# gmongaras/Stable-Diffusion-3-From-Scratch

Measured on AMD Instinct MI355X. Metric: train images/sec MMDiT-B 256^2 bf16, higher is better.
Workload: dtype bf16

## Files before the change

stable-diffusion-3-from-scratch_amd/_lib.py:

```python
import ctypes
import os
import re

_HERE = os.path.dirname(os.path.abspath(__file__))
def experiment(name: str, default: str) -> str:
    return os.environ.get(name, default) if os.environ.get("MMDIT_EXPERIMENTS") == "1" else default


LIB_PATH = os.environ.get("MMDIT_LIB") or os.path.join(_HERE, "libmmdit_hip.so")
HEADER_PATH = os.path.join(_HERE, "..", "include", "mmdit_hip.h")
HEADER_EXT_PATH = os.path.join(_HERE, "..", "include", "mmdit_hip_ext.h")
HEADER_HD128_PATH = os.path.join(_HERE, "..", "include", "mmdit_hip_hd128.h")
HEADER_ROPE3_PATH = os.path.join(_HERE, "..", "include", "mmdit_hip_rope3.h")
HEADER_QKHALF_PATH = os.path.join(_HERE, "..", "include", "mmdit_hip_qkhalf.h")
HEADER_TEXTLOSS_PATH = os.path.join(_HERE, "..", "include", "mmdit_hip_textloss.h")
HEADER_COS2_PATH = os.path.join(_HERE, "..", "include", "mmdit_hip_cos2.h")
HEADER_FP8PAD_PATH = os.path.join(_HERE, "..", "include", "mmdit_hip_fp8pad.h")
HEADER_MXPAD_PATH = os.path.join(_HERE, "..", "include", "mmdit_hip_mxpad.h")
HEADER_OPTIM_PATH = os.path.join(_HERE, "..", "include", "mmdit_hip_optim.h")

F32, BF16 = 0, 1
ACT_NONE, ACT_SILU, ACT_SWIGLU, ACT_SWIGLU_BWD = 0, 1, 2, 3
PREC_BF16, PREC_SPLIT = 0, 1
FP8 = 2

_vp, _i, _i64, _f, _d = ctypes.c_void_p, ctypes.c_int, ctypes.c_int64, ctypes.c_float, ctypes.c_double


class GemmArgs(ctypes.Structure):
    _fields_ = [
        ("A", _vp), ("a_dtype", _i), ("a_kmajor", _i), ("lda", _i64),
        ("B", _vp), ("b_dtype", _i), ("b_kmajor", _i), ("ldb", _i64),
        ("C", _vp), ("c_dtype", _i), ("ldc", _i64),
        ("M", _i), ("N", _i), ("K", _i),
        ("bias", _vp),
        ("act", _i),
        ("gate", _vp), ("ld_gate", _i64), ("rows_per_batch", _i),
        ("residual", _vp), ("ld_res", _i64),
        ("aux", _vp), ("aux_dtype", _i), ("ld_aux", _i64),
        ("accumulate", _i),
        ("precision", _i),
        ("split_k", _i),
        ("stream_k", _i),
        ("conv_mode", _i), ("conv_H", _i), ("conv_W", _i), ("conv_C", _i),
        ("scale_a", _vp), ("scale_b", _vp), ("scale_mode", _i), ("c_scales", _vp),
        ("dbias", _vp),
        ("cu_budget", _i),
    ]


class LnFwdProblem(ctypes.Structure):
    _fields_ = [("x", ctypes.c_void_p), ("acc", ctypes.c_void_p), ("gate", ctypes.c_void_p), ("ld_gate", ctypes.c_int64), ("x_out", ctypes.c_void_p),
                ("scale", ctypes.c_void_p), ("shift", ctypes.c_void_p), ("ld_mod", ctypes.c_int64), ("rows", ctypes.c_int), ("rows_per_batch", ctypes.c_int),
                ("out", ctypes.c_void_p), ("mean", ctypes.c_void_p), ("rstd", ctypes.c_void_p)]


class LnBwdProblem(ctypes.Structure):
    _fields_ = [("dout", ctypes.c_void_p), ("x", ctypes.c_void_p), ("mean", ctypes.c_void_p), ("rstd", ctypes.c_void_p), ("scale", ctypes.c_void_p),
                ("ld_mod", ctypes.c_int64), ("dres", ctypes.c_void_p), ("rows", ctypes.c_int), ("rows_per_batch", ctypes.c_int),
                ("dx", ctypes.c_void_p), ("dscale", ctypes.c_void_p), ("dshift", ctypes.c_void_p), ("ld_dmod", ctypes.c_int64),
                ("acc", ctypes.c_void_p), ("gate", ctypes.c_void_p), ("ld_gate", ctypes.c_int64), ("dacc", ctypes.c_void_p), ("dgate", ctypes.c_void_p),
                ("ld_dgate", ctypes.c_int64), ("dbias", ctypes.c_void_p), ("ld_dbias", ctypes.c_int64)]


class QkProblem(ctypes.Structure):
    _fields_ = [("qkv", ctypes.c_void_p), ("wq", ctypes.c_void_p), ("wk", ctypes.c_void_p), ("rope_cos", ctypes.c_void_p), ("rope_sin", ctypes.c_void_p),
                ("tokens", ctypes.c_int), ("tok0", ctypes.c_int), ("dqkv", ctypes.c_void_p), ("dwq", ctypes.c_void_p), ("dwk", ctypes.c_void_p)]


class MlpBwdProblem(ctypes.Structure):
    _fields_ = [("dh", ctypes.c_void_p), ("gu", ctypes.c_void_p), ("dgu", ctypes.c_void_p), ("rows", ctypes.c_int), ("dbias", ctypes.c_void_p)]


class QkEpilogue(ctypes.Structure):
    _fields_ = [("wq", _vp), ("wk", _vp), ("rope_cos", _vp), ("rope_sin", _vp), ("tokens", _i), ("tok0", _i)]


_SIGNATURES = {
    "mmdit_abi_version": ([], _i),
    "mmdit_struct_size": ([_i], _i),
    "mmdit_build_arch": ([], ctypes.c_char_p),
    "mmdit_gemm": ([ctypes.POINTER(GemmArgs), _vp], _i),
    "mmdit_gemm_grouped": ([ctypes.POINTER(GemmArgs), _i, _vp], _i),
    "mmdit_gemm_plan": ([ctypes.POINTER(GemmArgs), _i], _i),
    "mmdit_gemm_set_workspace": ([_vp, ctypes.c_longlong], _i),
    "mmdit_debug_occupy": ([_i, ctypes.c_longlong, _vp], _i),
    "mmdit_gemm_set_claiming": ([_i], _i),
    "mmdit_gemm_get_claiming": ([], _i),
    "mmdit_device_cus": ([], _i),
    "mmdit_gemm_qkv_norm_rope": ([ctypes.POINTER(GemmArgs), ctypes.POINTER(QkEpilogue), _i, _i, _i, _vp, _vp, _vp, _vp], _i),
    "mmdit_gemm_zero_mask": ([ctypes.POINTER(GemmArgs), _i, ctypes.POINTER(ctypes.c_uint)], _i),
    "mmdit_fp8_amax": ([_vp, _i, _i64, _vp, _vp], _i),
    "mmdit_fp8_quantize": ([_vp, _i, _i64, _vp, _vp, _vp, _vp], _i),
    "mmdit_fp8_quantize_delayed": ([_vp, _i, _i64, _vp, _i, ctypes.c_float, _vp, _vp], _i),
    "mmdit_mxfp8_quantize": ([_vp, _i, _i, _i, _i64, _vp, _vp, _vp], _i),
    "mmdit_ln_modulate_fwd_mx": ([_vp, _vp, _i, _vp, _i64, _vp, _vp, _vp, _i64, _i, _i, _i, _vp, _vp, _vp, _vp, _vp], _i),
    "mmdit_swiglu_fwd_mx": ([_vp, _i, _i, _i, _vp, _vp, _vp], _i),
    "mmdit_attn_fwd_mx": ([_vp, _vp, _vp, _i, _i, _i, _i, ctypes.c_float, _vp, _vp, _vp, _vp, _vp], _i),
    "mmdit_cast": ([_vp, _i, _vp, _i, _i64, _vp], _i),
    "mmdit_ln_modulate_fwd": ([ctypes.POINTER(LnFwdProblem), _i, _i, _i, _i, _vp], _i),
    "mmdit_ln_modulate_bwd": ([ctypes.POINTER(LnBwdProblem), _i, _i, _i, _vp], _i),
    "mmdit_qk_norm_rope_fwd": ([ctypes.POINTER(QkProblem), _i, _i, _i, _i, _i, _vp, _vp, _vp, _vp], _i),
    "mmdit_qk_norm_rope_bwd": ([ctypes.POINTER(QkProblem), _i, _vp, _vp, _vp, _i, _i, _i, _i, _i, _i, _vp], _i),
    "mmdit_qk_norm_rope_fwd_merge": ([ctypes.POINTER(QkProblem), _i, _i, _i, _i, _i, _vp, _vp, _vp, _vp], _i),
    "mmdit_qk_norm_rope_bwd_merge": ([ctypes.POINTER(QkProblem), _i, _vp, _vp, _vp, _i, _i, _i, _i, _i, _i, _vp], _i),
    "mmdit_mlp_act_bwd": ([ctypes.POINTER(MlpBwdProblem), _i, _i, _i, _i, _vp], _i),
    "mmdit_gate_residual_fwd": ([_vp, _vp, _i, _vp, _i64, _i, _i, _i, _vp, _vp], _i),
    "mmdit_text_rmsnorm_fwd": ([_vp, _i, _vp, _vp, _vp, _vp, _i, _i, _i, _i, _vp, _vp, _i, _vp], _i),
    "mmdit_text_rmsnorm_bwd": ([_vp, _vp, _i, _vp, _i, _vp, _vp, _vp, _vp, _i, _i, _i, _i, _vp, _vp, _vp, _vp, _vp], _i),
    "mmdit_attn_fwd": ([_vp, _vp, _vp, _i, _i, _i, _i, _f, _i, _vp, _vp, _vp, _vp], _i),
    "mmdit_attn_bwd_qk": ([_vp] * 9 + [_i, _i, _i, _i, _f] + [_vp] * 11 + [_vp], _i),
    "mmdit_attn_bwd": ([_vp, _vp, _vp, _vp, _vp, _vp, _vp, _vp, _vp, _i, _i, _i, _i, _f, _vp, _vp, _vp, _i, _vp], _i),
    "mmdit_attn_fwd_kv": ([_vp, _vp, _vp, _i, _i, _i, _i, _i, _f, _i, _vp, _vp, _vp, _vp], _i),
    "mmdit_attn_bwd_kv": ([_vp, _vp, _vp, _vp, _vp, _vp, _vp, _vp, _vp, _i, _i, _i, _i, _i, _f, _vp, _vp, _vp, _i, _vp], _i),
    "mmdit_swiglu_fwd": ([_vp, _vp, _i, _i, _i, _vp], _i),
    "mmdit_gelu_fwd": ([_vp, _vp, _i, _i, _i, _vp], _i),
    "mmdit_silu_bwd": ([_vp, _i, _vp, _vp, _i, _i, _i, _vp, _i, _vp], _i),
    "mmdit_gate_residual_bwd": ([_vp, _vp, _i, _vp, _i64, _i, _i, _i, _vp, _i, _vp, _i64, _vp, _i64, _vp], _i),
    "mmdit_flow_loss": ([_vp, _vp, _vp, _i, _i64, _f, _vp, _vp, _vp, _vp], _i),
    "mmdit_colsum": ([_vp, _i, _i, _i, _i64, _vp, _vp], _i),
    "mmdit_vae_nchw_to_nhwc": ([_vp, _i, _i, _i, _i, _i, _i, ctypes.c_float, ctypes.c_float, _vp, _vp], _i),
    "mmdit_vae_nhwc_to_nchw": ([_vp, _i, _i, _i, _i, _i, ctypes.c_float, ctypes.c_float, _vp, _vp], _i),
    "mmdit_vae_im2col3x3": ([_vp, _i, _i, _i, _i, _i, _vp, _vp], _i),
    "mmdit_vae_groupnorm": ([_vp, _i, _vp, _vp, _i, _i, _i, _i, _i, ctypes.c_float, _i, _vp, _vp, _i, _vp], _i),
    "mmdit_vae_pad_cast": ([_vp, _i, _i, _i, _i, _i, _i, _vp, _vp], _i),
    "mmdit_vae_softmax_rows": ([_vp, _i, _i, _i, ctypes.c_float, _vp, _vp], _i),
    "mmdit_vae_attn_fwd": ([_vp, _vp, _vp, _i, _i, _i, _i, _f, _vp, _vp], _i),
    "mmdit_patchify": ([_vp, _i, _i, _i, _i, _i, _vp, _i, _vp], _i),
    "mmdit_unpatchify": ([_vp, _i, _i, _i, _i, _i, _vp, _i, _vp], _i),
    "mmdit_time_embed_fwd": ([_vp, _vp, _vp, _i, _i, _vp, _i, _vp], _i),
    "mmdit_time_embed_bwd": ([_vp, _i, _vp, _vp, _vp, _i, _i, _vp, _vp], _i),
    "mmdit_grad_sumsq": ([_vp, _vp, _vp, _i, _vp, _vp], _i),
    "mmdit_clip_coef": ([_vp, _i, _vp, _f, _vp, _vp], _i),
    "mmdit_adamw_step": ([_vp, _vp, _vp, _i, _vp, _vp, _d, _d, _d, _d, _d, _vp], _i),
    "mmdit_adamw_step_dlr": ([_vp, _vp, _vp, _i, _vp, _vp, _vp, _d, _d, _d, _d, _vp], _i),
    "mmdit_cast_multi": ([_vp, _vp, _vp, _i, _vp], _i),
}
_EXT_SIGNATURES = {
    "mmdit_attn_fwd_e4m3": ([_vp, _vp, _vp, _i, _i, _i, _i, _f, _vp, _vp, _vp, _vp, _vp], _i),
}
ATTN_E4M3_KEY_TILE, ATTN_E4M3_QUERY_TILE = 64, 128
_HD128_SIGNATURES = {
    "mmdit_attn_fwd_hd128": _SIGNATURES["mmdit_attn_fwd"],
    "mmdit_attn_bwd_hd128": _SIGNATURES["mmdit_attn_bwd"],
    "mmdit_qk_norm_rope_fwd_hd128": _SIGNATURES["mmdit_qk_norm_rope_fwd"],
    "mmdit_qk_norm_rope_bwd_hd128": _SIGNATURES["mmdit_qk_norm_rope_bwd"],
}
ATTN_HD128_KEY_TILE, ATTN_HD128_QUERY_TILE = 32, 128
QK_HD128_MAX_HEADS, QK_HD128_RL_MIN_ROWS = 21, 2048
_ROPE3_SIGNATURES = {
    "mmdit_qk_norm_rope3_fwd": ([ctypes.POINTER(QkProblem), _i, _i, _i, _i, _i, _i, _vp, _vp, _vp, _vp], _i),
    "mmdit_qk_norm_rope3_bwd": ([ctypes.POINTER(QkProblem), _i, _vp, _vp, _vp, _i, _i, _i, _i, _i, _i, _i, _vp], _i),
}
_QKHALF_SIGNATURES = {
    "mmdit_attn_fwd_qkhalf": _SIGNATURES["mmdit_attn_fwd"],
    "mmdit_attn_bwd_qkhalf": _SIGNATURES["mmdit_attn_bwd"],
    "mmdit_qk_norm_rope_fwd_qkhalf": ([ctypes.POINTER(QkProblem), _i, _i, _i, _i, _i, _i, _i, _vp, _vp, _vp, _vp], _i),
    "mmdit_qk_norm_rope_bwd_qkhalf": ([ctypes.POINTER(QkProblem), _i, _vp, _vp, _vp, _i, _i, _i, _i, _i, _i, _i, _i, _vp], _i),
}
QKHALF_QK_DIM, QKHALF_V_DIM = 32, 64
ATTN_QKHALF_KEY_TILE, ATTN_QKHALF_QUERY_TILE = 32, 128
_TEXTLOSS_SIGNATURES = {
    "mmdit_text_loss": ([_vp, _i, _vp, _i, _vp, _i64, _i, _f, _vp, _i, _vp, _vp, _vp], _i),
}
TEXT_LOSS_ROWS_PER_WG, TEXT_LOSS_MAX_PARTIALS = 4, 256
TEXT_LOSS_LANE_COLS, TEXT_LOSS_WAVE_COLS = 8, 512
_COS2_SIGNATURES = {
    "mmdit_qk_l2norm_rope_fwd": ([ctypes.POINTER(QkProblem), _i, _i, _i, _i, _i, _i, _vp, _vp, _vp, _vp], _i),
    "mmdit_qk_l2norm_rope_bwd": ([ctypes.POINTER(QkProblem), _i, _vp, _vp, _vp, _i, _i, _i, _i, _i, _i, _vp], _i),
    "mmdit_attn_cos2_ws_bytes": ([_i, _i, _i], ctypes.c_longlong),
    "mmdit_attn_cos2_fwd": ([_vp, _vp, _vp, _i, _i, _i, _i, _i, _vp, _vp, _i, _vp, _vp, _vp], _i),
    "mmdit_attn_cos2_bwd": ([_vp, _vp, _vp, _i, _vp, _vp, _vp, _vp, _i, _vp, _i, _i, _i, _i, _vp, _vp, _vp, _i, _vp, _vp], _i),
}
_FP8PAD_SIGNATURES = {
    "mmdit_fp8_quantize_pad": ([_vp, _i, _i, _i, _i64, _vp, _vp, _vp, _vp], _i),
    "mmdit_fp8_quantize_delayed_pad": ([_vp, _i, _i, _i, _i64, _vp, _i, ctypes.c_float, _vp, _vp], _i),
    "mmdit_mxfp8_quantize_pad": ([_vp, _i, _i, _i, _i64, _vp, _vp, _vp], _i),
}
_MXPAD_SIGNATURES = {
    "mmdit_ln_modulate_fwd_mx_pad": ([ctypes.POINTER(LnFwdProblem), _i, _i, _i, _vp, _vp, _vp], _i),
    "mmdit_attn_fwd_mx_pad": _SIGNATURES["mmdit_attn_fwd_mx"],
    "mmdit_attn_fwd_e4m3_mx_pad": _EXT_SIGNATURES["mmdit_attn_fwd_e4m3"],
}
_OPTIM_SIGNATURES = {
    "mmdit_adamw_step_dlr_pt": _SIGNATURES["mmdit_adamw_step_dlr"],
}
COS2_HEAD_DIM = 64
ATTN_COS2_TOKEN_CHUNK, ATTN_COS2_ROW_TILE = 128, 64
HEAD_DIMS = (64, 128)
ADAMW_CHUNK = 65536
ABI_VERSION = 10
_STRUCTS = [("mmdit_gemm_args", GemmArgs), ("mmdit_ln_fwd_problem", LnFwdProblem), ("mmdit_ln_bwd_problem", LnBwdProblem),
            ("mmdit_qk_problem", QkProblem), ("mmdit_mlp_bwd_problem", MlpBwdProblem), ("mmdit_adamw_tensor", None), ("mmdit_cast_tensor", None), ("mmdit_qk_epilogue", QkEpilogue)]

_lib = None


def declared_symbols():
    with open(HEADER_PATH) as f:
        txt = f.read()
    return sorted(set(re.findall(r"\b(mmdit_[a-z0-9_]+)\s*\(", txt)) - {"mmdit_stream_t"})


def declared_ext_symbols():
    with open(HEADER_EXT_PATH) as f:
        txt = f.read()
    return sorted(set(re.findall(r"\b(mmdit_[a-z0-9_]+)\s*\(", txt)) - {"mmdit_stream_t"})


def declared_hd128_symbols():
    with open(HEADER_HD128_PATH) as f:
        txt = f.read()
    return sorted(set(re.findall(r"\b(mmdit_[a-z0-9_]+)\s*\(", txt)) - {"mmdit_stream_t"})


def declared_rope3_symbols():
    with open(HEADER_ROPE3_PATH) as f:
        txt = f.read()
    return sorted(set(re.findall(r"\b(mmdit_[a-z0-9_]+)\s*\(", txt)) - {"mmdit_stream_t"})


def declared_qkhalf_symbols():
    with open(HEADER_QKHALF_PATH) as f:
        txt = f.read()
    return sorted(set(re.findall(r"\b(mmdit_[a-z0-9_]+)\s*\(", txt)) - {"mmdit_stream_t"})


def declared_textloss_symbols():
    with open(HEADER_TEXTLOSS_PATH) as f:
        txt = f.read()
    return sorted(set(re.findall(r"\b(mmdit_[a-z0-9_]+)\s*\(", txt)) - {"mmdit_stream_t"})


def declared_cos2_symbols():
    with open(HEADER_COS2_PATH) as f:
        txt = f.read()
    return sorted(set(re.findall(r"\b(mmdit_[a-z0-9_]+)\s*\(", txt)) - {"mmdit_stream_t"})


def declared_fp8pad_symbols():
    with open(HEADER_FP8PAD_PATH) as f:
        txt = f.read()
    return sorted(set(re.findall(r"\b(mmdit_[a-z0-9_]+)\s*\(", txt)) - {"mmdit_stream_t"})


def declared_mxpad_symbols():
    with open(HEADER_MXPAD_PATH) as f:
        txt = f.read()
    return sorted(set(re.findall(r"\b(mmdit_[a-z0-9_]+)\s*\(", txt)) - {"mmdit_stream_t"})


def declared_optim_symbols():
    with open(HEADER_OPTIM_PATH) as f:
        txt = f.read()
    return sorted(set(re.findall(r"\b(mmdit_[a-z0-9_]+)\s*\(", txt)) - {"mmdit_stream_t"})


def lib():
    global _lib
    if _lib is None:
        if not os.path.exists(LIB_PATH):
            raise RuntimeError(
                f"{LIB_PATH} is missing: build it with `python __graft_entry__.py build` "
                "(hipcc --offload-arch=gfx950).  There is no PyTorch/CPU fallback for the MMDiT hot path.")
        try:
            import torch
            if torch.cuda.is_available():
                torch.cuda.init()
        except ImportError:
            pass
        L = ctypes.CDLL(LIB_PATH)
        for name, (argtypes, restype) in (list(_SIGNATURES.items()) + list(_EXT_SIGNATURES.items()) + list(_HD128_SIGNATURES.items()) + list(_ROPE3_SIGNATURES.items())
                                          + list(_QKHALF_SIGNATURES.items()) + list(_TEXTLOSS_SIGNATURES.items()) + list(_COS2_SIGNATURES.items()) + list(_FP8PAD_SIGNATURES.items()) + list(_MXPAD_SIGNATURES.items())
                                          + list(_OPTIM_SIGNATURES.items())):
            fn = getattr(L, name)
            fn.argtypes = argtypes
            fn.restype = restype
        if L.mmdit_abi_version() != ABI_VERSION:
            raise RuntimeError(f"{LIB_PATH}: ABI version {L.mmdit_abi_version()}, this binding is written for {ABI_VERSION}: rebuild (python __graft_entry__.py build)")
        for which, (name, struct) in enumerate(_STRUCTS):
            if struct is not None and L.mmdit_struct_size(which) != ctypes.sizeof(struct):
                raise RuntimeError(f"{LIB_PATH}: sizeof({name}) = {L.mmdit_struct_size(which)}, the binding's ctypes mirror has {ctypes.sizeof(struct)} bytes")
        _lib = L
    return _lib


ERR_ARG, ERR_DTYPE, ERR_SHAPE = -1, -2, -3


def check(status: int, what: str):
    if status != 0:
        kind = {-1: "invalid argument", -2: "dtype combination not built", -3: "unsupported shape"}.get(status, f"hipError {status}")
        raise RuntimeError(f"{what} failed: {kind}")
```

stable-diffusion-3-from-scratch_amd/build.py:

```python
import hashlib
import os
import subprocess
import sys
from concurrent.futures import ThreadPoolExecutor

HERE = os.path.dirname(os.path.abspath(__file__))
CSRC = os.path.join(HERE, "csrc")
LIB = os.path.join(HERE, "libmmdit_hip.so")
HEADER = os.path.join(HERE, "..", "include", "mmdit_hip.h")
HEADER_EXT = os.path.join(HERE, "..", "include", "mmdit_hip_ext.h")
HEADER_HD128 = os.path.join(HERE, "..", "include", "mmdit_hip_hd128.h")
HEADER_ROPE3 = os.path.join(HERE, "..", "include", "mmdit_hip_rope3.h")
HEADER_QKHALF = os.path.join(HERE, "..", "include", "mmdit_hip_qkhalf.h")
HEADER_TEXTLOSS = os.path.join(HERE, "..", "include", "mmdit_hip_textloss.h")
HEADER_COS2 = os.path.join(HERE, "..", "include", "mmdit_hip_cos2.h")
HEADER_FP8PAD = os.path.join(HERE, "..", "include", "mmdit_hip_fp8pad.h")
HEADER_MXPAD = os.path.join(HERE, "..", "include", "mmdit_hip_mxpad.h")
HEADER_OPTIM = os.path.join(HERE, "..", "include", "mmdit_hip_optim.h")
SOURCES = ["gemm.hip", "gemm_dma.hip", "gemm_lean.hip", "gemm8p.hip", "gemm8p_inf.hip", "rowops.hip", "fp8_pad.hip", "attention.hip", "attention_e4m3.hip", "attention_hd128.hip", "rowops_rope3.hip", "attention_qkhalf.hip", "rowops_qkhalf.hip", "attention_cos2.hip", "rowops_cos2.hip", "text_loss.hip", "vae.hip", "vae_attn.hip", "optim.hip"]
HIPCC = os.environ.get("HIPCC", "/opt/rocm/bin/hipcc")
FLAGS = ["--offload-arch=gfx950", "-O3", "-std=c++17", "-fPIC"] + os.environ.get("MMDIT_EXTRA_HIPCC_FLAGS", "").split()
SOURCE_FLAGS = {"vae_attn.hip": ["-mllvm", "-amdgpu-mfma-vgpr-form=1"]}


def _sha(paths, extra=""):
    h = hashlib.sha256(extra.encode())
    for p in paths:
        with open(p, "rb") as f:
            h.update(os.path.basename(p).encode() + b"\0" + f.read() + b"\0")
    return h.hexdigest()


def _read(path):
    try:
        with open(path) as f:
            return f.read().strip()
    except OSError:
        return None


def source_hash(src):
    headers = sorted(os.path.join(CSRC, f) for f in os.listdir(CSRC) if f.endswith(".h")) + [HEADER, HEADER_EXT, HEADER_HD128, HEADER_ROPE3, HEADER_QKHALF, HEADER_TEXTLOSS, HEADER_COS2, HEADER_FP8PAD, HEADER_MXPAD, HEADER_OPTIM]
    if src == "gemm8p_inf.hip":
        headers.append(os.path.join(CSRC, "gemm8p.hip"))
    return _sha([os.path.join(CSRC, src)] + headers, " ".join([HIPCC] + FLAGS + SOURCE_FLAGS.get(src, [])))


def build(force: bool = False, verbose: bool = False) -> str:
    want = {src: source_hash(src) for src in SOURCES}

    def cc(src):
        obj = os.path.join(CSRC, src.replace(".hip", ".o"))
        if not force and os.path.exists(obj) and _read(obj + ".sha") == want[src]:
            return obj, False
        cmd = [HIPCC] + FLAGS + SOURCE_FLAGS.get(src, []) + ["-c", os.path.join(CSRC, src), "-o", obj]
        if verbose:
            print(" ".join(cmd), flush=True)
        subprocess.run(cmd, check=True)
        with open(obj + ".sha", "w") as f:
            f.write(want[src])
        return obj, True

    with ThreadPoolExecutor(max_workers=8) as ex:
        res = list(ex.map(cc, SOURCES))
    objs = [o for o, _ in res]
    libsha = hashlib.sha256("".join(want[s] for s in SOURCES).encode()).hexdigest()
    if force or any(c for _, c in res) or not os.path.exists(LIB) or _read(LIB + ".sha") != libsha:
        cmd = [HIPCC, "--offload-arch=gfx950", "-shared", "-fPIC", "-o", LIB] + objs
        if verbose:
            print(" ".join(cmd), flush=True)
        subprocess.run(cmd, check=True)
        with open(LIB + ".sha", "w") as f:
            f.write(libsha)
    return LIB


def is_current() -> bool:
    libsha = hashlib.sha256("".join(source_hash(s) for s in SOURCES).encode()).hexdigest()
    return os.path.exists(LIB) and _read(LIB + ".sha") == libsha


if __name__ == "__main__":
    print(build(force="--force" in sys.argv, verbose=True))
```

stable-diffusion-3-from-scratch_amd/csrc/rowops.hip:

```cpp
#include "qk_rows.h"
#include "fp8_quant.h"
#include "../../include/mmdit_hip_hd128.h"
#include "../../include/mmdit_hip_mxpad.h"

namespace {

constexpr float LN_EPS = 1e-5f;

__device__ __forceinline__ float bf16_round(float x) { return __builtin_bit_cast(float, pack_bf2(x, 0.f) << 16); }

template <int NITX, typename TO, typename TA, bool RES, bool MX = false, bool PAD = false>
__device__ __forceinline__ void ln_mod_fwd_body(int block, const float* __restrict__ x, const float* __restrict__ scale, const float* __restrict__ shift,
                                                int64_t ld_mod, int rows, int d, int rpb, TO* __restrict__ out,
                                                float* __restrict__ mean_o, float* __restrict__ rstd_o,
                                                const TA* __restrict__ acc, const float* __restrict__ gate, int64_t ld_gate, float* __restrict__ xo,
                                                unsigned char* __restrict__ mx_scales) {
  constexpr int NIT = NITX < 0 ? -NITX : NITX;
  constexpr bool EXACT = NITX < 0;
  const int lane = threadIdx.x & 63, row = block * 4 + (threadIdx.x >> 6);
  if (row >= rows) return;
  const int nch = d >> 2;
  const int b = row / rpb;
  const float* xr = x + (int64_t)row * d;
  float v[NIT][4];
  float s = 0.f;
#pragma unroll
  for (int it = 0; it < NIT; it++) {
    int ch = lane + 64 * it;
    if (EXACT || ch < nch) {
      ld4(xr + ch * 4, v[it]);
      if constexpr (RES) {
        float av[4], g[4];
        ld4(acc + (int64_t)row * d + ch * 4, av);
        ld4(gate + (int64_t)b * ld_gate + ch * 4, g);
#pragma unroll
        for (int e = 0; e < 4; e++) v[it][e] = v[it][e] + g[e] * av[e];
        __builtin_nontemporal_store(f32x4{v[it][0], v[it][1], v[it][2], v[it][3]}, (f32x4*)(xo + (int64_t)row * d + ch * 4));
      }
      s += v[it][0] + v[it][1] + v[it][2] + v[it][3];
    }
    else { v[it][0] = v[it][1] = v[it][2] = v[it][3] = 0.f; }
  }
  const float mean = wave_sum(s) / d;
  float q = 0.f;
#pragma unroll
  for (int it = 0; it < NIT; it++) {
    int ch = lane + 64 * it;
    if (EXACT || ch < nch) {
#pragma unroll
      for (int e = 0; e < 4; e++) { float c = v[it][e] - mean; q += c * c; }
    }
  }
  const float rstd = rsqrtf(wave_sum(q) / d + LN_EPS);
  if (lane == 0) { mean_o[row] = mean; rstd_o[row] = rstd; }
  const float* sc = scale + (int64_t)b * ld_mod;
  const float* sh = shift + (int64_t)b * ld_mod;
  TO* orow = out + (int64_t)row * d;
  const int ldo = PAD ? d + 64 : d;
  if constexpr (PAD) {
    if (lane < 4) *(uint4*)((unsigned char*)out + (int64_t)row * ldo + d + lane * 16) = make_uint4(0u, 0u, 0u, 0u);
    if (lane < 2) mx_scales[mx_scale_index(row, (d >> 5) + lane, rows)] = 0;
  }
#pragma unroll
  for (int it = 0; it < NIT; it++) {
    int ch = lane + 64 * it;
    if (EXACT || ch < nch) {
      float a[4], h[4], o[4];
      ld4(sc + ch * 4, a); ld4(sh + ch * 4, h);
#pragma unroll
      for (int e = 0; e < 4; e++) o[e] = (v[it][e] - mean) * rstd * (1.f + a[e]) + h[e];
      if constexpr (MX) {
#pragma unroll
        for (int e = 0; e < 4; e++) o[e] = bf16_round(o[e]);
        float amax = fmaxf(fmaxf(fabsf(o[0]), fabsf(o[1])), fmaxf(fabsf(o[2]), fabsf(o[3])));
        amax = fmaxf(amax, __shfl_xor(amax, 1, 64));
        amax = fmaxf(amax, __shfl_xor(amax, 2, 64));
        amax = fmaxf(amax, __shfl_xor(amax, 4, 64));
        float inv;
        const int ex = mx_exponent(amax, inv);
        *(unsigned*)((unsigned char*)out + (int64_t)row * ldo + ch * 4) = mx_pack4(o, inv);
        if ((lane & 7) == 0) mx_scales[mx_scale_index(row, ch >> 3, rows)] = (unsigned char)(ex + 127);
      } else {
        st4(orow + ch * 4, o);
      }
    }
  }
}

struct LnFwdProb {
  const float* x; const float* scale; const float* shift; int64_t ld_mod; int rows, rpb; void* out; float* mean; float* rstd;
  const void* acc; const float* gate; int64_t ld_gate; float* xo; unsigned char* mx_scales;
};
template <int NIT, typename TO, typename TA, bool RES, bool MX = false, bool PAD = false>
__global__ __launch_bounds__(256) void ln_mod_fwd_kernel(LnFwdProb p0, LnFwdProb p1, int nblk0, int d) {
  const bool first = (int)blockIdx.x < nblk0;
  const LnFwdProb& p = first ? p0 : p1;
  ln_mod_fwd_body<NIT, TO, TA, RES, MX, PAD>(first ? (int)blockIdx.x : (int)blockIdx.x - nblk0, p.x, p.scale, p.shift, p.ld_mod, p.rows, d, p.rpb, (TO*)p.out, p.mean, p.rstd,
                                        (const TA*)p.acc, p.gate, p.ld_gate, p.xo, p.mx_scales);
}

template <typename TA>
__global__ __launch_bounds__(256) void gate_residual_fwd_kernel(const float* __restrict__ x, const TA* __restrict__ acc, const float* __restrict__ gate, int64_t ld_gate,
                                                                int rows, int d, int rpb, float* __restrict__ out) {
  const int nch = d >> 2;
  for (int64_t i = (int64_t)blockIdx.x * 256 + threadIdx.x; i < (int64_t)rows * nch; i += (int64_t)gridDim.x * 256) {
    const int row = (int)(i / nch), ch = (int)(i - (int64_t)row * nch);
    float xv[4], av[4], g[4];
    ld4(x + (int64_t)row * d + ch * 4, xv);
    ld4(acc + (int64_t)row * d + ch * 4, av);
    ld4(gate + (int64_t)(row / rpb) * ld_gate + ch * 4, g);
#pragma unroll
    for (int e = 0; e < 4; e++) xv[e] = xv[e] + g[e] * av[e];
    st4(out + (int64_t)row * d + ch * 4, xv);
  }
}

#ifndef MMDIT_LN_BWD_RCH
#define MMDIT_LN_BWD_RCH 16
#endif
constexpr int LN_BWD_RCH = MMDIT_LN_BWD_RCH;
template <int NITX, typename TG, typename TA, bool GATED>
__device__ __forceinline__ void ln_mod_bwd_body(int block, const TG* __restrict__ dout, const float* __restrict__ x, const float* __restrict__ mean_i,
                                                const float* __restrict__ rstd_i, const float* __restrict__ scale, int64_t ld_mod,
                                                const float* __restrict__ dres, int d, int rpb, int nchunk,
                                                float* __restrict__ dx, float* __restrict__ dscale, float* __restrict__ dshift, int64_t ld_dmod,
                                                const TA* __restrict__ acc, const float* __restrict__ gate, int64_t ld_gate, TA* __restrict__ dacc,
                                                float* __restrict__ dgate, int64_t ld_dgate, float* __restrict__ dbias, int64_t ld_dbias, int rch = LN_BWD_RCH) {
  constexpr int NIT = NITX < 0 ? -NITX : NITX;
  constexpr bool EXACT = NITX < 0;
  const int lane = threadIdx.x & 63, wave = threadIdx.x >> 6;
  const int b = block / nchunk, chunk = block % nchunk;
  const int nch = d >> 2;
  const float* sc = scale + (int64_t)b * ld_mod;
  __shared__ float s_a1[NIT * 256], s_gt[GATED ? NIT * 256 : 4];
  for (int c = threadIdx.x; c < NIT * 256; c += 256) {
    s_a1[c] = c < d ? sc[c] + 1.f : 0.f;
    if constexpr (GATED) s_gt[c] = c < d ? gate[(int64_t)b * ld_gate + c] : 0.f;
  }
  __syncthreads();
  float ds[NIT][4], dh[NIT][4];
  float sg[GATED ? NIT : 1][4], sb[GATED ? NIT : 1][4];
#pragma unroll
  for (int it = 0; it < NIT; it++) {
#pragma unroll
    for (int e = 0; e < 4; e++) { ds[it][e] = 0.f; dh[it][e] = 0.f; }
    if constexpr (GATED) {
#pragma unroll
      for (int e = 0; e < 4; e++) { sg[it][e] = 0.f; sb[it][e] = 0.f; }
    }
  }
  const int rend = min(rpb, (chunk + 1) * rch);
  for (int rl = chunk * rch + wave; rl < rend; rl += 4) {
    const int64_t row = (int64_t)b * rpb + rl;
    const float mean = mean_i[row], rstd = rstd_i[row];
    float g[NIT][4], xh[NIT][4];
    float c1 = 0.f, c2 = 0.f;
    asm volatile("" ::: "memory");
#pragma unroll
    for (int it = 0; it < NIT; it++) {
      int ch = lane + 64 * it;
      if (EXACT || ch < nch) {
        float dy[4], xv[4], a1[4];
        ld4_nt(dout + row * d + ch * 4, dy);
        ld4_nt(x + row * d + ch * 4, xv);
        ld4(s_a1 + ch * 4, a1);
#pragma unroll
        for (int e = 0; e < 4; e++) {
          xh[it][e] = (xv[e] - mean) * rstd;
          g[it][e] = dy[e] * a1[e];
          c1 += g[it][e]; c2 += g[it][e] * xh[it][e];
          ds[it][e] += dy[e] * xh[it][e]; dh[it][e] += dy[e];
        }
      }
    }
    c1 = wave_sum(c1) / d; c2 = wave_sum(c2) / d;
#pragma unroll
    for (int it = 0; it < NIT; it++) {
      int ch = lane + 64 * it;
      if (EXACT || ch < nch) {
        float o[4];
        if (dres) ld4(dres + row * d + ch * 4, o); else { o[0] = o[1] = o[2] = o[3] = 0.f; }
#pragma unroll
        for (int e = 0; e < 4; e++) o[e] += rstd * (g[it][e] - c1 - xh[it][e] * c2);
        st4(dx + row * d + ch * 4, o);
        if constexpr (GATED) {
          float av[4], da[4], gt[4];
          ld4_nt(acc + row * d + ch * 4, av);
          ld4(s_gt + ch * 4, gt);
#pragma unroll
          for (int e = 0; e < 4; e++) { da[e] = o[e] * gt[e]; sg[it][e] += o[e] * av[e]; sb[it][e] += da[e]; }
          st4(dacc + row * d + ch * 4, da);
        }
      }
    }
  }
  if constexpr (NIT <= 6) {
    __shared__ float red[4][NIT * 256];
    auto flush = [&](const float (&v)[NIT][4], float* dst) {
#pragma unroll
      for (int it = 0; it < NIT; it++)
#pragma unroll
        for (int e = 0; e < 4; e++) red[wave][(it * 64 + lane) * 4 + e] = v[it][e];
      __syncthreads();
      for (int c = threadIdx.x; c < d; c += 256) atomicAdd(dst + c, red[0][c] + red[1][c] + red[2][c] + red[3][c]);
      __syncthreads();
    };
    flush(ds, dscale + (int64_t)b * ld_dmod);
    flush(dh, dshift + (int64_t)b * ld_dmod);
    if constexpr (GATED) {
      flush(sg, dgate + (int64_t)b * ld_dgate);
      if (dbias) flush(sb, dbias + (int64_t)b * ld_dbias);
    }
  } else {
    auto flush = [&](const float (&v)[NIT][4], float* dst) {
#pragma unroll
      for (int it = 0; it < NIT; it++) {
        int ch = lane + 64 * it;
        if (EXACT || ch < nch) {
#pragma unroll
          for (int e = 0; e < 4; e++) atomicAdd(dst + ch * 4 + e, v[it][e]);
        }
      }
    };
    flush(ds, dscale + (int64_t)b * ld_dmod);
    flush(dh, dshift + (int64_t)b * ld_dmod);
    if constexpr (GATED) {
      flush(sg, dgate + (int64_t)b * ld_dgate);
      if (dbias) flush(sb, dbias + (int64_t)b * ld_dbias);
    }
  }
}

struct LnBwdProb {
  const void* dout; const float* x; const float* mean; const float* rstd; const float* scale; int64_t ld_mod; const float* dres; int rpb, nchunk;
  float* dx; float* dscale; float* dshift; int64_t ld_dmod;
  const void* acc; const float* gate; int64_t ld_gate; void* dacc; float* dgate; int64_t ld_dgate; float* dbias; int64_t ld_dbias;
};
template <int NIT, typename TG, typename TA, bool GATED>
__global__ __launch_bounds__(256) void ln_mod_bwd_kernel(LnBwdProb p0, LnBwdProb p1, int nblk0, int d, int rch) {
  const bool first = (int)blockIdx.x < nblk0;
  const LnBwdProb& p = first ? p0 : p1;
  ln_mod_bwd_body<NIT, TG, TA, GATED>(first ? (int)blockIdx.x : (int)blockIdx.x - nblk0, (const TG*)p.dout, p.x, p.mean, p.rstd, p.scale, p.ld_mod, p.dres, d, p.rpb, p.nchunk,
                                      p.dx, p.dscale, p.dshift, p.ld_dmod, (const TA*)p.acc, p.gate, p.ld_gate, (TA*)p.dacc, p.dgate, p.ld_dgate, p.dbias, p.ld_dbias, rch);
}

template <int NITX, typename TI, typename TO>
__global__ __launch_bounds__(256) void text_rms_fwd_kernel(const TI* __restrict__ x, const float* __restrict__ w, const float* __restrict__ sp,
                                                           int rows, int cnt, int tokens, int off, int d, TO* __restrict__ out) {
  constexpr int NIT = NITX < 0 ? -NITX : NITX;
  constexpr bool EXACT = NITX < 0;
  const int lane = threadIdx.x & 63, m = blockIdx.x * 4 + (threadIdx.x >> 6);
  if (m >= rows) return;
  const int nch = d >> 2;
  const TI* xr = x + ((int64_t)(m / cnt) * tokens + off + m % cnt) * d;
  float v[NIT][4];
  float q = 0.f;
#pragma unroll
  for (int it = 0; it < NIT; it++) {
    int ch = lane + 64 * it;
    if (EXACT || ch < nch) { ld4(xr + ch * 4, v[it]); q += v[it][0] * v[it][0] + v[it][1] * v[it][1] + v[it][2] * v[it][2] + v[it][3] * v[it][3]; }
  }
  const float rinv = rsqrtf(wave_sum(q) / d + RMS_EPS);
  const float s = sp[0];
  TO* orow = out + (int64_t)m * d;
#pragma unroll
  for (int it = 0; it < NIT; it++) {
    int ch = lane + 64 * it;
    if (EXACT || ch < nch) {
      float wv[4], o[4];
      ld4(w + ch * 4, wv);
#pragma unroll
      for (int e = 0; e < 4; e++) o[e] = s * (v[it][e] * rinv * wv[e]);
      st4(orow + ch * 4, o);
    }
  }
}

#ifndef TRB_ROWS
#define TRB_ROWS 64
#endif
struct TextRmsBwdHalf { const void* dout; const float* w; const float* sp; int rows, cnt, off; float* dw; float* dsp; };
template <int NITX, typename TI, typename TG>
__global__ __launch_bounds__(512) void text_rms_bwd_kernel(TextRmsBwdHalf h0, TextRmsBwdHalf h1, const TI* __restrict__ x, int tokens, int d) {
  constexpr int NIT = NITX < 0 ? -NITX : NITX;
  constexpr bool EXACT = NITX < 0;
  const TextRmsBwdHalf& hp = blockIdx.y == 0 ? h0 : h1;
  const TG* __restrict__ dout = (const TG*)hp.dout;
  const float* __restrict__ w = hp.w;
  const float* __restrict__ sp = hp.sp;
  const int rows = hp.rows, cnt = hp.cnt, off = hp.off;
  float* __restrict__ dw = hp.dw;
  float* __restrict__ dsp = hp.dsp;
  __shared__ float red[NIT * 256];
  for (int c = threadIdx.x; c < NIT * 256; c += 512) red[c] = 0.f;
  __syncthreads();
  const int lane = threadIdx.x & 63, wave = threadIdx.x >> 6;
  const int nch = d >> 2;
  const float s = sp[0];
  float accw[NIT][4], wv[NIT][4];
  float accs = 0.f;
#pragma unroll
  for (int it = 0; it < NIT; it++) {
    int ch = lane + 64 * it;
    if (EXACT || ch < nch) ld4(w + ch * 4, wv[it]); else { wv[it][0] = wv[it][1] = wv[it][2] = wv[it][3] = 0.f; }
#pragma unroll
    for (int e = 0; e < 4; e++) accw[it][e] = 0.f;
  }
  for (int m = blockIdx.x * TRB_ROWS + wave; m < min(rows, (int)(blockIdx.x + 1) * TRB_ROWS); m += 8) {
    const TI* xr = x + ((int64_t)(m / cnt) * tokens + off + m % cnt) * d;
    float v[NIT][4];
    float q = 0.f;
#pragma unroll
    for (int it = 0; it < NIT; it++) {
      int ch = lane + 64 * it;
      if (EXACT || ch < nch) { ld4(xr + ch * 4, v[it]); q += v[it][0] * v[it][0] + v[it][1] * v[it][1] + v[it][2] * v[it][2] + v[it][3] * v[it][3]; }
    }
    const float rinv = rsqrtf(wave_sum(q) / d + RMS_EPS);
#pragma unroll
    for (int it = 0; it < NIT; it++) {
      int ch = lane + 64 * it;
      if (EXACT || ch < nch) {
        float dy[4];
        ld4(dout + (int64_t)m * d + ch * 4, dy);
#pragma unroll
        for (int e = 0; e < 4; e++) { float xn = v[it][e] * rinv; accw[it][e] += dy[e] * s * xn; accs += dy[e] * xn * wv[it][e]; }
      }
    }
  }
#pragma unroll
  for (int it = 0; it < NIT; it++) {
    const int ch = lane + 64 * it;
    if (EXACT || ch < nch) {
#pragma unroll
      for (int e = 0; e < 4; e++) atomicAdd(&red[ch * 4 + e], accw[it][e]);
    }
  }
  __syncthreads();
#ifndef TRB_NO_GLOBAL
  for (int c = threadIdx.x; c < d; c += 512) atomicAdd(dw + c, red[c]);
#else
  if (red[threadIdx.x] == 123.456f) dw[0] = 1.f;
#endif
  accs = wave_sum(accs);
#ifndef TRB_NO_DSP
  if (lane == 0) atomicAdd(dsp, accs);
#else
  if (accs == 123.456f) dsp[0] = 1.f;
#endif
}


template <int HD, typename TI>
__device__ __forceinline__ void qk_norm_rope_fwd_body(int bid, int rstride, const TI* __restrict__ qkv, const float* __restrict__ wq, const float* __restrict__ wk,
                                                      const float* __restrict__ rcos, const float* __restrict__ rsin,
                                                      int rows, int tokens, int heads, int s_total, int tok0,
                                                      bf16_t* __restrict__ Q, bf16_t* __restrict__ K, bf16_t* __restrict__ V) {
  constexpr int CH = HD / 8, LOG_CH = CH == 8 ? 3 : 4;
  const int hc = threadIdx.x % (CH * heads), part = threadIdx.x / (CH * heads), head = hc >> LOG_CH, chunk = hc & (CH - 1);
  bf16_t* obase = part == 0 ? Q : part == 1 ? K : V;
  float w[8];
#pragma unroll
  for (int e = 0; e < 8; e++) w[e] = 0.f;
  if (part < 2) ld8((part == 0 ? wq : wk) + chunk * 8, w);
  const bool same_token = rcos && rstride % tokens == 0;
  float cs[2][8], sn[2][8];
  if (same_token && part < 2) {
    const int n = bid % tokens;
    ld8(rcos + (int64_t)n * HD + chunk * 8, cs[0]);
    ld8(rsin + (int64_t)n * HD + chunk * 8, sn[0]);
#pragma unroll
    for (int e = 0; e < 8; e++) { cs[1][e] = cs[0][e]; sn[1][e] = sn[0][e]; }
  }
  for (int row0 = bid; row0 < rows; row0 += 2 * rstride) {
    float x[2][8];
#pragma unroll
    for (int k = 0; k < 2; k++) {
      const int row = min(row0 + k * rstride, rows - 1);
      ld8(qkv + (((int64_t)row * 3 + part) * heads + head) * HD + chunk * 8, x[k]);
    }
    if (part < 2 && rcos && !same_token) {
#pragma unroll
      for (int k = 0; k < 2; k++) {
        const int n = min(row0 + k * rstride, rows - 1) % tokens;
        ld8(rcos + (int64_t)n * HD + chunk * 8, cs[k]);
        ld8(rsin + (int64_t)n * HD + chunk * 8, sn[k]);
      }
    }
#pragma unroll
    for (int k = 0; k < 2; k++) {
      const int row = row0 + k * rstride;
      if (row >= rows) break;
      const int n = row % tokens, b = row / tokens;
      if (part < 2) {
        float ss = 0.f;
#pragma unroll
        for (int e = 0; e < 8; e++) ss += x[k][e] * x[k][e];
        const float rinv = rsqrtf(group_sum<CH>(ss) * (1.f / HD) + RMS_EPS);
#pragma unroll
        for (int e = 0; e < 8; e++) x[k][e] = x[k][e] * rinv * w[e];
        if (rcos) {
#pragma unroll
          for (int p = 0; p < 4; p++) {
            float a = x[k][2 * p], bb = x[k][2 * p + 1];
            x[k][2 * p] = a * cs[k][2 * p] - bb * sn[k][2 * p];
            x[k][2 * p + 1] = bb * cs[k][2 * p + 1] + a * sn[k][2 * p + 1];
          }
        }
      }
      st8(obase + (((int64_t)b * heads + head) * s_total + tok0 + n) * HD + chunk * 8, x[k]);
    }
  }
}
template <int HD, typename TI>
__global__ __launch_bounds__(1024) void qk_norm_rope_fwd_kernel(QkProb p0, QkProb p1, int g0, int heads, int s_total,
                                                                bf16_t* __restrict__ Q, bf16_t* __restrict__ K, bf16_t* __restrict__ V) {
  QK_SELECT(p, bid, nwg);
  qk_norm_rope_fwd_body<HD, TI>(bid, nwg, (const TI*)p.qkv, p.wq, p.wk, p.rcos, p.rsin, p.rows, p.tokens, heads, s_total, p.tok0, Q, K, V);
}

enum QkFactors {
  QK_ONCE,
  QK_PER_PAIR,
  QK_PER_ROW,
};

template <int HD, QkFactors F, typename TG, typename TI, typename TO>
__device__ __forceinline__ void qk_norm_rope_bwd_body(int bid, int rstride, const TG* __restrict__ dQ, const TG* __restrict__ dK, const TG* __restrict__ dV,
                                                      const TI* __restrict__ qkv, const float* __restrict__ wq, const float* __restrict__ wk,
                                                      const float* __restrict__ rcos, const float* __restrict__ rsin,
                                                      int rows, int tokens, int heads, int s_total, int tok0,
                                                      TO* __restrict__ dqkv, float* __restrict__ dwq, float* __restrict__ dwk) {
  constexpr int CH = HD / 8, LOG_CH = CH == 8 ? 3 : 4, LOG_HD = LOG_CH + 3;
  __shared__ float sdw[2][HD];
  for (int i = threadIdx.x; i < 2 * HD; i += blockDim.x) sdw[i >> LOG_HD][i & (HD - 1)] = 0.f;
  __syncthreads();
  const int per_row = 3 * CH * heads, rlane = threadIdx.x / per_row, t = threadIdx.x - rlane * per_row;
  { const int RL = blockDim.x / per_row; bid = bid * RL + rlane; rstride *= RL; }
  const int hc = t % (CH * heads), part = t / (CH * heads);
  const int head = HD == 64 ? hc >> LOG_CH : hc / CH, chunk = HD == 64 ? hc & (CH - 1) : hc % CH;
  const TG* gbase = part == 0 ? dQ : part == 1 ? dK : dV;
  float w[8], aw[8];
#pragma unroll
  for (int e = 0; e < 8; e++) { w[e] = 0.f; aw[e] = 0.f; }
  if (part < 2) ld8((part == 0 ? wq : wk) + chunk * 8, w);
  const bool same_token = F == QK_ONCE ? rcos != nullptr : (rcos && rstride % tokens == 0);
  constexpr int NF = F == QK_PER_PAIR ? 2 : 1;
  float cs[NF][8], sn[NF][8];
  if (same_token && part < 2) {
    const int n = bid % tokens;
    ld8(rcos + (int64_t)n * HD + chunk * 8, cs[0]);
    ld8(rsin + (int64_t)n * HD + chunk * 8, sn[0]);
    if constexpr (F == QK_PER_PAIR) {
#pragma unroll
      for (int e = 0; e < 8; e++) { cs[1][e] = cs[0][e]; sn[1][e] = sn[0][e]; }
    }
  }
  for (int row0 = bid; row0 < rows; row0 += 2 * rstride) {
    float dz[2][8], x[2][8];
#pragma unroll
    for (int k = 0; k < 2; k++) {
      const int row = min(row0 + k * rstride, rows - 1);
      const int n = row % tokens, b = row / tokens;
      ld8_nt(gbase + (((int64_t)b * heads + head) * s_total + tok0 + n) * HD + chunk * 8, dz[k]);
    }
    if (part < 2) {
#pragma unroll
      for (int k = 0; k < 2; k++) {
        const int row = min(row0 + k * rstride, rows - 1);
        ld8_nt(qkv + (((int64_t)row * 3 + part) * heads + head) * HD + chunk * 8, x[k]);
        if constexpr (F == QK_PER_PAIR) {
          if (rcos && !same_token) {
            const int n = row % tokens;
            ld8(rcos + (int64_t)n * HD + chunk * 8, cs[k]);
            ld8(rsin + (int64_t)n * HD + chunk * 8, sn[k]);
          }
        }
      }
    }
// ... 249 lines not shown
  if (ty == 0 && c < ncols) {
#pragma unroll
    for (int e = 0; e < 8; e++) atomicAdd(dst + c + e, acc[e] + sbuf[tx * 8 + e]);
  }
  __syncthreads();
}

constexpr int MB_RCH = 128;
template <typename T, bool GELU>
__device__ __forceinline__ void mlp_act_bwd_body(int by, const T* __restrict__ dh, const T* __restrict__ gu, T* __restrict__ dgu,
                                                 int rows, int hidden, float* __restrict__ dbias) {
  __shared__ float sbuf[8 * 256];
  const int tx = threadIdx.x & 31, ty = threadIdx.x >> 5;
  const int c = blockIdx.x * 256 + tx * 8;
  const bool act = c < hidden;
  const int64_t ldi = GELU ? hidden : 2 * (int64_t)hidden;
  float sg[8], su[8];
#pragma unroll
  for (int e = 0; e < 8; e++) { sg[e] = 0.f; su[e] = 0.f; }
  const int rend = min(rows, (by + 1) * MB_RCH);
  if (act) {
    for (int r0 = by * MB_RCH + ty; r0 < rend; r0 += 16) {
      float d[2][8], g[2][8], u[2][8];
#pragma unroll
      for (int k = 0; k < 2; k++) {
        const int r = r0 + 8 * k;
        if (r < rend) {
          ld8_nt(dh + (int64_t)r * hidden + c, d[k]);
          ld8_nt(gu + r * ldi + c, g[k]);
          if constexpr (!GELU) ld8_nt(gu + r * ldi + hidden + c, u[k]);
        }
      }
#pragma unroll
      for (int k = 0; k < 2; k++) {
        const int r = r0 + 8 * k;
        if (r >= rend) break;
        float og[8], ou[8];
        if constexpr (GELU) {
#pragma unroll
          for (int e = 0; e < 8; e++) { og[e] = d[k][e] * gelu_grad_f(g[k][e]); sg[e] += og[e]; }
          st8(dgu + r * ldi + c, og);
        } else {
#pragma unroll
          for (int e = 0; e < 8; e++) {
            swiglu_bwd_f(d[k][e], g[k][e], u[k][e], og[e], ou[e]);
            sg[e] += og[e]; su[e] += ou[e];
          }
          st8(dgu + r * ldi + c, og);
          st8(dgu + r * ldi + hidden + c, ou);
        }
      }
    }
  }
  if (dbias) {
    const int col = blockIdx.x * 256 + threadIdx.x;
#pragma unroll
    for (int which = 0; which < (GELU ? 1 : 2); which++) {
#pragma unroll
      for (int e = 0; e < 8; e++) sbuf[ty * 256 + tx * 8 + e] = which == 0 ? sg[e] : su[e];
      __syncthreads();
      if (col < hidden) {
        float s = 0.f;
#pragma unroll
        for (int r = 0; r < 8; r++) s += sbuf[r * 256 + threadIdx.x];
        atomicAdd(dbias + which * hidden + col, s);
      }
      __syncthreads();
    }
  }
}
struct MlpBwdProb { const void* dh; const void* gu; void* dgu; int rows; float* dbias; };
template <typename T, bool GELU>
__global__ __launch_bounds__(256) void mlp_act_bwd_kernel(MlpBwdProb p0, MlpBwdProb p1, int nby0, int hidden) {
  const bool first = (int)blockIdx.y < nby0;
  const MlpBwdProb& p = first ? p0 : p1;
  mlp_act_bwd_body<T, GELU>(first ? (int)blockIdx.y : (int)blockIdx.y - nby0, (const T*)p.dh, (const T*)p.gu, (T*)p.dgu, p.rows, hidden, p.dbias);
}

constexpr int GR_RCH = 64;
template <typename TA, typename TO>
__global__ __launch_bounds__(256) void gate_res_bwd_kernel(const float* __restrict__ dy, const TA* __restrict__ acc, const float* __restrict__ gate, int64_t ld_gate,
                                                           int d, int rpb, int nchunk, TO* __restrict__ dacc,
                                                           float* __restrict__ dgate, int64_t ld_dgate, float* __restrict__ dbias, int64_t ld_dbias) {
  __shared__ float sbuf[8 * 256];
  const int tx = threadIdx.x & 31, ty = threadIdx.x >> 5;
  const int c = blockIdx.x * 256 + tx * 8;
  const bool act = c < d;
  const int b = blockIdx.y / nchunk, chunk = blockIdx.y % nchunk;
  float g[8], sgate[8], sb[8];
#pragma unroll
  for (int e = 0; e < 8; e++) { g[e] = 0.f; sgate[e] = 0.f; sb[e] = 0.f; }
  if (act) {
    ld8(gate + (int64_t)b * ld_gate + c, g);
    const int rend = min(rpb, (chunk + 1) * GR_RCH);
    for (int rl = chunk * GR_RCH + ty; rl < rend; rl += 16) {
      const int64_t row0 = (int64_t)b * rpb + rl, row1 = row0 + 8;
      const bool two = rl + 8 < rend;
      float dv0[8], av0[8], dv1[8], av1[8], o[8];
      ld8(dy + row0 * d + c, dv0);
      ld8(acc + row0 * d + c, av0);
      if (two) {
        ld8(dy + row1 * d + c, dv1);
        ld8(acc + row1 * d + c, av1);
      }
#pragma unroll
      for (int e = 0; e < 8; e++) { o[e] = dv0[e] * g[e]; sgate[e] += dv0[e] * av0[e]; sb[e] += o[e]; }
      st8(dacc + row0 * d + c, o);
      if (two) {
#pragma unroll
        for (int e = 0; e < 8; e++) { o[e] = dv1[e] * g[e]; sgate[e] += dv1[e] * av1[e]; sb[e] += o[e]; }
        st8(dacc + row1 * d + c, o);
      }
    }
  }
  const int col = blockIdx.x * 256 + threadIdx.x;
#pragma unroll
  for (int which = 0; which < 2; which++) {
    float* dst = which == 0 ? dgate + (int64_t)b * ld_dgate : (dbias ? dbias + (int64_t)b * ld_dbias : nullptr);
    if (!dst) break;
#pragma unroll
    for (int e = 0; e < 8; e++) sbuf[ty * 256 + tx * 8 + e] = which == 0 ? sgate[e] : sb[e];
    __syncthreads();
    if (col < d) {
      float s = 0.f;
#pragma unroll
      for (int r = 0; r < 8; r++) s += sbuf[r * 256 + threadIdx.x];
      atomicAdd(dst + col, s);
    }
    __syncthreads();
  }
}

template <typename T>
__global__ __launch_bounds__(256) void colsum_kernel(const T* __restrict__ x, int rows, int cols, int64_t ld, float* __restrict__ out, int rch) {
  __shared__ float sbuf[1024];
  const int tx = threadIdx.x & 127, ty = threadIdx.x >> 7;
  const int c = blockIdx.x * 1024 + tx * 8;
  float s[8];
#pragma unroll
  for (int e = 0; e < 8; e++) s[e] = 0.f;
  if (c < cols) {
    const int rend = min(rows, (int)(blockIdx.y + 1) * rch);
#pragma unroll 4
    for (int r = blockIdx.y * rch + ty; r < rend; r += 2) {
      float v[8];
      ld8(x + r * ld + c, v);
#pragma unroll
      for (int e = 0; e < 8; e++) s[e] += v[e];
    }
  }
  colsum_flush(s, sbuf, out, c, cols);
}

template <typename TG, typename TO>
__global__ __launch_bounds__(256) void silu_bwd_kernel(const TG* __restrict__ dy, const float* __restrict__ pre, TO* __restrict__ dpre, int rpg, int cols, float* __restrict__ dbias) {
  __shared__ float sb[4][64];
  const int cl = threadIdx.x & 63, rl = threadIdx.x >> 6;
  const int c = blockIdx.x * 64 + cl;
  const int r0 = blockIdx.y * rpg;
  float s = 0.f;
  if (c < cols) {
#pragma unroll 4
    for (int r = r0 + rl; r < r0 + rpg; r += 4) {
      const int64_t i = (int64_t)r * cols + c;
      const float p = pre[i], sig = sigmoid_f(p);
      const float g = io<TG>::ld(dy + i) * sig * (1.f + p * (1.f - sig));
      io<TO>::st(dpre + i, g);
      s += g;
    }
  }
  sb[rl][cl] = s;
  __syncthreads();
  if (rl == 0 && c < cols && dbias) dbias[(int64_t)blockIdx.y * cols + c] += sb[0][cl] + sb[1][cl] + sb[2][cl] + sb[3][cl];
}

template <typename TI, typename TO>
__global__ void cast_kernel(const TI* __restrict__ src, TO* __restrict__ dst, int64_t n) {
  const int64_t n8 = n >> 3;
  for (int64_t i = (int64_t)blockIdx.x * blockDim.x + threadIdx.x; i < n8; i += (int64_t)gridDim.x * blockDim.x) {
    float v[8];
    ld8(src + i * 8, v);
    st8(dst + i * 8, v);
  }
  if (blockIdx.x == 0 && threadIdx.x < (n & 7)) io<TO>::st(dst + n8 * 8 + threadIdx.x, io<TI>::ld(src + n8 * 8 + threadIdx.x));
}

template <typename TI, typename TO, bool TO_TOKENS>
__global__ void patch_kernel(const TI* __restrict__ src, TO* __restrict__ dst, int batch, int ch, int H, int W) {
  const int W2 = W >> 1, H2 = H >> 1;
  const int64_t total = (int64_t)batch * ch * H * W2;
  for (int64_t g = (int64_t)blockIdx.x * blockDim.x + threadIdx.x; g < total; g += (int64_t)gridDim.x * blockDim.x) {
    const int j = (int)(g % W2); int64_t r = g / W2;
    const int y = (int)(r % H); r /= H;
    const int c = (int)(r % ch); const int64_t b = r / ch;
    const int64_t img_off = ((b * ch + c) * H + y) * W + 2 * j;
    const int64_t tok_off = ((b * H2 + (y >> 1)) * W2 + j) * (int64_t)(ch * 4) + c * 4 + (y & 1) * 2;
    if (TO_TOKENS) { io<TO>::st(dst + tok_off, io<TI>::ld(src + img_off)); io<TO>::st(dst + tok_off + 1, io<TI>::ld(src + img_off + 1)); }
    else { io<TO>::st(dst + img_off, io<TI>::ld(src + tok_off)); io<TO>::st(dst + img_off + 1, io<TI>::ld(src + tok_off + 1)); }
  }
}

template <typename TO>
__global__ void time_embed_fwd_kernel(const float* __restrict__ t, const float* __restrict__ ts, const float* __restrict__ denom, int batch, int dim, TO* __restrict__ out) {
  const int i = blockIdx.x * blockDim.x + threadIdx.x, b = blockIdx.y;
  if (i >= dim) return;
  const float tau = t[b] * ts[0];
  const int half = dim >> 1;
  const float v = i < half ? sinf(tau / denom[2 * i]) : cosf(tau / denom[2 * (i - half) + 1]);
  io<TO>::st(out + (int64_t)b * dim + i, v);
}

template <typename TG>
__global__ __launch_bounds__(256) void time_embed_bwd_kernel(const TG* __restrict__ dout, const float* __restrict__ t, const float* __restrict__ ts,
                                                             const float* __restrict__ denom, int batch, int dim, float* __restrict__ dts) {
  __shared__ float red[4];
  const int b = blockIdx.x;
  const float tau = t[b] * ts[0];
  const int half = dim >> 1;
  float s = 0.f;
  for (int i = threadIdx.x; i < dim; i += 256) {
    const float g = io<TG>::ld(dout + (int64_t)b * dim + i);
    if (i < half) { const float dn = denom[2 * i]; s += g * cosf(tau / dn) / dn; }
    else { const float dn = denom[2 * (i - half) + 1]; s -= g * sinf(tau / dn) / dn; }
  }
  s = wave_sum(s);
  if ((threadIdx.x & 63) == 0) red[threadIdx.x >> 6] = s;
  __syncthreads();
  if (threadIdx.x == 0) atomicAdd(dts, (red[0] + red[1] + red[2] + red[3]) * t[b]);
}

inline int nit_for(int d) { return (d / 4 + 63) / 64; }
inline int grid_cap(int64_t n, int bs) { int64_t g = (n + bs - 1) / bs; return (int)(g < 1 ? 1 : g > 4096 ? 4096 : g); }

}

#define NIT_CASE(n, ...)                                                        \
  { if (d == (n) * 256) { constexpr int NIT = -(n); __VA_ARGS__; } else { constexpr int NIT = (n); __VA_ARGS__; } }
#define NIT_SWITCH(nit, ...)                                    \
  do {                                                          \
    if (nit <= 1) NIT_CASE(1, __VA_ARGS__)                      \
    else if (nit <= 2) NIT_CASE(2, __VA_ARGS__)                 \
    else if (nit <= 3) NIT_CASE(3, __VA_ARGS__)                 \
    else if (nit <= 4) NIT_CASE(4, __VA_ARGS__)                 \
    else if (nit <= 6) NIT_CASE(6, __VA_ARGS__)                 \
    else if (nit <= 9) NIT_CASE(9, __VA_ARGS__)                 \
    else if (nit <= 12) NIT_CASE(12, __VA_ARGS__)               \
    else NIT_CASE(16, __VA_ARGS__)                              \
  } while (0)

#define LN_FWD_NIT (NIT < 0 ? -NIT : NIT)

extern "C" int mmdit_abi_version(void) { return MMDIT_ABI_VERSION; }
extern "C" int mmdit_struct_size(int which) {
  switch (which) {
    case 0: return (int)sizeof(mmdit_gemm_args);
    case 1: return (int)sizeof(mmdit_ln_fwd_problem);
    case 2: return (int)sizeof(mmdit_ln_bwd_problem);
    case 3: return (int)sizeof(mmdit_qk_problem);
    case 4: return (int)sizeof(mmdit_mlp_bwd_problem);
    case 5: return (int)sizeof(mmdit_adamw_tensor);
    case 6: return (int)sizeof(mmdit_cast_tensor);
    case 7: return (int)sizeof(mmdit_qk_epilogue);
    default: return -1;
  }
}
extern "C" const char* mmdit_build_arch(void) { return "gfx950"; }

static int ln_mod_fwd_launch(const mmdit_ln_fwd_problem* probs, int count, int d, int out_dtype, unsigned char* const* mx_scales, hipStream_t s, bool pad = false) {
  MMDIT_CHECK_ARG(probs && count >= 1 && count <= 2 && d > 0 && d % 4 == 0 && d <= 4096);
  const bool res = probs[0].acc != nullptr;
  LnFwdProb q[2] = {};
  int nb[2] = {0, 0};
  for (int i = 0; i < count; i++) {
    const mmdit_ln_fwd_problem* p = probs + i;
    MMDIT_CHECK_ARG((p->acc != nullptr) == res);
    MMDIT_CHECK_ARG(p->x && p->scale && p->shift && p->out && p->mean && p->rstd && p->rows > 0 && p->rows_per_batch > 0 && p->ld_mod % 4 == 0);
    if (res) MMDIT_CHECK_ARG(p->gate && p->x_out && p->ld_gate % 4 == 0);
    q[i] = LnFwdProb{p->x, p->scale, p->shift, p->ld_mod, p->rows, p->rows_per_batch, p->out, p->mean, p->rstd, p->acc, p->gate, p->ld_gate, p->x_out, mx_scales ? mx_scales[i] : nullptr};
    nb[i] = (p->rows + 3) / 4;
  }
  const int nit = nit_for(d);
  dim3 grid(nb[0] + nb[1]);
#define LNL(TO, TA, RES, ...) NIT_SWITCH(nit, hipLaunchKernelGGL((ln_mod_fwd_kernel<LN_FWD_NIT, TO, TA, RES, __VA_ARGS__>), grid, dim3(256), 0, s, q[0], q[1], nb[0], d))
  if (mx_scales && pad) { if (res) { LNL(unsigned char, bf16_t, true, true, true); } else { LNL(unsigned char, bf16_t, false, true, true); } }
  else if (mx_scales) { if (res) { LNL(unsigned char, bf16_t, true, true); } else { LNL(unsigned char, bf16_t, false, true); } }
  else if (out_dtype == MMDIT_BF16) { if (res) { LNL(bf16_t, bf16_t, true, false); } else { LNL(bf16_t, bf16_t, false, false); } }
  else if (out_dtype == MMDIT_F32) { if (res) { LNL(float, float, true, false); } else { LNL(float, float, false, false); } }
  else return MMDIT_ERR_DTYPE;
#undef LNL
  return mmdit_launch_status();
}

extern "C" int mmdit_ln_modulate_fwd(const mmdit_ln_fwd_problem* probs, int count, int d, int acc_dtype, int out_dtype, mmdit_stream_t stream) {
  MMDIT_CHECK_ARG(probs && count >= 1 && (!probs[0].acc || acc_dtype == out_dtype));
  return ln_mod_fwd_launch(probs, count, d, out_dtype, nullptr, (hipStream_t)stream);
}

extern "C" int mmdit_ln_modulate_fwd_mx(const float* x, const void* acc, int acc_dtype, const float* gate, int64_t ld_gate, float* x_out,
                                        const float* scale, const float* shift, int64_t ld_mod, int rows, int d, int rpb,
                                        void* q_fp8, void* scales_e8m0, float* mean, float* rstd, mmdit_stream_t stream) {
  MMDIT_CHECK_ARG(scales_e8m0 && d % 64 == 0 && (!acc || acc_dtype == MMDIT_BF16));
  const mmdit_ln_fwd_problem p = {x, acc, gate, ld_gate, x_out, scale, shift, ld_mod, rows, rpb, q_fp8, mean, rstd};
  unsigned char* const sc[1] = {(unsigned char*)scales_e8m0};
  return ln_mod_fwd_launch(&p, 1, d, MMDIT_FP8, sc, (hipStream_t)stream);
}

extern "C" int mmdit_ln_modulate_fwd_mx_pad(const mmdit_ln_fwd_problem* probs, int count, int d, int acc_dtype, void* scales_e8m0_0, void* scales_e8m0_1,
                                            mmdit_stream_t stream) {
  MMDIT_CHECK_ARG(probs && count >= 1 && count <= 2 && scales_e8m0_0 && (count == 1 || scales_e8m0_1));
  if (d <= 0 || d % 64 != 0) return MMDIT_ERR_SHAPE;
  for (int i = 0; i < count; i++)
    if (probs[i].rows > 0 && (int64_t)probs[i].rows * ((d + 127) / 128 * 128) / 16 > 0x7fffffffll) return MMDIT_ERR_SHAPE;
  MMDIT_CHECK_ARG(!probs[0].acc || acc_dtype == MMDIT_BF16);
  unsigned char* const sc[2] = {(unsigned char*)scales_e8m0_0, (unsigned char*)scales_e8m0_1};
  return ln_mod_fwd_launch(probs, count, d, MMDIT_FP8, sc, (hipStream_t)stream, d % 128 != 0);
}

extern "C" int mmdit_gate_residual_fwd(const float* x, const void* acc, int acc_dtype, const float* gate, int64_t ld_gate, int rows, int d, int rpb,
                                       float* out, mmdit_stream_t stream) {
  MMDIT_CHECK_ARG(x && acc && gate && out && rows > 0 && d > 0 && d % 4 == 0 && rpb > 0 && ld_gate % 4 == 0);
  hipStream_t s = (hipStream_t)stream;
  dim3 grid(grid_cap((int64_t)rows * (d / 4), 256));
  if (acc_dtype == MMDIT_BF16) hipLaunchKernelGGL((gate_residual_fwd_kernel<bf16_t>), grid, dim3(256), 0, s, x, (const bf16_t*)acc, gate, ld_gate, rows, d, rpb, out);
  else if (acc_dtype == MMDIT_F32) hipLaunchKernelGGL((gate_residual_fwd_kernel<float>), grid, dim3(256), 0, s, x, (const float*)acc, gate, ld_gate, rows, d, rpb, out);
  else return MMDIT_ERR_DTYPE;
  return mmdit_launch_status();
}

static int ln_bwd_one_round_rch(const mmdit_ln_bwd_problem* a, const mmdit_ln_bwd_problem* b, int d, int dout_dtype, bool gated) {
  auto wgs = [&](int r) { return (long)(a->rows / a->rows_per_batch) * ((a->rows_per_batch + r - 1) / r) + (long)(b->rows / b->rows_per_batch) * ((b->rows_per_batch + r - 1) / r); };
  const int nit_ = nit_for(d), nit_abs = nit_ < 0 ? -nit_ : nit_;
  int per_cu = nit_abs <= 3 ? 4 : nit_abs == 4 ? 3 : 2, cus = 256;
  {
    static int occ[64][17][2][2], cu_count[64];
    const int dev = mmdit_current_device(), ti = dout_dtype == MMDIT_BF16 ? 0 : 1, gi = gated ? 1 : 0, ni = nit_abs > 16 ? 16 : nit_abs;
    if (!cu_count[dev]) {
      int n = 0;
      cu_count[dev] = (hipDeviceGetAttribute(&n, hipDeviceAttributeMultiprocessorCount, dev) == hipSuccess && n > 0) ? n : 256;
    }
    cus = cu_count[dev];
    if (!occ[dev][ni][ti][gi]) {
      int nbq = 0;
      hipError_t e = hipErrorUnknown;
#define LNQ(T, G) NIT_SWITCH(nit_, e = hipOccupancyMaxActiveBlocksPerMultiprocessor(&nbq, (const void*)ln_mod_bwd_kernel<(NIT < 0 ? -NIT : NIT), T, T, G>, 256, 0))
      if (dout_dtype == MMDIT_BF16) { if (gated) { LNQ(bf16_t, true); } else { LNQ(bf16_t, false); } }
      else if (dout_dtype == MMDIT_F32) { if (gated) { LNQ(float, true); } else { LNQ(float, false); } }
#undef LNQ
      occ[dev][ni][ti][gi] = (e == hipSuccess && nbq > 0) ? nbq : 8;
    }
    per_cu = per_cu < occ[dev][ni][ti][gi] ? per_cu : occ[dev][ni][ti][gi];
  }
  const long slots = (long)cus * per_cu;
  if (wgs(LN_BWD_RCH) > slots && wgs(LN_BWD_RCH) <= 2 * slots)
    for (int r = LN_BWD_RCH + 4; r <= 64; r += 4)
      if (wgs(r) <= slots) return r;
  return LN_BWD_RCH;
}

extern "C" int mmdit_ln_modulate_bwd(const mmdit_ln_bwd_problem* probs, int count, int d, int dout_dtype, mmdit_stream_t stream) {
  MMDIT_CHECK_ARG(probs && count >= 1 && count <= 2 && d > 0 && d % 4 == 0 && d <= 4096);
  const bool gated = probs[0].acc != nullptr;
  for (int i = 0; i < count; i++) {
    const mmdit_ln_bwd_problem* p = probs + i;
    MMDIT_CHECK_ARG((p->acc != nullptr) == gated);
    MMDIT_CHECK_ARG(p->dout && p->x && p->mean && p->rstd && p->scale && p->dx && p->dscale && p->dshift && p->rows > 0 && p->rows_per_batch > 0 &&
                    p->rows % p->rows_per_batch == 0 && p->ld_mod % 4 == 0);
    if (gated) MMDIT_CHECK_ARG(p->gate && p->dacc && p->dgate && p->ld_gate % 4 == 0);
  }
  if (dout_dtype != MMDIT_BF16 && dout_dtype != MMDIT_F32) return MMDIT_ERR_DTYPE;
  const int rch = count == 2 ? ln_bwd_one_round_rch(probs, probs + 1, d, dout_dtype, gated) : LN_BWD_RCH;
  LnBwdProb q[2] = {};
  int nb[2] = {0, 0};
  for (int i = 0; i < count; i++) {
    const mmdit_ln_bwd_problem* p = probs + i;
    const int nchunk = (p->rows_per_batch + rch - 1) / rch;
    nb[i] = (p->rows / p->rows_per_batch) * nchunk;
    q[i] = LnBwdProb{p->dout, p->x, p->mean, p->rstd, p->scale, p->ld_mod, p->dres, p->rows_per_batch, nchunk, p->dx, p->dscale, p->dshift, p->ld_dmod,
                     p->acc, p->gate, p->ld_gate, p->dacc, p->dgate, p->ld_dgate, p->dbias, p->ld_dbias};
  }
  hipStream_t s = (hipStream_t)stream;
  const int nit = nit_for(d);
  dim3 grid(nb[0] + nb[1]);
#define LNL(T, G) NIT_SWITCH(nit, hipLaunchKernelGGL((ln_mod_bwd_kernel<(NIT < 0 ? -NIT : NIT), T, T, G>), grid, dim3(256), 0, s, q[0], q[1], nb[0], d, rch))
  if (dout_dtype == MMDIT_BF16) { if (gated) { LNL(bf16_t, true); } else { LNL(bf16_t, false); } }
  else { if (gated) { LNL(float, true); } else { LNL(float, false); } }
#undef LNL
  return mmdit_launch_status();
}

extern "C" int mmdit_text_rmsnorm_fwd(const void* x, int x_dtype, const float* w1, const float* w2, const float* s1, const float* s2,
                                      int batch, int tokens, int split, int d, void* out1, void* out2, int out_dtype, mmdit_stream_t stream) {
  MMDIT_CHECK_ARG(x && w1 && w2 && s1 && s2 && out1 && out2 && batch > 0 && split > 0 && split < tokens && d % 4 == 0 && d <= 4096);
  hipStream_t s = (hipStream_t)stream;
  const int nit = nit_for(d);
  for (int half = 0; half < 2; half++) {
    const int cnt = half ? tokens - split : split, off = half ? split : 0, rows = batch * cnt;
    const float* w = half ? w2 : w1; const float* sp = half ? s2 : s1; void* out = half ? out2 : out1;
    dim3 grid((rows + 3) / 4);
#define TRF(TI, TO) NIT_SWITCH(nit, hipLaunchKernelGGL((text_rms_fwd_kernel<LN_FWD_NIT, TI, TO>), grid, dim3(256), 0, s, (const TI*)x, w, sp, rows, cnt, tokens, off, d, (TO*)out))
    if (x_dtype == MMDIT_F32 && out_dtype == MMDIT_F32) { TRF(float, float); }
    else if (x_dtype == MMDIT_F32 && out_dtype == MMDIT_BF16) { TRF(float, bf16_t); }
    else if (x_dtype == MMDIT_BF16 && out_dtype == MMDIT_BF16) { TRF(bf16_t, bf16_t); }
    else if (x_dtype == MMDIT_BF16 && out_dtype == MMDIT_F32) { TRF(bf16_t, float); }
    else return MMDIT_ERR_DTYPE;
#undef TRF
  }
  return mmdit_launch_status();
}

extern "C" int mmdit_text_rmsnorm_bwd(const void* dout1, const void* dout2, int dout_dtype, const void* x, int x_dtype,
                                      const float* w1, const float* w2, const float* s1, const float* s2, int batch, int tokens, int split, int d,
                                      float* dw1, float* dw2, float* ds1, float* ds2, mmdit_stream_t stream) {
  MMDIT_CHECK_ARG(dout1 && dout2 && x && w1 && w2 && s1 && s2 && dw1 && dw2 && ds1 && ds2 && batch > 0 && split > 0 && split < tokens && d % 4 == 0 && d <= 4096);
  hipStream_t s = (hipStream_t)stream;
  const int nit = nit_for(d);
  TextRmsBwdHalf h[2];
  int maxrows = 0;
  for (int half = 0; half < 2; half++) {
    const int cnt = half ? tokens - split : split, rows = batch * cnt;
    h[half] = TextRmsBwdHalf{half ? dout2 : dout1, half ? w2 : w1, half ? s2 : s1, rows, cnt, half ? split : 0, half ? dw2 : dw1, half ? ds2 : ds1};
    maxrows = rows > maxrows ? rows : maxrows;
  }
  dim3 grid((maxrows + TRB_ROWS - 1) / TRB_ROWS, 2);
#define TRB(TI, TG) NIT_SWITCH(nit, hipLaunchKernelGGL((text_rms_bwd_kernel<NIT, TI, TG>), grid, dim3(512), 0, s, h[0], h[1], (const TI*)x, tokens, d))
  if (x_dtype == MMDIT_F32 && dout_dtype == MMDIT_F32) { TRB(float, float); }
  else if (x_dtype == MMDIT_F32 && dout_dtype == MMDIT_BF16) { TRB(float, bf16_t); }
  else if (x_dtype == MMDIT_BF16 && dout_dtype == MMDIT_BF16) { TRB(bf16_t, bf16_t); }
  else if (x_dtype == MMDIT_BF16 && dout_dtype == MMDIT_F32) { TRB(bf16_t, float); }
  else return MMDIT_ERR_DTYPE;
#undef TRB
  return mmdit_launch_status();
}

constexpr int QK_RL_MIN_ROWS = 2048;
static_assert(QK_RL_MIN_ROWS == MMDIT_QK_HD128_RL_MIN_ROWS && 1024 / (3 * 128 / 8) == MMDIT_QK_HD128_MAX_HEADS, "include/mmdit_hip_hd128.h documents this policy");
static int qk_rl(int row_threads, int min_rows) {
  static const int env = [] { const char* e = mmdit_exp_env("MMDIT_QK_RL"); return e ? atoi(e) : 0; }();
  int rl = 1024 / row_threads;
  if (env > 0 && env < rl) rl = env;
  if (rl < 1 || min_rows < QK_RL_MIN_ROWS) rl = 1;
  return rl;
}
static int qk_bwd_lanes(int rl) {
  static const int env = [] { const char* e = mmdit_exp_env("MMDIT_QK_LANES"); return e ? atoi(e) : 768; }();
  return rl > 1 ? env : 512;
}
static int qk_grid(int hd, int rows, int tokens, bool rope, int lanes_max, int rl) {
  const int lanes = rows < lanes_max ? rows : lanes_max;
  if (rope && tokens <= lanes) {
    int k = lanes / tokens;
    while (k > 1 && (k * tokens) % rl) k--;
    if ((k * tokens) % rl == 0) return k * tokens / rl;
  }
  if (hd == 64 && rope && tokens > lanes && tokens <= rows && tokens <= (rl > 1 ? 2048 : 1024) && tokens % rl == 0) return tokens / rl;
  return lanes / rl > 0 ? lanes / rl : 1;
}

template <int HD>
static int qk_fwd_launch(const mmdit_qk_problem* probs, int count, int qkv_dtype, int batch, int heads, int s_total, int heads_err,
                         void* Q, void* K, void* V, mmdit_stream_t stream) {
  constexpr int ROW_T = 3 * HD / 8;
  MMDIT_CHECK_ARG(Q && K && V);
  QkProb q[2] = {};
  if (int e = qk_list(probs, count, batch, heads, HD, s_total, 1024 / ROW_T, heads_err, false, false, nullptr, nullptr, nullptr, q)) return e;
  if (qkv_dtype != MMDIT_BF16 && qkv_dtype != MMDIT_F32) return MMDIT_ERR_DTYPE;
  int g[2] = {0, 0};
  for (int i = 0; i < count; i++) g[i] = qk_grid(HD, q[i].rows, q[i].tokens, q[i].rcos != nullptr, 1024, 1);
  hipStream_t s = (hipStream_t)stream;
  const dim3 grid(g[0] + g[1]), block(ROW_T * heads);
  if (qkv_dtype == MMDIT_BF16) hipLaunchKernelGGL((qk_norm_rope_fwd_kernel<HD, bf16_t>), grid, block, 0, s, q[0], q[1], g[0], heads, s_total, (bf16_t*)Q, (bf16_t*)K, (bf16_t*)V);
  else hipLaunchKernelGGL((qk_norm_rope_fwd_kernel<HD, float>), grid, block, 0, s, q[0], q[1], g[0], heads, s_total, (bf16_t*)Q, (bf16_t*)K, (bf16_t*)V);
  return mmdit_launch_status();
}

template <int HD>
static int qk_bwd_launch(const mmdit_qk_problem* probs, int count, const void* dQ, const void* dK, const void* dV, int dq_dtype,
                         int qkv_dtype, int dqkv_dtype, int batch, int heads, int s_total, int heads_err, mmdit_stream_t stream) {
  constexpr int ROW_T = 3 * HD / 8;
  QkProb q[2] = {};
  if (int e = qk_list(probs, count, batch, heads, HD, s_total, 1024 / ROW_T, heads_err, false, true, dQ, dK, dV, q)) return e;
  const int combo = qk_bwd_combo(dq_dtype, qkv_dtype, dqkv_dtype);
  if (combo < 0) return MMDIT_ERR_DTYPE;
  const int rl = qk_rl(ROW_T * heads, count == 2 && q[1].rows < q[0].rows ? q[1].rows : q[0].rows);
  int g[2] = {0, 0};
  bool once = true;
  for (int i = 0; i < count; i++) {
    g[i] = qk_grid(HD, q[i].rows, q[i].tokens, q[i].rcos != nullptr, qk_bwd_lanes(rl), rl);
    once = once && (!q[i].rcos || (g[i] * rl) % q[i].tokens == 0);
  }
  hipStream_t s = (hipStream_t)stream;
  const dim3 grid(g[0] + g[1]), block(ROW_T * heads * rl);
#define QKL(F, TG, TI, TO) hipLaunchKernelGGL((qk_norm_rope_bwd_kernel<HD, F, TG, TI, TO>), grid, block, 0, s, q[0], q[1], g[0], heads, s_total)
#define QKF(TG, TI, TO) do { if constexpr (HD == 128) QKL(QK_PER_ROW, TG, TI, TO); else if (once) QKL(QK_ONCE, TG, TI, TO); else QKL(QK_PER_PAIR, TG, TI, TO); } while (0)
  if (combo == 0) QKF(bf16_t, bf16_t, bf16_t);
  else if (combo == 1) QKF(float, float, float);
  else QKF(bf16_t, float, float);
#undef QKF
#undef QKL
  return mmdit_launch_status();
}

extern "C" int mmdit_qk_norm_rope_fwd(const mmdit_qk_problem* probs, int count, int qkv_dtype, int batch, int heads, int s_total,
                                      void* Q, void* K, void* V, mmdit_stream_t stream) {
  return qk_fwd_launch<64>(probs, count, qkv_dtype, batch, heads, s_total, MMDIT_ERR_ARG, Q, K, V, stream);
}
extern "C" int mmdit_qk_norm_rope_bwd(const mmdit_qk_problem* probs, int count, const void* dQ, const void* dK, const void* dV, int dq_dtype,
                                      int qkv_dtype, int dqkv_dtype, int batch, int heads, int s_total, mmdit_stream_t stream) {
  return qk_bwd_launch<64>(probs, count, dQ, dK, dV, dq_dtype, qkv_dtype, dqkv_dtype, batch, heads, s_total, MMDIT_ERR_ARG, stream);
}
extern "C" int mmdit_qk_norm_rope_fwd_hd128(const mmdit_qk_problem* probs, int count, int qkv_dtype, int batch, int heads, int s_total,
                                            void* Q, void* K, void* V, mmdit_stream_t stream) {
  return qk_fwd_launch<128>(probs, count, qkv_dtype, batch, heads, s_total, MMDIT_ERR_SHAPE, Q, K, V, stream);
}
extern "C" int mmdit_qk_norm_rope_bwd_hd128(const mmdit_qk_problem* probs, int count, const void* dQ, const void* dK, const void* dV, int dq_dtype,
                                            int qkv_dtype, int dqkv_dtype, int batch, int heads, int s_total, mmdit_stream_t stream) {
  return qk_bwd_launch<128>(probs, count, dQ, dK, dV, dq_dtype, qkv_dtype, dqkv_dtype, batch, heads, s_total, MMDIT_ERR_SHAPE, stream);
}

constexpr int QK_MERGE_MAX_HEADS = 512 / 24;
extern "C" int mmdit_qk_norm_rope_fwd_merge(const mmdit_qk_problem* probs, int count, int qkv_dtype, int batch, int heads, int s_total,
                                            void* Q, void* K, void* V, mmdit_stream_t stream) {
  MMDIT_CHECK_ARG(Q && K && V);
  QkProb q[2] = {};
  if (int e = qk_list(probs, count, batch, heads, 64, s_total, QK_MERGE_MAX_HEADS, MMDIT_ERR_ARG, true, false, nullptr, nullptr, nullptr, q)) return e;
  if (qkv_dtype != MMDIT_BF16 && qkv_dtype != MMDIT_F32) return MMDIT_ERR_DTYPE;
  int g[2] = {0, 0};
  for (int i = 0; i < count; i++) { const int pairs = q[i].rows / 2; g[i] = pairs < 1024 ? pairs : 1024; }
  hipStream_t s = (hipStream_t)stream;
  dim3 grid(g[0] + g[1]);
  if (qkv_dtype == MMDIT_BF16) hipLaunchKernelGGL((qk_merge_fwd_kernel<bf16_t>), grid, dim3(24 * heads), 0, s, q[0], q[1], g[0], heads, s_total, (bf16_t*)Q, (bf16_t*)K, (bf16_t*)V);
  else hipLaunchKernelGGL((qk_merge_fwd_kernel<float>), grid, dim3(24 * heads), 0, s, q[0], q[1], g[0], heads, s_total, (bf16_t*)Q, (bf16_t*)K, (bf16_t*)V);
  return mmdit_launch_status();
}

extern "C" int mmdit_qk_norm_rope_bwd_merge(const mmdit_qk_problem* probs, int count, const void* dQ, const void* dK, const void* dV, int dq_dtype,
                                            int qkv_dtype, int dqkv_dtype, int batch, int heads, int s_total, mmdit_stream_t stream) {
  QkProb q[2] = {};
  if (int e = qk_list(probs, count, batch, heads, 64, s_total, QK_MERGE_MAX_HEADS, MMDIT_ERR_ARG, true, true, dQ, dK, dV, q)) return e;
  const int combo = qk_bwd_combo(dq_dtype, qkv_dtype, dqkv_dtype);
  if (combo < 0) return MMDIT_ERR_DTYPE;
  int g[2] = {0, 0};
  for (int i = 0; i < count; i++) { const int pairs = q[i].rows / 2; g[i] = pairs < 512 ? pairs : 512; }
  hipStream_t s = (hipStream_t)stream;
  dim3 grid(g[0] + g[1]);
#define QKM(TG, TI, TO) hipLaunchKernelGGL((qk_merge_bwd_kernel<TG, TI, TO>), grid, dim3(24 * heads), 0, s, q[0], q[1], g[0], heads, s_total)
  if (combo == 0) QKM(bf16_t, bf16_t, bf16_t);
  else if (combo == 1) QKM(float, float, float);
  else QKM(bf16_t, float, float);
#undef QKM
  return mmdit_launch_status();
}

extern "C" int mmdit_mlp_act_bwd(const mmdit_mlp_bwd_problem* probs, int count, int dtype, int hidden, int gelu, mmdit_stream_t stream) {
  MMDIT_CHECK_ARG(probs && count >= 1 && count <= 2 && hidden > 0 && hidden % 8 == 0);
  MlpBwdProb q[2] = {};
  int nby[2] = {0, 0};
  for (int i = 0; i < count; i++) {
    MMDIT_CHECK_ARG(probs[i].dh && probs[i].gu && probs[i].dgu && probs[i].rows > 0);
    q[i] = MlpBwdProb{probs[i].dh, probs[i].gu, probs[i].dgu, probs[i].rows, probs[i].dbias};
    nby[i] = (probs[i].rows + MB_RCH - 1) / MB_RCH;
  }
  dim3 grid((hidden + 255) / 256, nby[0] + nby[1]);
  hipStream_t s = (hipStream_t)stream;
#define MBL(T, G) hipLaunchKernelGGL((mlp_act_bwd_kernel<T, G>), grid, dim3(256), 0, s, q[0], q[1], nby[0], hidden)
  if (dtype == MMDIT_BF16) { if (gelu) MBL(bf16_t, true); else MBL(bf16_t, false); }
  else if (dtype == MMDIT_F32) { if (gelu) MBL(float, true); else MBL(float, false); }
  else return MMDIT_ERR_DTYPE;
#undef MBL
  return mmdit_launch_status();
}

template <bool GELU>
static int mlp_act_fwd(const void* gu, void* h, int dtype, int rows, int hidden, mmdit_stream_t stream) {
  MMDIT_CHECK_ARG(gu && h && rows > 0 && hidden > 0 && hidden % 8 == 0);
  dim3 grid((hidden + 255) / 256, (rows + CO_RCH - 1) / CO_RCH);
  hipStream_t s = (hipStream_t)stream;
  if (dtype == MMDIT_BF16) hipLaunchKernelGGL((mlp_act_fwd_kernel<bf16_t, GELU>), grid, dim3(256), 0, s, (const bf16_t*)gu, (bf16_t*)h, rows, hidden);
  else if (dtype == MMDIT_F32) hipLaunchKernelGGL((mlp_act_fwd_kernel<float, GELU>), grid, dim3(256), 0, s, (const float*)gu, (float*)h, rows, hidden);
  else return MMDIT_ERR_DTYPE;
  return mmdit_launch_status();
}
extern "C" int mmdit_swiglu_fwd_mx(const void* gu, int dtype, int rows, int hidden, void* q_fp8, void* scales_e8m0, mmdit_stream_t stream) {
  MMDIT_CHECK_ARG(gu && q_fp8 && scales_e8m0 && rows > 0 && hidden > 0 && hidden % 64 == 0);
  dim3 grid((hidden + 255) / 256, (rows + CO_RCH - 1) / CO_RCH);
  hipStream_t s = (hipStream_t)stream;
  if (dtype == MMDIT_BF16) hipLaunchKernelGGL((mlp_act_fwd_kernel<bf16_t, false, true>), grid, dim3(256), 0, s, (const bf16_t*)gu, (bf16_t*)q_fp8, rows, hidden, (unsigned char*)scales_e8m0);
  else return MMDIT_ERR_DTYPE;
  return mmdit_launch_status();
}
extern "C" int mmdit_swiglu_fwd(const void* gu, void* h, int dtype, int rows, int hidden, mmdit_stream_t st) { return mlp_act_fwd<false>(gu, h, dtype, rows, hidden, st); }
extern "C" int mmdit_gelu_fwd(const void* u, void* h, int dtype, int rows, int hidden, mmdit_stream_t st) { return mlp_act_fwd<true>(u, h, dtype, rows, hidden, st); }

extern "C" int mmdit_silu_bwd(const void* dy, int dy_dtype, const float* pre, void* dpre, int dpre_dtype, int rows, int cols, float* dbias, int rows_per_bias,
                              mmdit_stream_t stream) {
  MMDIT_CHECK_ARG(dy && pre && dpre && rows > 0 && cols > 0);
  const int rpg = rows_per_bias > 0 ? rows_per_bias : rows;
  MMDIT_CHECK_ARG(rows % rpg == 0);
  hipStream_t s = (hipStream_t)stream;
  dim3 grid((cols + 63) / 64, rows / rpg);
  if (dy_dtype == MMDIT_BF16 && dpre_dtype == MMDIT_BF16) hipLaunchKernelGGL((silu_bwd_kernel<bf16_t, bf16_t>), grid, dim3(256), 0, s, (const bf16_t*)dy, pre, (bf16_t*)dpre, rpg, cols, dbias);
  else if (dy_dtype == MMDIT_F32 && dpre_dtype == MMDIT_F32) hipLaunchKernelGGL((silu_bwd_kernel<float, float>), grid, dim3(256), 0, s, (const float*)dy, pre, (float*)dpre, rpg, cols, dbias);
  else if (dy_dtype == MMDIT_F32 && dpre_dtype == MMDIT_BF16) hipLaunchKernelGGL((silu_bwd_kernel<float, bf16_t>), grid, dim3(256), 0, s, (const float*)dy, pre, (bf16_t*)dpre, rpg, cols, dbias);
  else return MMDIT_ERR_DTYPE;
  return mmdit_launch_status();
}

extern "C" int mmdit_gate_residual_bwd(const float* dy, const void* acc, int acc_dtype, const float* gate, int64_t ld_gate, int rows, int d, int rpb,
                                       void* dacc, int dacc_dtype, float* dgate, int64_t ld_dgate, float* dbias, int64_t ld_dbias, mmdit_stream_t stream) {
  MMDIT_CHECK_ARG(dy && acc && gate && dacc && dgate && rows > 0 && d % 8 == 0 && rpb > 0 && rows % rpb == 0 && ld_gate % 4 == 0);
  hipStream_t s = (hipStream_t)stream;
  const int nchunk = (rpb + GR_RCH - 1) / GR_RCH;
  dim3 grid((d + 255) / 256, (rows / rpb) * nchunk);
  if (acc_dtype == MMDIT_BF16 && dacc_dtype == MMDIT_BF16) hipLaunchKernelGGL((gate_res_bwd_kernel<bf16_t, bf16_t>), grid, dim3(256), 0, s, dy, (const bf16_t*)acc, gate, ld_gate, d, rpb, nchunk, (bf16_t*)dacc, dgate, ld_dgate, dbias, ld_dbias);
  else if (acc_dtype == MMDIT_F32 && dacc_dtype == MMDIT_F32) hipLaunchKernelGGL((gate_res_bwd_kernel<float, float>), grid, dim3(256), 0, s, dy, (const float*)acc, gate, ld_gate, d, rpb, nchunk, (float*)dacc, dgate, ld_dgate, dbias, ld_dbias);
  else return MMDIT_ERR_DTYPE;
  return mmdit_launch_status();
}

namespace {
template <typename T>
__global__ __launch_bounds__(256) void flow_loss_partial_kernel(const float* __restrict__ v, const T* __restrict__ x0, const T* __restrict__ eps, int64_t n8, float coef2,
                                                                float* __restrict__ dv, float* __restrict__ partials) {
  float s = 0.f;
  for (int64_t i = (int64_t)blockIdx.x * 256 + threadIdx.x; i < n8; i += (int64_t)gridDim.x * 256) {
    float a[8], b[8], c[8], g[8];
    ld8(v + i * 8, a);
    ld8(x0 + i * 8, b);
    ld8(eps + i * 8, c);
#pragma unroll
    for (int e = 0; e < 8; e++) {
      float lab = c[e] - b[e];
      if (sizeof(T) == 2) lab = bf2f(f2bf(lab));
      const float d = a[e] - lab;
      s += d * d;
      g[e] = coef2 * d;
    }
    if (dv) st8(dv + i * 8, g);
  }
  __shared__ float sm[4];
  s = wave_sum(s);
  if ((threadIdx.x & 63) == 0) sm[threadIdx.x >> 6] = s;
  __syncthreads();
  if (threadIdx.x == 0) partials[blockIdx.x] = ((sm[0] + sm[1]) + sm[2]) + sm[3];
}
__global__ __launch_bounds__(64) void flow_loss_final_kernel(const float* __restrict__ partials, int count, float coef, float* __restrict__ loss) {
  float s = 0.f;
  for (int i = threadIdx.x; i < count; i += 64) s += partials[i];
  s = wave_sum(s);
  if (threadIdx.x == 0) loss[0] = s * coef;
}
}

extern "C" int mmdit_flow_loss(const float* v, const void* x0, const void* eps, int in_dtype, int64_t n, float coef, float* dv, float* partials,
                               float* loss, mmdit_stream_t stream) {
  MMDIT_CHECK_ARG(v && x0 && eps && partials && loss && n > 0 && n % 8 == 0);
  const int64_t n8 = n / 8;
  const int grid = (int)((n8 + 255) / 256 < 256 ? (n8 + 255) / 256 : 256);
  hipStream_t s = (hipStream_t)stream;
  if (in_dtype == MMDIT_BF16)
    hipLaunchKernelGGL((flow_loss_partial_kernel<bf16_t>), dim3(grid), dim3(256), 0, s, v, (const bf16_t*)x0, (const bf16_t*)eps, n8, 2.f * coef, dv, partials);
  else if (in_dtype == MMDIT_F32)
    hipLaunchKernelGGL((flow_loss_partial_kernel<float>), dim3(grid), dim3(256), 0, s, v, (const float*)x0, (const float*)eps, n8, 2.f * coef, dv, partials);
  else
    return MMDIT_ERR_DTYPE;
  hipLaunchKernelGGL(flow_loss_final_kernel, dim3(1), dim3(64), 0, s, (const float*)partials, grid, coef, loss);
  return mmdit_launch_status();
}

extern "C" int mmdit_colsum(const void* x, int dtype, int rows, int cols, int64_t ld, float* out, mmdit_stream_t stream) {
  MMDIT_CHECK_ARG(x && out && rows > 0 && cols > 0 && cols % 8 == 0 && ld % 8 == 0);
  hipStream_t s = (hipStream_t)stream;
  const int rch = rows <= 256 ? 8 : CO_RCH;
  dim3 grid((cols + 1023) / 1024, (rows + rch - 1) / rch);
  if (dtype == MMDIT_BF16) hipLaunchKernelGGL((colsum_kernel<bf16_t>), grid, dim3(256), 0, s, (const bf16_t*)x, rows, cols, ld, out, rch);
  else if (dtype == MMDIT_F32) hipLaunchKernelGGL((colsum_kernel<float>), grid, dim3(256), 0, s, (const float*)x, rows, cols, ld, out, rch);
  else return MMDIT_ERR_DTYPE;
  return mmdit_launch_status();
}

namespace {
template <typename TI>
__global__ __launch_bounds__(256) void fp8_amax_kernel(const TI* __restrict__ x, int64_t n8, float* __restrict__ amax) {
  float m = 0.f;
  for (int64_t i = (int64_t)blockIdx.x * 256 + threadIdx.x; i < n8; i += (int64_t)gridDim.x * 256) {
    float v[8];
    ld8(x + i * 8, v);
#pragma unroll
    for (int e = 0; e < 8; e++) m = fmaxf(m, fabsf(v[e]));
  }
  __shared__ float sm[4];
  m = wave_max(m);
  if ((threadIdx.x & 63) == 0) sm[threadIdx.x >> 6] = m;
  __syncthreads();
  if (threadIdx.x == 0) atomicMax((unsigned int*)amax, __float_as_uint(fmaxf(fmaxf(sm[0], sm[1]), fmaxf(sm[2], sm[3]))));
}
template <typename TI>
__global__ __launch_bounds__(256) void fp8_quant_kernel(const TI* __restrict__ x, int64_t n8, const float* __restrict__ amax, uint2* __restrict__ q, float* __restrict__ scale) {
  float dq;
  const float s = fp8_range(amax[0], dq);
  if (blockIdx.x == 0 && threadIdx.x == 0) scale[0] = dq;
  for (int64_t i = (int64_t)blockIdx.x * 256 + threadIdx.x; i < n8; i += (int64_t)gridDim.x * 256) {
    float v[8];
    ld8(x + i * 8, v);
    q[i] = fp8_pack8(v, s);
  }
}
template <typename TI>
__global__ __launch_bounds__(256) void fp8_quant_delayed_kernel(const TI* __restrict__ x, int64_t n8, float* __restrict__ state, int phase, float margin,
                                                                uint2* __restrict__ q) {
  __shared__ float sm[4];
  float dq;
  const float s = fp8_range(state[phase % 3] * margin, dq);
  if (blockIdx.x == 0 && threadIdx.x == 0) { state[3] = dq; state[(phase + 2) % 3] = 0.f; }
  float m = 0.f;
  for (int64_t i = (int64_t)blockIdx.x * 256 + threadIdx.x; i < n8; i += (int64_t)gridDim.x * 256) {
    float v[8];
    ld8(x + i * 8, v);
    m = fp8_amax8(m, v);
    q[i] = fp8_pack8(v, s);
  }
  fp8_wg_amax(m, state + (phase + 1) % 3, sm);
}
}

namespace {
template <typename TI>
__global__ __launch_bounds__(256) void mxfp8_quant_kernel(const TI* __restrict__ x, int rows, int K, int64_t ldx, uint4* __restrict__ q, unsigned char* __restrict__ sc) {
  mx_quant_block((int64_t)blockIdx.x * 256 + threadIdx.x, x, rows, K, K, ldx, q, sc);
}
}

extern "C" int mmdit_mxfp8_quantize(const void* x, int x_dtype, int rows, int K, int64_t ldx, void* q_fp8, void* scales, mmdit_stream_t stream) {
  MMDIT_CHECK_ARG(x && q_fp8 && scales && rows > 0 && K > 0 && K % 64 == 0 && ldx >= K && ldx % 8 == 0);
  hipStream_t s = (hipStream_t)stream;
  const int64_t nblk = (int64_t)rows * (K / 32);
  const dim3 grid((unsigned)((nblk + 255) / 256));
  if (x_dtype == MMDIT_F32) hipLaunchKernelGGL((mxfp8_quant_kernel<float>), grid, dim3(256), 0, s, (const float*)x, rows, K, ldx, (uint4*)q_fp8, (unsigned char*)scales);
  else if (x_dtype == MMDIT_BF16) hipLaunchKernelGGL((mxfp8_quant_kernel<bf16_t>), grid, dim3(256), 0, s, (const bf16_t*)x, rows, K, ldx, (uint4*)q_fp8, (unsigned char*)scales);
  else return MMDIT_ERR_DTYPE;
  return mmdit_launch_status();
}

extern "C" int mmdit_fp8_quantize_delayed(const void* x, int x_dtype, int64_t n, float* state, int phase, float margin, void* q_fp8, mmdit_stream_t stream) {
  MMDIT_CHECK_ARG(x && state && q_fp8 && n > 0 && n % 8 == 0 && phase >= 0 && margin >= 1.f);
  hipStream_t s = (hipStream_t)stream;
  const int g0 = grid_cap(n / 8, 256);
  dim3 grid(g0 > 1024 ? 1024 : g0);
  if (x_dtype == MMDIT_F32) hipLaunchKernelGGL((fp8_quant_delayed_kernel<float>), grid, dim3(256), 0, s, (const float*)x, n / 8, state, phase, margin, (uint2*)q_fp8);
  else if (x_dtype == MMDIT_BF16) hipLaunchKernelGGL((fp8_quant_delayed_kernel<bf16_t>), grid, dim3(256), 0, s, (const bf16_t*)x, n / 8, state, phase, margin, (uint2*)q_fp8);
  else return MMDIT_ERR_DTYPE;
  return mmdit_launch_status();
}

extern "C" int mmdit_fp8_amax(const void* x, int x_dtype, int64_t n, float* amax, mmdit_stream_t stream) {
  MMDIT_CHECK_ARG(x && amax && n > 0 && n % 8 == 0);
  hipStream_t s = (hipStream_t)stream;
  const int g0 = grid_cap(n / 8, 256);
  dim3 grid(g0 > 1024 ? 1024 : g0);
  if (x_dtype == MMDIT_F32) hipLaunchKernelGGL((fp8_amax_kernel<float>), grid, dim3(256), 0, s, (const float*)x, n / 8, amax);
  else if (x_dtype == MMDIT_BF16) hipLaunchKernelGGL((fp8_amax_kernel<bf16_t>), grid, dim3(256), 0, s, (const bf16_t*)x, n / 8, amax);
  else return MMDIT_ERR_DTYPE;
  return mmdit_launch_status();
}
extern "C" int mmdit_fp8_quantize(const void* x, int x_dtype, int64_t n, const float* amax, void* q_fp8, float* scale, mmdit_stream_t stream) {
  MMDIT_CHECK_ARG(x && amax && q_fp8 && scale && n > 0 && n % 8 == 0);
  hipStream_t s = (hipStream_t)stream;
  dim3 grid(grid_cap(n / 8, 256));
  if (x_dtype == MMDIT_F32) hipLaunchKernelGGL((fp8_quant_kernel<float>), grid, dim3(256), 0, s, (const float*)x, n / 8, amax, (uint2*)q_fp8, scale);
  else if (x_dtype == MMDIT_BF16) hipLaunchKernelGGL((fp8_quant_kernel<bf16_t>), grid, dim3(256), 0, s, (const bf16_t*)x, n / 8, amax, (uint2*)q_fp8, scale);
  else return MMDIT_ERR_DTYPE;
  return mmdit_launch_status();
}

extern "C" int mmdit_cast(const void* src, int src_dtype, void* dst, int dst_dtype, int64_t n, mmdit_stream_t stream) {
  MMDIT_CHECK_ARG(src && dst && n > 0);
  hipStream_t s = (hipStream_t)stream;
  dim3 grid(grid_cap(n / 8 + 1, 256));
  if (src_dtype == MMDIT_F32 && dst_dtype == MMDIT_BF16) hipLaunchKernelGGL((cast_kernel<float, bf16_t>), grid, dim3(256), 0, s, (const float*)src, (bf16_t*)dst, n);
  else if (src_dtype == MMDIT_BF16 && dst_dtype == MMDIT_F32) hipLaunchKernelGGL((cast_kernel<bf16_t, float>), grid, dim3(256), 0, s, (const bf16_t*)src, (float*)dst, n);
  else return MMDIT_ERR_DTYPE;
  return mmdit_launch_status();
}

template <bool TO_TOKENS>
static int patch_dispatch(const void* src, int sdt, void* dst, int ddt, int batch, int ch, int H, int W, mmdit_stream_t stream) {
  MMDIT_CHECK_ARG(src && dst && batch > 0 && ch > 0 && H > 0 && W > 0 && H % 2 == 0 && W % 2 == 0);
  hipStream_t s = (hipStream_t)stream;
  dim3 grid(grid_cap((int64_t)batch * ch * H * (W / 2), 256));
#define PK(TI, TO) hipLaunchKernelGGL((patch_kernel<TI, TO, TO_TOKENS>), grid, dim3(256), 0, s, (const TI*)src, (TO*)dst, batch, ch, H, W)
  if (sdt == MMDIT_F32 && ddt == MMDIT_F32) PK(float, float);
  else if (sdt == MMDIT_F32 && ddt == MMDIT_BF16) PK(float, bf16_t);
  else if (sdt == MMDIT_BF16 && ddt == MMDIT_BF16) PK(bf16_t, bf16_t);
  else if (sdt == MMDIT_BF16 && ddt == MMDIT_F32) PK(bf16_t, float);
  else return MMDIT_ERR_DTYPE;
#undef PK
  return mmdit_launch_status();
}
extern "C" int mmdit_patchify(const void* img, int img_dtype, int batch, int ch, int H, int W, void* tokens, int tok_dtype, mmdit_stream_t st) {
  return patch_dispatch<true>(img, img_dtype, tokens, tok_dtype, batch, ch, H, W, st);
}
extern "C" int mmdit_unpatchify(const void* tokens, int tok_dtype, int batch, int ch, int H, int W, void* img, int img_dtype, mmdit_stream_t st) {
  return patch_dispatch<false>(tokens, tok_dtype, img, img_dtype, batch, ch, H, W, st);
}

extern "C" int mmdit_time_embed_fwd(const float* t, const float* time_scale, const float* denom, int batch, int dim, void* out, int out_dtype, mmdit_stream_t stream) {
  MMDIT_CHECK_ARG(t && time_scale && denom && out && batch > 0 && dim > 0 && dim % 2 == 0);
  hipStream_t s = (hipStream_t)stream;
  dim3 grid((dim + 255) / 256, batch);
  if (out_dtype == MMDIT_BF16) hipLaunchKernelGGL((time_embed_fwd_kernel<bf16_t>), grid, dim3(256), 0, s, t, time_scale, denom, batch, dim, (bf16_t*)out);
  else if (out_dtype == MMDIT_F32) hipLaunchKernelGGL((time_embed_fwd_kernel<float>), grid, dim3(256), 0, s, t, time_scale, denom, batch, dim, (float*)out);
  else return MMDIT_ERR_DTYPE;
  return mmdit_launch_status();
}
extern "C" int mmdit_time_embed_bwd(const void* dout, int dout_dtype, const float* t, const float* time_scale, const float* denom, int batch, int dim, float* dtime_scale, mmdit_stream_t stream) {
  MMDIT_CHECK_ARG(dout && t && time_scale && denom && dtime_scale && batch > 0 && dim > 0 && dim % 2 == 0);
  hipStream_t s = (hipStream_t)stream;
  if (dout_dtype == MMDIT_BF16) hipLaunchKernelGGL((time_embed_bwd_kernel<bf16_t>), dim3(batch), dim3(256), 0, s, (const bf16_t*)dout, t, time_scale, denom, batch, dim, dtime_scale);
  else if (dout_dtype == MMDIT_F32) hipLaunchKernelGGL((time_embed_bwd_kernel<float>), dim3(batch), dim3(256), 0, s, (const float*)dout, t, time_scale, denom, batch, dim, dtime_scale);
  else return MMDIT_ERR_DTYPE;
  return mmdit_launch_status();
}
```

stable-diffusion-3-from-scratch_amd/engine.py:

```python
from types import SimpleNamespace as NS

import torch

from . import _lib, ops
from ._lib import ACT_SILU, PREC_BF16, PREC_SPLIT

F32 = torch.float32
BF16 = torch.bfloat16


class Mode:
    def __init__(self, fast: bool = True, fp8: bool = False, mx: bool = False):
        self.fast = fast
        self.fp8 = fp8
        self.mx = mx
        self.T = BF16 if fast else F32
        self.prec = PREC_BF16 if fast else PREC_SPLIT
        self.attn_mode = 0 if fast else 1
        self.attn_e4m3 = False
        self._q = {}

    def act(self, t):
        return t if t.dtype == self.T else ops.cast(t, self.T)

# ... 271 lines not shown
    sv.Q = torch.empty((B, H, S, hd // 2 if qk_half else hd), dtype=m.T if cos2 else BF16, device=dev)
    merge = w.kv_merge
    rope3 = w.rope3
    if merge:
        assert N % 2 == 0 and Mt % 2 == 0, "Merge attention requires an even number of keys"
        if m.fp8:
            raise RuntimeError("kv_merge_attn: no fp8 / mxfp8 path")
        if hd != 64:
            raise RuntimeError(f"kv_merge_attn: head width {hd} is not built (the pair-averaging kernels are 64 wide)")
        sv.K, sv.V = torch.empty((B, H, S // 2, 64), dtype=BF16, device=dev), torch.empty((B, H, S // 2, 64), dtype=BF16, device=dev)
    else:
        sv.K, sv.V = torch.empty_like(sv.Q), torch.empty((B, H, S, hd), dtype=sv.Q.dtype, device=dev)
    fused = None
    if not merge and not rope3 and not qk_half and not cos2 and _QKV_FUSE and m.fast and dev.type == "cuda" and m.T == BF16 and (not m.fp8 or mxf) and hd == 64:
        qp = [dict(A=sv.ln1x, B=w.Wqkv_x, out_dtype=m.T, precision=m.prec), dict(A=sv.ln1c, B=w.Wqkv_c, out_dtype=m.T, precision=m.prec)]
        if mxf:
            qq = [_to_fp8(m, p) for p in qp]
            qp = qq if all(x is not p for x, p in zip(qq, qp)) else None
        if qp is not None:
            fused = ops.gemm_qkv_norm_rope(qp, [(w.wq_x, w.wk_x, rope[0], rope[1], N, 0), (w.wq_c, w.wk_c, None, None, Mt, N)], H, S, sv.Q, sv.K, sv.V, raw=_QKV_RAW or not mxf)
    if fused is not None:
        sv.qkv_x, sv.qkv_c = fused
    else:
        sv.qkv_x, sv.qkv_c = _group(m, [dict(A=sv.ln1x, B=w.Wqkv_x, out_dtype=m.T), dict(A=sv.ln1c, B=w.Wqkv_c, out_dtype=m.T)], fp8=True)
    if fused is not None:
        pass
    elif cos2:
        ops.qk_l2norm_rope_fwd_pair((sv.qkv_x, rope[0], rope[1], N, 0), (sv.qkv_c, None, None, Mt, N), B, H, S, sv.Q, sv.K, sv.V)
    elif qk_half:
        ops.qk_norm_rope_fwd_qkhalf_pair((sv.qkv_x, w.wq_x, w.wk_x, rope[0], rope[1], N, 0), (sv.qkv_c, w.wq_c, w.wk_c, None, None, Mt, N), B, H, S, sv.Q, sv.K, sv.V)
    elif rope3:
        ops.qk_norm_rope3_fwd_pair((sv.qkv_x, w.wq_x, w.wk_x, rope[0], rope[1], N, 0), (sv.qkv_c, w.wq_c, w.wk_c, None, None, Mt, N), B, H, S, sv.Q, sv.K, sv.V)
    elif merge:
        ops.qk_norm_rope_fwd_merge_pair((sv.qkv_x, w.wq_x, w.wk_x, rope[0], rope[1], N, 0), (sv.qkv_c, w.wq_c, w.wk_c, None, None, Mt, N), B, H, S, sv.Q, sv.K, sv.V)
    elif _LN_PAIR and dev.type == "cuda":
        ops.qk_norm_rope_fwd_pair((sv.qkv_x, w.wq_x, w.wk_x, rope[0], rope[1], N, 0), (sv.qkv_c, w.wq_c, w.wk_c, None, None, Mt, N), B, H, S, sv.Q, sv.K, sv.V)
    else:
        ops.qk_norm_rope_fwd(sv.qkv_x, w.wq_x, w.wk_x, rope[0], rope[1], B, N, H, S, 0, sv.Q, sv.K, sv.V)
        ops.qk_norm_rope_fwd(sv.qkv_c, w.wq_c, w.wk_c, None, None, B, Mt, H, S, N, sv.Q, sv.K, sv.V)
    if cos2:
        sv.Ox, sv.Oc, sv.den = ops.attn_cos2_fwd(sv.Q, sv.K, sv.V, N)
        sv.Oxa = sv.Ox.view(B * N, d)
        if both:
            sv.Oca = sv.Oc.view(B * Mt, d)
    elif qk_half:
        sv.Ox, sv.Oc, sv.lse = ops.attn_fwd_qkhalf(sv.Q, sv.K, sv.V, N, hd ** -0.5, m.attn_mode)
        sv.Oxa = m.act(sv.Ox.view(B * N, d))
        if both:
            sv.Oca = m.act(sv.Oc.view(B * Mt, d))
    elif mxf:
        sv.Oxa, sv.Oca = ops.attn_fwd_e4m3_mx(sv.Q, sv.K, sv.V, N, 64 ** -0.5, pad=True) if m.attn_e4m3 else ops.attn_fwd_mx(sv.Q, sv.K, sv.V, N, 64 ** -0.5, pad=True)
    elif m.fp8 and m.attn_e4m3 and not keep and not merge and dev.type == "cuda":
        sv.Ox, sv.Oc = ops.attn_fwd_e4m3(sv.Q, sv.K, sv.V, N, 64 ** -0.5)
        sv.Oxa = sv.Ox.view(B * N, d)
        if both:
            sv.Oca = sv.Oc.view(B * Mt, d)
    else:
        sv.Ox, sv.Oc, sv.lse = ops.attn_fwd(sv.Q, sv.K, sv.V, N, hd ** -0.5, m.attn_mode, s_kv=S // 2 if merge else None)
        sv.Oxa = m.act(sv.Ox.view(B * N, d))
        if both:
            sv.Oca = m.act(sv.Oc.view(B * Mt, d))

    probs = [dict(A=sv.Oxa, B=w.Wo_x, out_dtype=m.T)]
    if both:
        probs.append(dict(A=sv.Oca, B=w.Wo_c, out_dtype=m.T))
    outs = _group(m, probs, fp8=True)
    sv.acc_ox = outs[0]
    if both:
        sv.acc_oc = outs[1]
        (sv.X1, sv.ln2x, sv.mu2x, sv.rs2x), (sv.C1, sv.ln2c, sv.mu2c, sv.rs2c) = _norm_pair(
            m, (Pending(sv.X, sv.acc_ox, ms.gate1x, N), ms.scale2x, ms.shift2x, N), (Pending(sv.C, sv.acc_oc, ms.gate1c, Mt), ms.scale2c, ms.shift2c, Mt), mx=mxf)
    else:
        sv.C1 = sv.C
        sv.X1, sv.ln2x, sv.mu2x, sv.rs2x = _norm(m, Pending(sv.X, sv.acc_ox, ms.gate1x, N), ms.scale2x, ms.shift2x, N, mx=mxf)
    fuse = _FUSE_SWIGLU and m.fast and dev.type == "cuda" and not w.mlp_x.gelu and w.mlp_x.hidden % 128 == 0 and (mx_fuse_width(d) if m.fp8 else d % 64 == 0)

    def up(xn, mw, rows):
        if fuse and mxf:
            q, sc = ops._mx_buffers(rows, mw.hidden, dev)
            return dict(A=xn, B=mw.Wup, bias=mw.bup, act=ops.ACT_SWIGLU, out=q, out_scales=sc)
        if fuse:
            return dict(A=xn, B=mw.Wup, bias=mw.bup, act=ops.ACT_SWIGLU, aux=torch.empty((rows, 2 * mw.hidden), dtype=m.T, device=dev) if keep else None)
        return dict(A=xn, B=mw.Wup, bias=mw.bup, out_dtype=m.T)

    probs = [up(sv.ln2x, w.mlp_x, B * N)]
    if both:
        probs.append(up(sv.ln2c, w.mlp_c, B * Mt))
    outs = _group(m, probs, fp8=True)
    pre = [p.get("aux") for p in probs]
    if fuse and mxf:
        outs = [ops.MxAct(p["out"], p["out_scales"]) for p in probs]
    if fuse:
        sv.gu_x, sv.h_x = pre[0], outs[0]
    else:
        sv.gu_x = outs[0]
        sv.h_x = ops.swiglu_fwd_mx(sv.gu_x, w.mlp_x.hidden) if mxf else ops.mlp_act_fwd(sv.gu_x, w.mlp_x.hidden, w.mlp_x.gelu)
    probs = [dict(A=sv.h_x, B=w.mlp_x.Wdown, bias=w.mlp_x.bdown, out_dtype=m.T)]
    if both:
        if fuse:
            sv.gu_c, sv.h_c = pre[1], outs[1]
        else:
            sv.gu_c = outs[1]
            sv.h_c = ops.swiglu_fwd_mx(sv.gu_c, w.mlp_c.hidden) if mxf else ops.mlp_act_fwd(sv.gu_c, w.mlp_c.hidden, w.mlp_c.gelu)
        probs.append(dict(A=sv.h_c, B=w.mlp_c.Wdown, bias=w.mlp_c.bdown, out_dtype=m.T))
    outs = _group(m, probs, fp8=True)
    sv.acc_mx = outs[0]
    X2 = Pending(sv.X1, sv.acc_mx, ms.gate2x, N)
    if both:
        sv.acc_mc = outs[1]
        C2 = Pending(sv.C1, sv.acc_mc, ms.gate2c, Mt)
    else:
        C2 = Pending(sv.C1)
    if not lazy:
        X2, C2 = X2.value(), C2.value()
    return X2, C2, sv


_LN_PAIR = _lib.experiment("MMDIT_LN_PAIR", "1") != "0"
_MX_FUSE = _lib.experiment("MMDIT_MX_FUSE", "1") != "0"
_BATCH_WMOD = _lib.experiment("MMDIT_BATCH_WMOD", "1") != "0"
_QKV_FUSE = _lib.experiment("MMDIT_QKV_FUSE", "1") != "0"
_QKV_RAW = _lib.experiment("MMDIT_QKV_RAW", "0") == "1"
_QK_FUSE = _lib.experiment("MMDIT_ATTN_QK_FUSE", "1") != "0"
_FUSE_SWIGLU_BWD = _lib.experiment("MMDIT_FUSE_SWIGLU_BWD", "1") != "0"
_FUSE_GATE = _lib.experiment("MMDIT_FUSE_GATE", "1") != "0"


def _qk_bwd_two_pass(m, w, sv, g, dOx, dOc, dims, rope, dev):
    B, N, Mt, H, d = dims
    S = N + Mt
    if getattr(w, "cos2", False):
        dQ, dK, dV = ops.attn_cos2_bwd(sv.Q, sv.K, sv.V, sv.Ox, sv.Oc, dOx, dOc, sv.den, N, m.T)
        return ops.qk_l2norm_rope_bwd_pair(dQ, dK, dV, (sv.qkv_x, rope[0], rope[1], N, 0), (sv.qkv_c, None, None, Mt, N), B, H, S, m.T)
    if getattr(w, "qk_half", False):
        dQ, dK, dV = ops.attn_bwd_qkhalf(sv.Q, sv.K, sv.V, sv.Ox, sv.Oc, dOx, dOc, sv.lse, N, w.hd ** -0.5, m.T)
        return ops.qk_norm_rope_bwd_qkhalf_pair(dQ, dK, dV, (sv.qkv_x, w.wq_x, w.wk_x, rope[0], rope[1], N, 0, g.wq_x, g.wk_x),
                                                (sv.qkv_c, w.wq_c, w.wk_c, None, None, Mt, N, g.wq_c, g.wk_c), B, H, S, m.T)
    if w.kv_merge:
        dQ, dK, dV = ops.attn_bwd(sv.Q, sv.K, sv.V, sv.Ox, sv.Oc, dOx, dOc, sv.lse, N, w.hd ** -0.5, m.T, s_kv=S // 2)
        return ops.qk_norm_rope_bwd_merge_pair(dQ, dK, dV, (sv.qkv_x, w.wq_x, w.wk_x, rope[0], rope[1], N, 0, g.wq_x, g.wk_x),
                                               (sv.qkv_c, w.wq_c, w.wk_c, None, None, Mt, N, g.wq_c, g.wk_c), B, H, S, m.T)
    dQ, dK, dV = ops.attn_bwd(sv.Q, sv.K, sv.V, sv.Ox, sv.Oc, dOx, dOc, sv.lse, N, w.hd ** -0.5, m.T)
    if w.rope3:
        return ops.qk_norm_rope3_bwd_pair(dQ, dK, dV, (sv.qkv_x, w.wq_x, w.wk_x, rope[0], rope[1], N, 0, g.wq_x, g.wk_x),
                                          (sv.qkv_c, w.wq_c, w.wk_c, None, None, Mt, N, g.wq_c, g.wk_c), B, H, S, m.T)
    if _LN_PAIR and dev.type == "cuda":
        return ops.qk_norm_rope_bwd_pair(dQ, dK, dV, (sv.qkv_x, w.wq_x, w.wk_x, rope[0], rope[1], N, 0, g.wq_x, g.wk_x),
                                         (sv.qkv_c, w.wq_c, w.wk_c, None, None, Mt, N, g.wq_c, g.wk_c), B, H, S, m.T)
    dqkv_x = ops.qk_norm_rope_bwd(dQ, dK, dV, sv.qkv_x, w.wq_x, w.wk_x, rope[0], rope[1], B, N, H, S, 0, g.wq_x, g.wk_x, m.T)
    dqkv_c = ops.qk_norm_rope_bwd(dQ, dK, dV, sv.qkv_c, w.wq_c, w.wk_c, None, None, B, Mt, H, S, N, g.wq_c, g.wk_c, m.T)
    return dqkv_x, dqkv_c


def block_bwd_begin(m, w, sv, dims, dev, defer_cond=False):
    B, N, Mt, H, d = dims
    both = not w.last
    ms = _mod_views(sv.mod, d, w.last)
    g = NS(mlp_x=NS(), mlp_c=NS() if both else None)
    hx = sv.gu_x.shape[1]
    nb = 2 if both else 1
    nw = w.hd // 2 if getattr(w, "qk_half", False) else w.hd
    cos2 = getattr(w, "cos2", False)
    shapes = [(nb * d,), (hx,)] + ([] if cos2 else [(nw,), (nw,), (nw,), (nw,)]) + ([(sv.gu_c.shape[1],)] if both else []) + ([] if defer_cond else [(d,)])
    npar = len(shapes)
    shapes += [tuple(sv.mod.shape), (B, nb * d)]
    zs, small_arena = _zeros_views(shapes, dev, prefix=npar)
    st = NS(g=g, ms=ms, zs=zs, npar=npar, small_arena=small_arena, both=both)
    st.bdown, g.mlp_x.bup = zs[:2]
    if not cos2:
        g.wq_x, g.wk_x, g.wq_c, g.wk_c = zs[2:6]
    if not defer_cond:
        g.by = zs[npar - 1]
    st.dmod, st.bpart = zs[npar], zs[npar + 1]
    g.mlp_x.bdown = st.bdown[:d]
    if both:
        g.mlp_c.bdown, g.mlp_c.bup = st.bdown[d:], zs[2 if cos2 else 6]
    st.dms = _mod_views(st.dmod, d, w.last)
    st.req_x = (sv.acc_mx, ms.gate2x, st.dms.gate2x, st.bpart[:, :d])
    st.req_c = (sv.acc_mc, ms.gate2c, st.dms.gate2c, st.bpart[:, d:]) if both else None
    return st


def block_bwd(m, w, sv, dX2, dC2, dy_acc, dims, rope, defer_cond=False, st=None, dacc=None, nxt=None, defer_wmod=False):
    B, N, Mt, H, d = dims
    S, dev = N + Mt, dX2.device
    both = not w.last
    if st is None:
        st = block_bwd_begin(m, w, sv, dims, dev, defer_cond)
    g, ms, dms, bpart, bdown, dmod = st.g, st.ms, st.dms, st.bpart, st.bdown, st.dmod
    pending = []
    fuse = _FUSE_GATE

    def defer(ns, name, dY, Xa):
        pending.append((lambda o, ns=ns, name=name: setattr(ns, name, o), _wg(dY, Xa)))

    dacc_x = dacc[0] if dacc is not None else ops.gate_residual_bwd(dX2, sv.acc_mx, ms.gate2x, N, dms.gate2x, bpart[:, :d], m.T)
    probs = [dict(A=dacc_x, B=w.mlp_x.Wdown, b_kmajor=True, out_dtype=m.T)]
    if both:
        dacc_c = dacc[1] if dacc is not None else ops.gate_residual_bwd(dC2, sv.acc_mc, ms.gate2c, Mt, dms.gate2c, bpart[:, d:], m.T)
        probs.append(dict(A=dacc_c, B=w.mlp_c.Wdown, b_kmajor=True, out_dtype=m.T))
    ops.colsum(bpart, bdown)
    dgu = None
    if (_FUSE_SWIGLU_BWD and m.fast and dev.type == "cuda" and m.prec == PREC_BF16 and dacc_x.dtype == BF16 and sv.gu_x.dtype == BF16
            and not w.mlp_x.gelu and (not both or not w.mlp_c.gelu)):
        fp = [dict(A=dacc_x, B=w.mlp_x.Wdown, aux=sv.gu_x, dbias=g.mlp_x.bup, precision=m.prec)]
        if both:
            fp.append(dict(A=dacc_c, B=w.mlp_c.Wdown, aux=sv.gu_c, dbias=g.mlp_c.bup, precision=m.prec))
        dgu = ops.gemm_swiglu_bwd(fp)
    if dgu is None:
        dh = _group(m, probs)
    defer(g.mlp_x, "Wdown", dacc_x, sv.h_x)
    pair = both and _LN_PAIR and dev.type == "cuda" and w.mlp_x.hidden == w.mlp_c.hidden and w.mlp_x.gelu == w.mlp_c.gelu
    if dgu is not None:
        dgu_x, dgu_c = dgu[0], (dgu[1] if both else None)
    elif pair:
        dgu_x, dgu_c = ops.mlp_act_bwd_pair((dh[0], sv.gu_x, g.mlp_x.bup), (dh[1], sv.gu_c, g.mlp_c.bup), w.mlp_x.hidden, w.mlp_x.gelu)
    else:
        dgu_x = ops.mlp_act_bwd(dh[0], sv.gu_x, w.mlp_x.hidden, g.mlp_x.bup, w.mlp_x.gelu)
    probs = [dict(A=dgu_x, B=w.mlp_x.Wup, b_kmajor=True, out_dtype=m.T)]
    defer(g.mlp_x, "Wup", dgu_x, sv.ln2x)
    if both:
        defer(g.mlp_c, "Wdown", dacc_c, sv.h_c)
        if not pair and dgu is None:
            dgu_c = ops.mlp_act_bwd(dh[1], sv.gu_c, w.mlp_c.hidden, g.mlp_c.bup, w.mlp_c.gelu)
        probs.append(dict(A=dgu_c, B=w.mlp_c.Wup, b_kmajor=True, out_dtype=m.T))
        defer(g.mlp_c, "Wup", dgu_c, sv.ln2c)
    dln2 = _group(m, probs)

    ax = dict(dout=dln2[0], x=sv.X1, mean=sv.mu2x, rstd=sv.rs2x, scale=ms.scale2x, dres=dX2, rpb=N, dscale=dms.scale2x, dshift=dms.shift2x)
    if fuse:
        ax["gated"] = (sv.acc_ox, ms.gate1x, dms.gate1x, None)
    dC1 = dC2
    if both:
        ac = dict(dout=dln2[1], x=sv.C1, mean=sv.mu2c, rstd=sv.rs2c, scale=ms.scale2c, dres=dC2, rpb=Mt, dscale=dms.scale2c, dshift=dms.shift2c)
        if fuse:
            ac["gated"] = (sv.acc_oc, ms.gate1c, dms.gate1c, None)
        rx, rc = _ln_bwd_pair(ax, ac)
    else:
        rx = ops.ln_modulate_bwd(ax["dout"], ax["x"], ax["mean"], ax["rstd"], ax["scale"], ax["dres"], N, ax["dscale"], ax["dshift"], gated=ax.get("gated"))
    if fuse:
        dX1, dacc_x = rx
    else:
        dX1 = rx
        dacc_x = ops.gate_residual_bwd(dX1, sv.acc_ox, ms.gate1x, N, dms.gate1x, None, m.T)
    oT = m.T if getattr(w, "cos2", False) else BF16
    probs = [dict(A=dacc_x, B=w.Wo_x, b_kmajor=True, out_dtype=oT)]
    defer(g, "Wo_x", dacc_x, sv.Oxa)
    if both:
        if fuse:
            dC1, dacc_c = rc
        else:
            dC1 = rc
            dacc_c = ops.gate_residual_bwd(dC1, sv.acc_oc, ms.gate1c, Mt, dms.gate1c, None, m.T)
        probs.append(dict(A=dacc_c, B=w.Wo_c, b_kmajor=True, out_dtype=oT))
        defer(g, "Wo_c", dacc_c, sv.Oca)
    dO = _group(m, probs)
    dOx, dOc = dO[0], (dO[1] if both else None)

    if not w.kv_merge and not w.rope3 and not getattr(w, "qk_half", False) and not getattr(w, "cos2", False) and _QK_FUSE and m.fast and dev.type == "cuda" and ops.attn_bwd_qk_ok(sv.Q, N, sv.qkv_x) and g.wq_x.data_ptr() + 768 == g.wk_c.data_ptr():
        dqkv_x, dqkv_c = ops.attn_bwd_qk(sv.Q, sv.K, sv.V, sv.Ox, sv.Oc, dOx, dOc, sv.lse, N, 64 ** -0.5, sv.qkv_x, sv.qkv_c, w.wq_x, w.wk_x, w.wq_c, w.wk_c,
                                         rope[0], rope[1], torch.as_strided(g.wq_x, (256,), (1,)))
    else:
        dqkv_x, dqkv_c = _qk_bwd_two_pass(m, w, sv, g, dOx, dOc, dims, rope, dev)
    dln1 = _group(m, [dict(A=dqkv_x, B=w.Wqkv_x, b_kmajor=True, out_dtype=m.T), dict(A=dqkv_c, B=w.Wqkv_c, b_kmajor=True, out_dtype=m.T)])
    defer(g, "Wqkv_x", dqkv_x, sv.ln1x)
    defer(g, "Wqkv_c", dqkv_c, sv.ln1c)
    nacc = None
    ax = dict(dout=dln1[0], x=sv.X, mean=sv.mu1x, rstd=sv.rs1x, scale=ms.scale1x, dres=dX1, rpb=N, dscale=dms.scale1x, dshift=dms.shift1x)
    ac = dict(dout=dln1[1], x=sv.C, mean=sv.mu1c, rstd=sv.rs1c, scale=ms.scale1c, dres=dC1, rpb=Mt, dscale=dms.scale1c, dshift=dms.shift1c)
    if nxt is not None and fuse:
        ax["gated"], ac["gated"] = nxt.req_x, nxt.req_c
        (dX, nax), (dC, nac) = _ln_bwd_pair(ax, ac)
        nacc = (nax, nac)
    else:
        dX, dC = _ln_bwd_pair(ax, ac)

    dmod_a = m.act(dmod)
    if defer_cond:
        if not defer_wmod:
            defer(g, "Wmod", dmod_a, sv.yp)
        dy_acc = dmod_a
    else:
        defer(g, "Wmod", dmod_a, sv.yp)
        dyp = _dgrad(m, dmod_a, w.Wmod, F32, **({"split_k": 16} if m.fast else {}))
        dpre = ops.silu_bwd(dyp, sv.pre, m.T, g.by)
        dy_acc = _dgrad(m, dpre, w.Wy, F32, residual=dy_acc)
        defer(g, "Wy", dpre, sv.y)

    wg_arena = _wgrad_flush(m, pending)
    g.arenas = [wg_arena, st.small_arena] if wg_arena is not None else None
    if nxt is not None:
        return dX, dC, dy_acc, g, nacc
    return dX, dC, dy_acc, g


def text_fwd(m, W, c):
    B, Mt = c.shape[0], c.shape[1]
    d = W.dim
    cn1, cn2 = ops.text_rmsnorm_fwd(c, W.wn1, W.wn2, W.s1, W.s2, W.split, m.T)
    c1, c2 = _group(m, [dict(A=cn1, B=W.Wc1, out_dtype=F32), dict(A=cn2, B=W.Wc2, out_dtype=F32)])
    C = torch.cat([c1.view(B, W.split, d), c2.view(B, Mt - W.split, d)], dim=1).view(B * Mt, d)
    return C, cn1, cn2


def model_fwd(m, W, x_t, t, c, c_pooled, rope, keep=True, C=None, text_head=True):
    B, Cin, Hh, Ww = x_t.shape
    d, H = W.dim, W.heads
    N, Mt = (Hh // 2) * (Ww // 2), c.shape[1]
    dims = (B, N, Mt, H, d)
    sv = NS(dims=dims, img=(B, Cin, Hh, Ww), c=c, t=t)
    sv.pe = ops.time_embed_fwd(t, W.time_scale, W.denom, m.T)
    temb = _gemm(m, sv.pe, W.Wt, out_dtype=F32)
    sv.cp = m.act(c_pooled)
    sv.y = _gemm(m, sv.cp, W.Wcond, residual=temb, out_dtype=m.T)

    if C is None:
        C, sv.cn1, sv.cn2 = text_fwd(m, W, c)

    sv.patches = ops.patchify(x_t, m.T)
    sv.X0 = _gemm(m, sv.patches, W.Wpatch, out_dtype=m.T)
    X = _gemm(m, sv.X0, W.Wpe, bias=W.bpe, out_dtype=F32)

    sv.blocks = []
    conds, sv.pre_all = cond_fwd_all(m, W.blocks, sv.y)
    for wb, cond in zip(W.blocks, conds):
        X, C, bs = block_fwd(m, wb, X, C, sv.y, dims, rope, cond, keep, lazy=True)
        sv.blocks.append(bs)

    sv.modo = _gemm(m, sv.y, W.Wmod_out, out_dtype=F32)
    sv.Xf, sv.lnf, sv.muf, sv.rsf = _norm(m, X, sv.modo[:, d:], sv.modo[:, :d], N)
    Z = _gemm(m, sv.lnf, W.Wout, bias=W.bout, out_dtype=F32)
    v = ops.unpatchify(Z, B, Cin, Hh, Ww, F32)
    sv.txt = None
    if getattr(W, "Wtxt", None) is not None and text_head:
        sv.Cfa = m.act(C.value() if isinstance(C, Pending) else C)
        sv.txt = _gemm(m, sv.Cfa, W.Wtxt, bias=W.btxt, out_dtype=F32)
    return v, sv


def _grad_tensors(g):
    out = []
    for v in vars(g).values():
        if isinstance(v, NS):
            out += _grad_tensors(v)
        elif torch.is_tensor(v):
            out.append(v)
    return out


def _set_grad_tensors(g, new, pos=0):
    for k, v in list(vars(g).items()):
        if isinstance(v, NS):
            pos = _set_grad_tensors(v, new, pos)
        elif torch.is_tensor(v):
            setattr(g, k, new[pos])
            pos += 1
    return pos


def model_bwd(m, W, sv, dv, rope, on_grads=None, dtxt=None):
    B, N, Mt, H, d = sv.dims
    _, Cin, Hh, Ww = sv.img
    dev = dv.device
    if dev.type == "cuda":
        ops.zero_pool_begin(dev)
    g = NS()
    pending = []

    def defer(name, dY, Xa):
        pending.append((lambda o, name=name: setattr(g, name, o), _wg(dY, Xa)))

    dZ = ops.patchify(dv.contiguous(), m.T)
    g.bout = ops.zeros(W.Wout.shape[0], dev)
    ops.colsum(dZ, g.bout)
    dlnf = _dgrad(m, dZ, W.Wout, m.T)
    defer("Wout", dZ, sv.lnf)
    dmodo = ops.zeros(sv.modo.shape, dev) if sv.modo.dtype == F32 else torch.zeros_like(sv.modo)
    nblk = len(W.blocks)
    sts = [None] * nblk
    sts[nblk - 1] = block_bwd_begin(m, W.blocks[-1], sv.blocks[-1], sv.dims, dev, defer_cond=True)
    dacc = None
    if _FUSE_GATE:
        dX, dax = ops.ln_modulate_bwd(dlnf, sv.Xf, sv.muf, sv.rsf, sv.modo[:, d:], None, N, dmodo[:, d:], dmodo[:, :d], gated=sts[-1].req_x)
        dacc = (dax, None)
    else:
        dX = ops.ln_modulate_bwd(dlnf, sv.Xf, sv.muf, sv.rsf, sv.modo[:, d:], None, N, dmodo[:, d:], dmodo[:, :d])
    dmodo_a = m.act(dmodo)
    dy_acc = _dgrad(m, dmodo_a, W.Wmod_out, F32, **({"split_k": 4} if m.fast else {}))
    defer("Wmod_out", dmodo_a, sv.y)

    dC = None
    if getattr(W, "Wtxt", None) is not None:
        if sv.txt is None:
            raise RuntimeError("model_bwd: the forward ran with text_head=False (nothing was saved for the text head's backward)")
        rows_t = B * Mt
        if dtxt is None:
            dtxt_a = torch.zeros((rows_t, W.Wtxt.shape[0]), dtype=m.T, device=dev)
        else:
            dtxt = dtxt.reshape(rows_t, W.Wtxt.shape[0])
            if not dtxt.is_contiguous():
                dtxt = dtxt.contiguous()
            dtxt_a = m.act(dtxt)
        g.btxt = ops.zeros(W.Wtxt.shape[0], dev)
        ops.colsum(dtxt_a if dtxt is None else dtxt, g.btxt)
        dC = _dgrad(m, dtxt_a, W.Wtxt, F32)
        defer("Wtxt", dtxt_a, sv.Cfa)
        if _FUSE_GATE:
            acc_mc, gate2c, dgate2c, bpart_c = sts[-1].req_c
            dacc = (dacc[0], ops.gate_residual_bwd(dC, acc_mc, gate2c, Mt, dgate2c, bpart_c, m.T))
    g.blocks = [None] * nblk
    dmods = [None] * nblk
    yps = [None] * nblk
    batch_wmod = on_grads is None and _BATCH_WMOD
    for i in range(nblk - 1, -1, -1):
        if i > 0:
            sts[i - 1] = block_bwd_begin(m, W.blocks[i - 1], sv.blocks[i - 1], sv.dims, dev, defer_cond=True)
            dX, dC, dmods[i], g.blocks[i], dacc = block_bwd(m, W.blocks[i], sv.blocks[i], dX, dC, None, sv.dims, rope, defer_cond=True,
                                                            st=sts[i], dacc=dacc, nxt=sts[i - 1], defer_wmod=batch_wmod)
        else:
            dX, dC, dmods[i], g.blocks[i] = block_bwd(m, W.blocks[i], sv.blocks[i], dX, dC, None, sv.dims, rope, defer_cond=True, st=sts[i], dacc=dacc,
                                                      defer_wmod=batch_wmod)
        sts[i] = None
        yps[i] = sv.blocks[i].yp
        sv.blocks[i] = None
        if on_grads is not None:
            repl = on_grads(_grad_tensors(g.blocks[i]), _wg_streams.get(dev), g.blocks[i].arenas)
            if repl is not None:
                _set_grad_tensors(g.blocks[i], repl)

    dyp_all = ops.zeros((nblk * B, d), dev)
    by_all = ops.zeros((nblk, d), dev)
    for i0 in range(0, nblk, 12):
        _group(m, [dict(A=dmods[i], B=W.blocks[i].Wmod, b_kmajor=True, out=dyp_all[i * B:(i + 1) * B], **({"split_k": 4} if m.fast else {}))
                   for i in range(i0, min(nblk, i0 + 12))])
    dpre_all = ops.silu_bwd(dyp_all, sv.pre_all, m.T, by_all, rows_per_bias=B)
    dyc = torch.empty((nblk + 1, B, d), dtype=F32, device=dev)
    dyc[nblk].copy_(dy_acc)
    for i0 in range(0, nblk, 12):
        _group(m, [dict(A=dpre_all[i * B:(i + 1) * B], B=W.blocks[i].Wy, b_kmajor=True, out=dyc[i]) for i in range(i0, min(nblk, i0 + 12))])
    dy_acc = dyc.sum(0)
    late = []
    for i in range(nblk):
        g.blocks[i].by = by_all[i]
        pending.append((lambda o, i=i: setattr(g.blocks[i], "Wy", o), _wg(dpre_all[i * B:(i + 1) * B], sv.y)))
        late += [(i, "by"), (i, "Wy")]
        if batch_wmod:
            pending.append((lambda o, i=i: setattr(g.blocks[i], "Wmod", o), _wg(dmods[i], yps[i])))

    g.bpe = ops.zeros(d, dev)
    ops.colsum(dX, g.bpe)
    dX_a = m.act(dX)
    dX0 = _dgrad(m, dX_a, W.Wpe, m.T)
    defer("Wpe", dX_a, sv.X0)
    defer("Wpatch", dX0, sv.patches)

    dCv = dC.view(B, Mt, d)
    dc1 = m.act(dCv[:, :W.split].reshape(B * W.split, d))
    dc2 = m.act(dCv[:, W.split:].reshape(B * (Mt - W.split), d))
    dcn1, dcn2 = _group(m, [dict(A=dc1, B=W.Wc1, b_kmajor=True, out_dtype=m.T), dict(A=dc2, B=W.Wc2, b_kmajor=True, out_dtype=m.T)])
    defer("Wc1", dc1, sv.cn1)
    defer("Wc2", dc2, sv.cn2)
    g.wn1, g.wn2, g.s1, g.s2 = ops.text_rmsnorm_bwd(dcn1, dcn2, sv.c, W.wn1, W.wn2, W.s1, W.s2, W.split)

    dy_a = m.act(dy_acc)
    defer("Wcond", dy_a, sv.cp)
    dpe = _dgrad(m, dy_a, W.Wt, m.T)
    defer("Wt", dy_a, sv.pe)
    g.time_scale = ops.time_embed_bwd(dpe, sv.t, W.time_scale, W.denom)
    _wgrad_flush(m, pending)
    if on_grads is not None:
        keys = [k for k, v in vars(g).items() if torch.is_tensor(v)]
        repl = on_grads([getattr(g, k) for k in keys] + [getattr(g.blocks[i], n) for i, n in late], _wg_streams.get(dev))
        if repl is not None:
            for k, t in zip(keys, repl):
                setattr(g, k, t)
            for (i, n), t in zip(late, repl[len(keys):]):
                setattr(g.blocks[i], n, t)
    wgrad_join(dev)
    return g
```

stable-diffusion-3-from-scratch_amd/ops.py:

```python
import ctypes
import os

import torch

from . import _lib
from ._lib import ACT_NONE, ACT_SILU, ACT_SWIGLU, ACT_SWIGLU_BWD, BF16, F32, FP8, PREC_BF16, PREC_SPLIT, GemmArgs, check

_DT = {torch.float32: F32, torch.bfloat16: BF16, torch.float8_e4m3fn: FP8}

PROFILE = None
_ZERO_ALL = _lib.experiment("MMDIT_ZERO_ALL", "0") == "1"


class _ZeroPool:

    def __init__(self):
        self.buf, self.off, self.cap, self.need = None, 0, 0, 0

    def begin(self, device):
        self.cap = max(self.cap, self.need)
        self.need, self.off = 0, 0
        self.buf = torch.zeros(self.cap, dtype=torch.float32, device=device) if self.cap else None

    def take(self, numel, device):
# ... 364 lines not shown

def attn_fwd_e4m3(Q, K, V, n_img, scale, mx=False):
    B, H, S, n_txt, D = _attn_e4m3_operands(Q, K, V, n_img)
    if mx:
        qx, sx = _mx_buffers(B * n_img, D, Q.device)
        qc, scc = _mx_buffers(B * n_txt, D, Q.device) if n_txt else (None, None)
        check(_lib.lib().mmdit_attn_fwd_e4m3(_p(Q), _p(K), _p(V), B, H, S, n_img, float(scale), _p(qx), _p(qc), _p(sx), _p(scc), _s()), "mmdit_attn_fwd_e4m3")
        return MxAct(qx, sx), (MxAct(qc, scc) if n_txt else None)
    Ox = torch.empty((B, n_img, D), dtype=torch.bfloat16, device=Q.device)
    Oc = torch.empty((B, n_txt, D), dtype=torch.bfloat16, device=Q.device) if n_txt else None
    check(_lib.lib().mmdit_attn_fwd_e4m3(_p(Q), _p(K), _p(V), B, H, S, n_img, float(scale), _p(Ox), _p(Oc), None, None, _s()), "mmdit_attn_fwd_e4m3")
    return Ox, Oc


def attn_fwd_e4m3_mx(Q, K, V, n_img, scale, pad=False):
    B, H, S, n_txt, D = _attn_e4m3_operands(Q, K, V, n_img)
    if not (pad and D % 128 == 64):
        return attn_fwd_e4m3(Q, K, V, n_img, scale, mx=True)
    qx, sx = _mx_buffers(B * n_img, fp8_k_pad(D), Q.device)
    qc, scc = _mx_buffers(B * n_txt, fp8_k_pad(D), Q.device) if n_txt else (None, None)
    check(_lib.lib().mmdit_attn_fwd_e4m3_mx_pad(_p(Q), _p(K), _p(V), B, H, S, n_img, float(scale), _p(qx), _p(qc), _p(sx), _p(scc), _s()), "mmdit_attn_fwd_e4m3_mx_pad")
    return MxAct(qx, sx), (MxAct(qc, scc) if n_txt else None)


def quant_mxfp8(x, pad=False):
    rows, K = x.shape
    if _pads(x, pad):
        Kp = fp8_k_pad(K)
        q, sc = _mx_buffers(rows, Kp, x.device)
        check(_lib.lib().mmdit_mxfp8_quantize_pad(_p(x), _dt(x), rows, K, x.stride(0), _p(q), _p(sc), _s()), "mmdit_mxfp8_quantize_pad")
        return q, sc
    q = torch.empty((rows, K), dtype=torch.float8_e4m3fn, device=x.device)
    sc = torch.empty(mx_scale_bytes(rows, K), dtype=torch.uint8, device=x.device)
    check(_lib.lib().mmdit_mxfp8_quantize(_p(x), _dt(x), rows, K, x.stride(0), _p(q), _p(sc), _s()), "mmdit_mxfp8_quantize")
    return q, sc


class Fp8Site:

    def __init__(self, margin=1.5):
        self.state, self.phase, self.margin = None, 0, margin

    def quantise(self, x, pad=False):
        L = _lib.lib()
        if self.state is None:
            self.state = torch.zeros(4, dtype=torch.float32, device=x.device)
            check(L.mmdit_fp8_amax(_p(_c(x)), _dt(x), x.numel(), _p(self.state), _s()), "mmdit_fp8_amax")
        margin = float(self.margin if self.phase else 1.0)
        if _pads(x, pad):
            rows, K = x.shape
            q = torch.empty((rows, fp8_k_pad(K)), dtype=torch.float8_e4m3fn, device=x.device)
            check(L.mmdit_fp8_quantize_delayed_pad(_p(_c(x)), _dt(x), rows, K, K, _p(self.state), self.phase, margin, _p(q), _s()), "mmdit_fp8_quantize_delayed_pad")
            self.phase += 1
            return q, self.state[3:]
        q = torch.empty(x.shape, dtype=torch.float8_e4m3fn, device=x.device)
        check(L.mmdit_fp8_quantize_delayed(_p(_c(x)), _dt(x), x.numel(), _p(self.state), self.phase, margin,
                                           _p(q), _s()), "mmdit_fp8_quantize_delayed")
        self.phase += 1
        return q, self.state[3:]


def cast(src, dtype, out=None):
    if out is None:
        out = torch.empty(src.shape, dtype=dtype, device=src.device)
    check(_lib.lib().mmdit_cast(_p(_c(src)), _dt(src), _p(_c(out)), _dt(out), src.numel(), _s()), "mmdit_cast")
    return out


_CAST_TABLES = {}


def cast_multi(pairs):
    import numpy as np
    dev = pairs[0][0].device
    key = tuple((s.data_ptr(), d.data_ptr(), s.numel()) for s, d in pairs)
    t = _CAST_TABLES.get(key)
    if t is None:
        for s, d in pairs:
            if s.dtype != torch.float32 or d.dtype != torch.bfloat16 or not s.is_contiguous() or not d.is_contiguous() or s.numel() != d.numel() or d.device != dev:
                raise RuntimeError("cast_multi: contiguous fp32 sources and bf16 destinations of equal size on one device")
        rec = np.array(key, dtype=np.int64).reshape(-1)
        ct = np.concatenate([np.full((n + _lib.ADAMW_CHUNK - 1) // _lib.ADAMW_CHUNK, i, dtype=np.int32) for i, (_, _, n) in enumerate(key)])
        co = np.concatenate([np.arange(0, n, _lib.ADAMW_CHUNK, dtype=np.int64) for _, _, n in key])
        host = [torch.from_numpy(a).pin_memory() for a in (rec, ct, co)]
        if len(_CAST_TABLES) >= 8:
            _CAST_TABLES.pop(next(iter(_CAST_TABLES)))
        t = _CAST_TABLES[key] = dict(host=host, dev=[h.to(dev, non_blocking=True) for h in host], n=len(ct))
    check(_lib.lib().mmdit_cast_multi(_p(t["dev"][0]), _p(t["dev"][1]), _p(t["dev"][2]), t["n"], _s()), "mmdit_cast_multi")


def _ln_fwd(plist, out_dtype, mx=False, pad=False):
    res = plist[0].get("acc") is not None
    d = plist[0]["x"].shape[1]
    if mx and d % 128 and not (pad and d % 128 == 64):
        raise RuntimeError(f"adaLN with MX output over a problem list: d = {d} needs pad=True and d % 64 == 0 (the e4m3 GEMM's 128-wide K tile)")
    probs, outs, keep = (_lib.LnFwdProblem * len(plist))(), [], []
    for q, p in zip(probs, plist):
        assert (p.get("acc") is not None) == res
        x = _c(p["x"])
        rows, dev = x.shape[0], x.device
        x1 = torch.empty((rows, d), dtype=torch.float32, device=dev) if res else x
        out = MxAct(*_mx_buffers(rows, fp8_k_pad(d), dev)) if mx else torch.empty((rows, d), dtype=out_dtype, device=dev)
        mean = torch.empty((rows,), dtype=torch.float32, device=dev)
        rstd = torch.empty((rows,), dtype=torch.float32, device=dev)
        q.x, q.scale, q.shift, q.ld_mod, q.rows, q.rows_per_batch = _p(x), _p(p["scale"]), _p(p["shift"]), p["scale"].stride(0), rows, p["rpb"]
        q.out, q.mean, q.rstd = _p(out.q if mx else out), _p(mean), _p(rstd)
        keep.append(x)
        if res:
            acc = _c(p["acc"])
            q.acc, q.gate, q.ld_gate, q.x_out = _p(acc), _p(p["gate"]), p["gate"].stride(0), _p(x1)
            keep.append(acc)
        outs.append((x1, out, mean, rstd))
    if mx:
        check(_lib.lib().mmdit_ln_modulate_fwd_mx_pad(probs, len(plist), d, _dt(plist[0]["acc"]) if res else BF16, _p(outs[0][1].sc), _p(outs[-1][1].sc) if len(outs) > 1 else None,
                                                      _s()), "mmdit_ln_modulate_fwd_mx_pad")
        return outs
    acc_dt = _dt(plist[0]["acc"]) if res else _DT[out_dtype]
    check(_lib.lib().mmdit_ln_modulate_fwd(probs, len(plist), d, acc_dt, _DT[out_dtype], _s()), "mmdit_ln_modulate_fwd")
    return outs


def ln_modulate_fwd(x, scale, shift, rows_per_batch, out_dtype):
    return _ln_fwd([dict(x=x, scale=scale, shift=shift, rpb=rows_per_batch)], out_dtype)[0][1:]


def ln_modulate_fwd_res(x, acc, gate, scale, shift, rows_per_batch, out_dtype):
    return _ln_fwd([dict(x=x, scale=scale, shift=shift, rpb=rows_per_batch, acc=acc, gate=gate)], out_dtype)[0]


def ln_modulate_fwd_pair(pa, pb, out_dtype, mx=False, pad=False):
    return _ln_fwd([pa, pb], out_dtype, mx=mx, pad=pad)


def _ln_bwd(plist):
    gated = plist[0].get("gated") is not None
    d = plist[0]["x"].shape[1]
    probs, outs, keep = (_lib.LnBwdProblem * len(plist))(), [], []
    for q, p in zip(probs, plist):
        assert (p.get("gated") is not None) == gated
        dout, x = _c(p["dout"]), p["x"]
        rows, dev = x.shape[0], x.device
        dx = torch.empty((rows, d), dtype=torch.float32, device=dev)
        q.dout, q.x, q.mean, q.rstd, q.scale, q.ld_mod = _p(dout), _p(x), _p(p["mean"]), _p(p["rstd"]), _p(p["scale"]), p["scale"].stride(0)
        q.dres, q.rows, q.rows_per_batch = _p(p.get("dres")), rows, p["rpb"]
        q.dx, q.dscale, q.dshift, q.ld_dmod = _p(dx), _p(p["dscale"]), _p(p["dshift"]), p["dscale"].stride(0)
        keep.append(dout)
        if gated:
            acc, gate, dgate, dbias = p["gated"]
            acc = _c(acc)
            if acc.dtype != dout.dtype:
                raise RuntimeError(f"ln_modulate_bwd: acc ({acc.dtype}) and dout ({dout.dtype}) must have one dtype")
            dacc = torch.empty((rows, d), dtype=acc.dtype, device=dev)
            q.acc, q.gate, q.ld_gate, q.dacc, q.dgate, q.ld_dgate = _p(acc), _p(gate), gate.stride(0), _p(dacc), _p(dgate), dgate.stride(0)
            q.dbias, q.ld_dbias = _p(dbias), (dbias.stride(0) if dbias is not None else 0)
            keep.append(acc)
            outs.append((dx, dacc))
        else:
            outs.append(dx)
    check(_lib.lib().mmdit_ln_modulate_bwd(probs, len(plist), d, _dt(plist[0]["dout"]), _s()), "mmdit_ln_modulate_bwd")
    return outs


def ln_modulate_bwd_pair(pa, pb):
    return _ln_bwd([pa, pb])


def gate_residual_fwd(x, acc, gate, rows_per_batch):
    rows, d = x.shape
    out = torch.empty((rows, d), dtype=torch.float32, device=x.device)
    check(_lib.lib().mmdit_gate_residual_fwd(_p(_c(x)), _p(_c(acc)), _dt(acc), _p(gate), gate.stride(0), rows, d, rows_per_batch, _p(out), _s()), "mmdit_gate_residual_fwd")
    return out


def ln_modulate_bwd(dout, x, mean, rstd, scale, dres, rows_per_batch, dscale, dshift, gated=None):
    p = dict(dout=dout, x=x, mean=mean, rstd=rstd, scale=scale, dres=dres, rpb=rows_per_batch, dscale=dscale, dshift=dshift)
    if gated is not None:
        p["gated"] = gated
    return _ln_bwd([p])[0]


def text_rmsnorm_fwd(x, w1, w2, s1, s2, split, out_dtype):
    batch, tokens, d = x.shape
    out1 = torch.empty((batch * split, d), dtype=out_dtype, device=x.device)
    out2 = torch.empty((batch * (tokens - split), d), dtype=out_dtype, device=x.device)
    check(_lib.lib().mmdit_text_rmsnorm_fwd(_p(_c(x)), _dt(x), _p(w1), _p(w2), _p(s1), _p(s2), batch, tokens, split, d,
                                            _p(out1), _p(out2), _dt(out1), _s()), "mmdit_text_rmsnorm_fwd")
    return out1, out2


def text_rmsnorm_bwd(dout1, dout2, x, w1, w2, s1, s2, split):
    batch, tokens, d = x.shape
    dw1, dw2 = zeros(w1.shape, w1.device), zeros(w2.shape, w2.device)
    ds1, ds2 = zeros(s1.shape, s1.device), zeros(s2.shape, s2.device)
    check(_lib.lib().mmdit_text_rmsnorm_bwd(_p(_c(dout1)), _p(_c(dout2)), _dt(dout1), _p(x), _dt(x), _p(w1), _p(w2), _p(s1), _p(s2),
                                            batch, tokens, split, d, _p(dw1), _p(dw2), _p(ds1), _p(ds2), _s()), "mmdit_text_rmsnorm_bwd")
    return dw1, dw2, ds1, ds2


def _head_dim(t, what="attention"):
    hd = t.shape[-1]
    if hd not in _lib.HEAD_DIMS:
        raise RuntimeError(f"{what} kernels are built for head_dim 64 (the reference's dim = 64*num_heads convention) and 128, got {hd}")
    return hd


def _qk_hd128(fn, streams, heads, bwd):
    if fn not in ("mmdit_qk_norm_rope_fwd", "mmdit_qk_norm_rope_bwd"):
        raise RuntimeError(f"{fn}: built for head_dim 64 only")
    if heads > _lib.QK_HD128_MAX_HEADS:
        raise RuntimeError(f"{fn}_hd128: at most {_lib.QK_HD128_MAX_HEADS} heads (a qkv row is one workgroup of 48 * heads threads), got {heads}")
    for st in streams:
        if st[0].shape[-1] != 3 * heads * 128 or st[1].numel() != 128 or st[2].numel() != 128 or (st[3] is not None and st[3].shape[-1] != 128):
            raise RuntimeError(f"{fn}_hd128: qkv rows are 3 * heads * 128 wide, norm weights 128, RoPE tables (tokens, 128); got {tuple(st[0].shape)}, "
                               f"{st[1].numel()}, {st[2].numel()}, {None if st[3] is None else tuple(st[3].shape)}")
        if bwd and (st[7].numel() != 128 or st[8].numel() != 128):
            raise RuntimeError(f"{fn}_hd128: dwq / dwk are 128 floats")
    return fn + "_hd128"


def _qk(fn, streams, batch, heads, s_total, T3, out_dtype=None, status=check):
    probs, outs = (_lib.QkProblem * len(streams))(), []
    for q, st in zip(probs, streams):
        qkv, wq, wk, rc, rs, tokens, tok0 = st[:7]
        q.qkv, q.wq, q.wk, q.rope_cos, q.rope_sin, q.tokens, q.tok0 = _p(_c(qkv)), _p(wq), _p(wk), _p(rc), _p(rs), tokens, tok0
        if out_dtype is not None:
            dqkv = torch.empty(qkv.shape, dtype=out_dtype, device=qkv.device)
            q.dqkv, q.dwq, q.dwk = _p(dqkv), _p(st[7]), _p(st[8])
            outs.append(dqkv)
    a, b, c = (_p(t) for t in T3)
    if _head_dim(T3[0], "QK-norm / RoPE") == 128:
        fn = _qk_hd128(fn, streams, heads, out_dtype is not None)
    launch, qkv_dt = getattr(_lib.lib(), fn), _dt(streams[0][0])
    if out_dtype is None:
        status(launch(probs, len(streams), qkv_dt, batch, heads, s_total, a, b, c, _s()), fn)
    else:
        status(launch(probs, len(streams), a, b, c, _dt(T3[0]), qkv_dt, _DT[out_dtype], batch, heads, s_total, _s()), fn)
    return outs


def qk_norm_rope_fwd(qkv, wq, wk, rope_cos, rope_sin, batch, tokens, heads, s_total, tok0, Q, K, V):
    _qk("mmdit_qk_norm_rope_fwd", [(qkv, wq, wk, rope_cos, rope_sin, tokens, tok0)], batch, heads, s_total, (Q, K, V))


def qk_norm_rope_bwd(dQ, dK, dV, qkv, wq, wk, rope_cos, rope_sin, batch, tokens, heads, s_total, tok0, dwq, dwk, out_dtype):
    return _qk("mmdit_qk_norm_rope_bwd", [(qkv, wq, wk, rope_cos, rope_sin, tokens, tok0, dwq, dwk)], batch, heads, s_total, (dQ, dK, dV), out_dtype)[0]


def qk_norm_rope_fwd_pair(img, txt, batch, heads, s_total, Q, K, V):
    _qk("mmdit_qk_norm_rope_fwd", [img, txt], batch, heads, s_total, (Q, K, V))


def qk_norm_rope_bwd_pair(dQ, dK, dV, img, txt, batch, heads, s_total, out_dtype):
    return _qk("mmdit_qk_norm_rope_bwd", [img, txt], batch, heads, s_total, (dQ, dK, dV), out_dtype)


def _qk_rope3(fn, streams, batch, heads, s_total, T3, out_dtype=None):
    hd = _head_dim(T3[0], "QK-norm / RoPE2dV2")
    bwd = out_dtype is not None
    for t in T3:
        if tuple(t.shape) != (batch, heads, s_total, hd) or t.dtype != T3[0].dtype or (not bwd and t.dtype != torch.bfloat16):
            raise RuntimeError(f"{fn}: {'dQ / dK / dV' if bwd else 'Q / K / V (bfloat16)'} are (batch, heads, s_total, head_dim) = {(batch, heads, s_total, hd)} of one dtype, "
                               f"got {t.dtype} {tuple(t.shape)}")
        _c(t)
    probs, outs = (_lib.QkProblem * len(streams))(), []
    for q, st in zip(probs, streams):
        qkv, wq, wk, rc, rs, tokens, tok0 = st[:7]
        if qkv.dim() != 2 or tuple(qkv.shape) != (batch * tokens, 3 * heads * hd) or wq.numel() != hd or wk.numel() != hd:
            raise RuntimeError(f"{fn}: qkv rows are (batch * tokens, 3 * heads * {hd}) = {(batch * tokens, 3 * heads * hd)}, norm weights {hd} wide; got {tuple(qkv.shape)}, "
                               f"{wq.numel()}, {wk.numel()}")
        if (rc is None) != (rs is None):
            raise RuntimeError(f"{fn}: the cos and the sin table come together (or neither: the text stream)")
        for tb in (rc, rs):
            if tb is not None and (tuple(tb.shape) != (tokens, 2 * (hd // 3)) or tb.dtype != torch.float32):
                raise RuntimeError(f"{fn}: the RoPE2dV2 tables are fp32 (tokens, 2 * (head_dim // 3)) = {(tokens, 2 * (hd // 3))}, got {tb.dtype} {tuple(tb.shape)}")
            if tb is not None:
                _c(tb)
        if tokens < 1 or tok0 < 0 or tok0 + tokens > s_total:
            raise RuntimeError(f"{fn}: tokens [{tok0}, {tok0 + tokens}) are outside the joint sequence of {s_total}")
        if wq.dtype != torch.float32 or wk.dtype != torch.float32:
            raise RuntimeError(f"{fn}: the norm weights are fp32")
        q.qkv, q.wq, q.wk, q.rope_cos, q.rope_sin, q.tokens, q.tok0 = _p(_c(qkv)), _p(_c(wq)), _p(_c(wk)), _p(rc), _p(rs), tokens, tok0
        if bwd:
            if any(t.numel() != hd or t.dtype != torch.float32 for t in st[7:9]):
                raise RuntimeError(f"{fn}: dwq / dwk are {hd} fp32 values")
            dqkv = torch.empty(qkv.shape, dtype=out_dtype, device=qkv.device)
            q.dqkv, q.dwq, q.dwk = _p(dqkv), _p(_c(st[7])), _p(_c(st[8]))
            outs.append(dqkv)
    if any(st[0].dtype != streams[0][0].dtype for st in streams):
        raise RuntimeError(f"{fn}: the streams of one launch share the qkv dtype")
    a, b, c = (_p(t) for t in T3)
    launch, qkv_dt = getattr(_lib.lib(), fn), _dt(streams[0][0])
    if not bwd:
        check(launch(probs, len(streams), qkv_dt, batch, heads, hd, s_total, a, b, c, _s()), fn)
    else:
        check(launch(probs, len(streams), a, b, c, _dt(T3[0]), qkv_dt, _DT[out_dtype], batch, heads, hd, s_total, _s()), fn)
    return outs


def qk_norm_rope3_fwd(qkv, wq, wk, rope_cos, rope_sin, batch, tokens, heads, s_total, tok0, Q, K, V):
    _qk_rope3("mmdit_qk_norm_rope3_fwd", [(qkv, wq, wk, rope_cos, rope_sin, tokens, tok0)], batch, heads, s_total, (Q, K, V))


def qk_norm_rope3_bwd(dQ, dK, dV, qkv, wq, wk, rope_cos, rope_sin, batch, tokens, heads, s_total, tok0, dwq, dwk, out_dtype):
    return _qk_rope3("mmdit_qk_norm_rope3_bwd", [(qkv, wq, wk, rope_cos, rope_sin, tokens, tok0, dwq, dwk)], batch, heads, s_total, (dQ, dK, dV), out_dtype)[0]


def qk_norm_rope3_fwd_pair(img, txt, batch, heads, s_total, Q, K, V):
# ... 263 lines not shown
            raise RuntimeError(f"attention operands are bfloat16 of one shape (batch, heads, S, head_dim), got {t.dtype} {tuple(t.shape)}")
        _c(t)


def attn_fwd(Q, K, V, n_img, scale, mode, s_kv=None):
    batch, heads, S, hd = Q.shape
    _head_dim(Q)
    D = heads * hd
    Ox = torch.empty((batch, n_img, D), dtype=torch.bfloat16, device=Q.device)
    Oc = torch.empty((batch, S - n_img, D), dtype=torch.bfloat16, device=Q.device) if S > n_img else None
    lse = torch.empty((batch, heads, S), dtype=torch.float32, device=Q.device)
    if s_kv is not None:
        _kv_operands(Q, K, V, s_kv)
        check(_lib.lib().mmdit_attn_fwd_kv(_p(Q), _p(K), _p(V), batch, heads, S, int(s_kv), n_img, float(scale), mode, _p(Ox), _p(Oc), _p(lse), _s()), "mmdit_attn_fwd_kv")
        return Ox, Oc, lse
    if hd == 128:
        _plain_operands(Q, K, V)
        check(_lib.lib().mmdit_attn_fwd_hd128(_p(Q), _p(K), _p(V), batch, heads, S, n_img, float(scale), mode, _p(Ox), _p(Oc), _p(lse), _s()), "mmdit_attn_fwd_hd128")
        return Ox, Oc, lse
    check(_lib.lib().mmdit_attn_fwd(_p(Q), _p(K), _p(V), batch, heads, S, n_img, float(scale), mode, _p(Ox), _p(Oc), _p(lse), _s()), "mmdit_attn_fwd")
    return Ox, Oc, lse


def attn_bwd(Q, K, V, Ox, Oc, dOx, dOc, lse, n_img, scale, out_dtype, s_kv=None):
    batch, heads, S, hd = Q.shape
    _head_dim(Q)
    delta = torch.empty((batch, heads, S), dtype=torch.float32, device=Q.device)
    dQ = torch.empty(Q.shape, dtype=out_dtype, device=Q.device)
    if s_kv is not None:
        _kv_operands(Q, K, V, s_kv)
        dK = torch.empty(K.shape, dtype=out_dtype, device=Q.device)
        dV = torch.empty(K.shape, dtype=out_dtype, device=Q.device)
        check(_lib.lib().mmdit_attn_bwd_kv(_p(Q), _p(K), _p(V), _p(_c(Ox)), _p(_c(Oc)), _p(_c(dOx)), _p(_c(dOc)), _p(_c(lse)), _p(delta), batch, heads, S, int(s_kv),
                                           n_img, float(scale), _p(dQ), _p(dK), _p(dV), _dt(dQ), _s()), "mmdit_attn_bwd_kv")
        return dQ, dK, dV
    dK = torch.empty(Q.shape, dtype=out_dtype, device=Q.device)
    dV = torch.empty(Q.shape, dtype=out_dtype, device=Q.device)
    if hd == 128:
        _plain_operands(Q, K, V)
        check(_lib.lib().mmdit_attn_bwd_hd128(_p(Q), _p(K), _p(V), _p(_c(Ox)), _p(_c(Oc)), _p(_c(dOx)), _p(_c(dOc)), _p(_c(lse)), _p(delta), batch, heads, S, n_img,
                                              float(scale), _p(dQ), _p(dK), _p(dV), _dt(dQ), _s()), "mmdit_attn_bwd_hd128")
        return dQ, dK, dV
    check(_lib.lib().mmdit_attn_bwd(_p(Q), _p(K), _p(V), _p(Ox), _p(Oc), _p(_c(dOx)), _p(_c(dOc)), _p(lse), _p(delta), batch, heads, S, n_img,
                                    float(scale), _p(dQ), _p(dK), _p(dV), _dt(dQ), _s()), "mmdit_attn_bwd")
    return dQ, dK, dV


def attn_bwd_qk(Q, K, V, Ox, Oc, dOx, dOc, lse, n_img, scale, qkv_x, qkv_c, wq_x, wk_x, wq_c, wk_c, rope_cos, rope_sin, dw4):
    batch, heads, S, hd = Q.shape
    delta = torch.empty((batch, heads, S), dtype=torch.float32, device=Q.device)
    dqkv_x = torch.empty(qkv_x.shape, dtype=torch.bfloat16, device=Q.device)
    dqkv_c = torch.empty(qkv_c.shape, dtype=torch.bfloat16, device=Q.device)
    if dw4.dtype != torch.float32 or dw4.numel() != 256 or not dw4.is_contiguous():
        raise RuntimeError("attn_bwd_qk: dw4 is the contiguous fp32 [wq_x | wk_x | wq_c | wk_c] accumulator (256)")
    check(_lib.lib().mmdit_attn_bwd_qk(_p(Q), _p(K), _p(V), _p(Ox), _p(Oc), _p(_c(dOx)), _p(_c(dOc)), _p(lse), _p(delta), batch, heads, S, n_img, float(scale),
                                       _p(_c(qkv_x)), _p(_c(qkv_c)), _p(wq_x), _p(wk_x), _p(wq_c), _p(wk_c), _p(rope_cos), _p(rope_sin),
                                       _p(dqkv_x), _p(dqkv_c), _p(dw4), _s()), "mmdit_attn_bwd_qk")
    return dqkv_x, dqkv_c


def attn_bwd_qk_ok(Q, n_img, qkv_x):
    return Q.is_cuda and Q.shape[-1] == 64 and n_img % 32 == 0 and n_img < Q.shape[2] and qkv_x.dtype == torch.bfloat16


def mlp_act_fwd(gu, hidden, gelu=False):
    rows = gu.shape[0]
    h = torch.empty((rows, hidden), dtype=gu.dtype, device=gu.device)
    fn = _lib.lib().mmdit_gelu_fwd if gelu else _lib.lib().mmdit_swiglu_fwd
    check(fn(_p(_c(gu)), _p(h), _dt(gu), rows, hidden, _s()), "mmdit_mlp_act_fwd")
    return h


def _mlp_bwd(plist, hidden, gelu):
    probs, outs, keep = (_lib.MlpBwdProblem * len(plist))(), [], []
    for q, (dh, gu, dbias) in zip(probs, plist):
        dh = _c(dh)
        dgu = torch.empty_like(gu)
        q.dh, q.gu, q.dgu, q.rows, q.dbias = _p(dh), _p(gu), _p(dgu), gu.shape[0], _p(dbias)
        keep.append(dh)
        outs.append(dgu)
    check(_lib.lib().mmdit_mlp_act_bwd(probs, len(plist), _dt(plist[0][1]), hidden, int(gelu), _s()), "mmdit_mlp_act_bwd")
    return outs


def mlp_act_bwd(dh, gu, hidden, dbias, gelu=False):
    return _mlp_bwd([(dh, gu, dbias)], hidden, gelu)[0]


def mlp_act_bwd_pair(a, b, hidden, gelu=False):
    return _mlp_bwd([a, b], hidden, gelu)


def silu_bwd(dy, pre, out_dtype, dbias, rows_per_bias=0):
    rows, cols = pre.shape
    dpre = torch.empty((rows, cols), dtype=out_dtype, device=pre.device)
    check(_lib.lib().mmdit_silu_bwd(_p(_c(dy)), _dt(dy), _p(pre), _p(dpre), _dt(dpre), rows, cols, _p(dbias), int(rows_per_bias), _s()), "mmdit_silu_bwd")
    return dpre


def gate_residual_bwd(dy, acc, gate, rows_per_batch, dgate, dbias, out_dtype):
    rows, d = dy.shape
    dacc = torch.empty((rows, d), dtype=out_dtype, device=dy.device)
    ld_dbias = dbias.stride(0) if (dbias is not None and dbias.dim() == 2) else 0
    check(_lib.lib().mmdit_gate_residual_bwd(_p(_c(dy)), _p(acc), _dt(acc), _p(gate), gate.stride(0), rows, d, rows_per_batch,
                                             _p(dacc), _dt(dacc), _p(dgate), dgate.stride(0), _p(dbias), ld_dbias, _s()), "mmdit_gate_residual_bwd")
    return dacc


def flow_loss(v, x0, eps, accumulation_steps=1, need_grad=True):
    n = v.numel()
    if v.dtype != torch.float32 or x0.dtype != eps.dtype or x0.numel() != n or eps.numel() != n or n % 8:
        raise RuntimeError("flow_loss: v fp32, x0 and eps of one dtype and v's size, numel % 8 == 0")
    loss = torch.empty((), dtype=torch.float32, device=v.device)
    part = torch.empty(256, dtype=torch.float32, device=v.device)
    dv = torch.empty(v.shape, dtype=torch.float32, device=v.device) if need_grad else None
    check(_lib.lib().mmdit_flow_loss(_p(_c(v)), _p(_c(x0)), _p(_c(eps)), _dt(x0), n, 1.0 / (n * accumulation_steps), _p(dv), _p(part), _p(loss), _s()), "mmdit_flow_loss")
    return loss, dv


def text_loss(pred, label, mask, coef, grad_dtype=None):
    if pred.dim() < 2 or label.shape != pred.shape:
        raise RuntimeError(f"text_loss: pred and label must have one shape (..., cols), got {tuple(pred.shape)} and {tuple(label.shape)}")
    cols = pred.shape[-1]
    rows = pred.numel() // max(cols, 1)
    if mask.dtype != torch.bool or mask.numel() != rows or tuple(mask.shape) != tuple(pred.shape[:-1]):
        raise RuntimeError(f"text_loss: mask must be a torch.bool tensor of shape {tuple(pred.shape[:-1])} (one entry per row), got {mask.dtype} {tuple(mask.shape)}")
    if rows < 1 or cols < 8 or cols % 8:
        raise RuntimeError(f"text_loss: needs at least one row and cols % 8 == 0 (16-byte loads), got rows={rows}, cols={cols}")
    for t, what in ((pred, "pred"), (label, "label")):
        if t.dtype not in (torch.float32, torch.bfloat16):
            raise RuntimeError(f"text_loss: {what} must be float32 or bfloat16, got {t.dtype}")
    if grad_dtype not in (None, torch.float32, torch.bfloat16):
        raise RuntimeError(f"text_loss: grad_dtype must be None, float32 or bfloat16, got {grad_dtype}")
    if pred.device != label.device or pred.device != mask.device:
        raise RuntimeError("text_loss: pred, label and mask must live on one device")
    pred, label, mask = _c(pred), _c(label), _c(mask)
    if pred.data_ptr() % 16 or label.data_ptr() % 16:
        raise RuntimeError("text_loss: pred and label must be 16-byte aligned")
    _p(pred), _p(label), _p(mask)
    loss = torch.empty((), dtype=torch.float32, device=pred.device)
    part = torch.empty(_lib.TEXT_LOSS_MAX_PARTIALS, dtype=torch.float32, device=pred.device)
    dpred = torch.empty(pred.shape, dtype=grad_dtype, device=pred.device) if grad_dtype is not None else None
    check(_lib.lib().mmdit_text_loss(_p(pred), _dt(pred), _p(label), _dt(label), _p(mask), rows, cols, float(coef), _p(dpred), _dt(dpred) if dpred is not None else F32,
                                     _p(part), _p(loss), _s()), "mmdit_text_loss")
    return loss, dpred


def colsum(x, out):
    rows, cols = x.shape
    check(_lib.lib().mmdit_colsum(_p(x), _dt(x), rows, cols, x.stride(0), _p(out), _s()), "mmdit_colsum")
    return out


def patchify(img, out_dtype):
    batch, ch, H, W = img.shape
    tokens = torch.empty((batch * (H // 2) * (W // 2), ch * 4), dtype=out_dtype, device=img.device)
    check(_lib.lib().mmdit_patchify(_p(_c(img)), _dt(img), batch, ch, H, W, _p(tokens), _dt(tokens), _s()), "mmdit_patchify")
    return tokens


def unpatchify(tokens, batch, ch, H, W, out_dtype):
    img = torch.empty((batch, ch, H, W), dtype=out_dtype, device=tokens.device)
    check(_lib.lib().mmdit_unpatchify(_p(_c(tokens)), _dt(tokens), batch, ch, H, W, _p(img), _dt(img), _s()), "mmdit_unpatchify")
    return img


def time_embed_fwd(t, time_scale, denom, out_dtype):
    batch, dim = t.shape[0], denom.shape[0]
    out = torch.empty((batch, dim), dtype=out_dtype, device=t.device)
    check(_lib.lib().mmdit_time_embed_fwd(_p(t), _p(time_scale), _p(denom), batch, dim, _p(out), _dt(out), _s()), "mmdit_time_embed_fwd")
    return out


def time_embed_bwd(dout, t, time_scale, denom):
    batch, dim = t.shape[0], denom.shape[0]
    dts = zeros(time_scale.shape, time_scale.device)
    check(_lib.lib().mmdit_time_embed_bwd(_p(_c(dout)), _dt(dout), _p(t), _p(time_scale), _p(denom), batch, dim, _p(dts), _s()), "mmdit_time_embed_bwd")
    return dts


def vae_nchw_to_nhwc(x, c_padded, scale=1.0, shift=0.0):
    B, C, H, W = x.shape
    out = torch.empty((B, H, W, c_padded), dtype=torch.bfloat16, device=x.device)
    check(_lib.lib().mmdit_vae_nchw_to_nhwc(_p(_c(x)), _dt(x), B, C, H, W, c_padded, float(scale), float(shift), _p(out), _s()), "mmdit_vae_nchw_to_nhwc")
    return out


def vae_nhwc_to_nchw(x2d, B, C, H, W, lo=-float("inf"), hi=float("inf")):
    out = torch.empty((B, C, H, W), dtype=torch.float32, device=x2d.device)
    check(_lib.lib().mmdit_vae_nhwc_to_nchw(_p(_c(x2d)), B, C, H, W, x2d.shape[1], float(lo), float(hi), _p(out), _s()), "mmdit_vae_nhwc_to_nchw")
    return out


def vae_im2col3x3(x, mode=0):
    B, H, W, C = x.shape
    Ho, Wo = (H // 2, W // 2) if mode == 1 else (2 * H, 2 * W) if mode == 2 else (H, W)
    out = torch.empty((B * Ho * Wo, 9 * C), dtype=torch.bfloat16, device=x.device)
    check(_lib.lib().mmdit_vae_im2col3x3(_p(_c(x)), B, H, W, C, mode, _p(out), _s()), "mmdit_vae_im2col3x3")
    return out, Ho, Wo


def vae_groupnorm(x, gamma, beta, B, H, W, groups, eps, silu, padded_out=None):
    C = x.shape[1]
    sums = torch.zeros(B * groups * 2, dtype=torch.float32, device=x.device)
    out = padded_out if padded_out is not None else torch.empty((B * H * W, C), dtype=torch.bfloat16, device=x.device)
    check(_lib.lib().mmdit_vae_groupnorm(_p(_c(x)), _dt(x), _p(gamma), _p(beta), B, H, W, C, groups, float(eps), int(silu), _p(sums), _p(out),
                                         int(padded_out is not None), _s()), "mmdit_vae_groupnorm")
    return out


def vae_pad_cast(x, B, H, W, padded_out, upsample=False):
    check(_lib.lib().mmdit_vae_pad_cast(_p(_c(x)), _dt(x), B, H, W, x.shape[1], int(upsample), _p(padded_out), _s()), "mmdit_vae_pad_cast")
    return padded_out


def vae_softmax_rows(x, scale, cols=None):
    rows, ld = x.shape
    cols = ld if cols is None else cols
    out = torch.empty((rows, ld), dtype=torch.bfloat16, device=x.device)
    check(_lib.lib().mmdit_vae_softmax_rows(_p(_c(x)), rows, cols, ld, float(scale), _p(out), _s()), "mmdit_vae_softmax_rows")
    return out


def _rows_ld(t, C, what):
    if not t.is_cuda:
        raise RuntimeError("mmdit HIP op called with a CPU tensor: the MMDiT hot path has no CPU fallback")
    if t.dtype != torch.bfloat16 or t.dim() != 2 or t.shape[1] != C:
        raise RuntimeError(f"{what} must be a bf16 (rows, {C}) tensor")
    if t.stride(1) != 1 or t.stride(0) < C or t.stride(0) % 8 or t.data_ptr() % 16:
        raise RuntimeError(f"{what} must be contiguous or a 16-byte aligned column slice of a contiguous matrix")
    return t.stride(0)


def vae_attention(q, k, v, batch, tokens, scale):
    C = q.shape[1]
    ld = _rows_ld(q, C, "q")
    if _rows_ld(k, C, "k") != ld or _rows_ld(v, C, "v") != ld:
        raise RuntimeError("q, k and v must share one row pitch")
    if not (q.shape[0] == k.shape[0] == v.shape[0] == batch * tokens):
        raise RuntimeError(f"q, k and v need batch * tokens = {batch * tokens} rows")
    out = torch.empty((batch * tokens, C), dtype=torch.bfloat16, device=q.device)
    check(_lib.lib().mmdit_vae_attn_fwd(_p(q), _p(k), _p(v), ld, batch, tokens, C, float(scale), _p(out), _s()), "mmdit_vae_attn_fwd")
    return out
```

Before: 2363.

## Fuse colsum with bf16 cast, batch dmod activation, retune text RMS backward

Adds a tall colsum kernel that splits rows over many workgroups, with an optional fused fp32-to-bf16 cast, and uses it for the patch-embedding bias gradient and for colsums over more than 256 rows. Per-block dmod buffers are carved from one shared arena so the activation cast runs once over all blocks instead of once per block. The gate-bias partial buffer and its separate colsum are dropped; gate residual backward now accumulates straight into the down-projection bias. The text RMSNorm backward kernel picks rows per workgroup adaptively, caches weights in shared memory and loads two rows at a time. These cut kernel launches and memory passes but depend on atomics and on the changed dbias stride handling being correct.

```diff
diff --git a/include/mmdit_hip_tail.h b/include/mmdit_hip_tail.h
--- /dev/null
+++ b/include/mmdit_hip_tail.h
@@ -0,0 +1,16 @@
+#ifndef MMDIT_HIP_TAIL_H
+#define MMDIT_HIP_TAIL_H
+
+#include "mmdit_hip.h"
+
+#ifdef __cplusplus
+extern "C" {
+#endif
+
+int mmdit_colsum_cast(const float* x, int rows, int cols, int64_t ld, void* y_bf16, float* out, mmdit_stream_t stream);
+
+#ifdef __cplusplus
+}
+#endif
+
+#endif
diff --git a/stable-diffusion-3-from-scratch_amd/_lib.py b/stable-diffusion-3-from-scratch_amd/_lib.py
--- a/stable-diffusion-3-from-scratch_amd/_lib.py
+++ b/stable-diffusion-3-from-scratch_amd/_lib.py
@@ -18,6 +18,7 @@
 HEADER_FP8PAD_PATH = os.path.join(_HERE, "..", "include", "mmdit_hip_fp8pad.h")
 HEADER_MXPAD_PATH = os.path.join(_HERE, "..", "include", "mmdit_hip_mxpad.h")
 HEADER_OPTIM_PATH = os.path.join(_HERE, "..", "include", "mmdit_hip_optim.h")
+HEADER_TAIL_PATH = os.path.join(_HERE, "..", "include", "mmdit_hip_tail.h")
 
 F32, BF16 = 0, 1
 ACT_NONE, ACT_SILU, ACT_SWIGLU, ACT_SWIGLU_BWD = 0, 1, 2, 3
@@ -185,6 +186,9 @@
 _OPTIM_SIGNATURES = {
     "mmdit_adamw_step_dlr_pt": _SIGNATURES["mmdit_adamw_step_dlr"],
 }
+_TAIL_SIGNATURES = {
+    "mmdit_colsum_cast": ([_vp, _i, _i, _i64, _vp, _vp, _vp], _i),
+}
 COS2_HEAD_DIM = 64
 ATTN_COS2_TOKEN_CHUNK, ATTN_COS2_ROW_TILE = 128, 64
 HEAD_DIMS = (64, 128)
@@ -252,6 +256,12 @@
 
 def declared_optim_symbols():
     with open(HEADER_OPTIM_PATH) as f:
+        txt = f.read()
+    return sorted(set(re.findall(r"\b(mmdit_[a-z0-9_]+)\s*\(", txt)) - {"mmdit_stream_t"})
+
+
+def declared_tail_symbols():
+    with open(HEADER_TAIL_PATH) as f:
         txt = f.read()
     return sorted(set(re.findall(r"\b(mmdit_[a-z0-9_]+)\s*\(", txt)) - {"mmdit_stream_t"})
 
@@ -272,7 +282,7 @@
         L = ctypes.CDLL(LIB_PATH)
         for name, (argtypes, restype) in (list(_SIGNATURES.items()) + list(_EXT_SIGNATURES.items()) + list(_HD128_SIGNATURES.items()) + list(_ROPE3_SIGNATURES.items())
                                           + list(_QKHALF_SIGNATURES.items()) + list(_TEXTLOSS_SIGNATURES.items()) + list(_COS2_SIGNATURES.items()) + list(_FP8PAD_SIGNATURES.items()) + list(_MXPAD_SIGNATURES.items())
-                                          + list(_OPTIM_SIGNATURES.items())):
+                                          + list(_OPTIM_SIGNATURES.items()) + list(_TAIL_SIGNATURES.items())):
             fn = getattr(L, name)
             fn.argtypes = argtypes
             fn.restype = restype
diff --git a/stable-diffusion-3-from-scratch_amd/build.py b/stable-diffusion-3-from-scratch_amd/build.py
--- a/stable-diffusion-3-from-scratch_amd/build.py
+++ b/stable-diffusion-3-from-scratch_amd/build.py
@@ -17,6 +17,7 @@
 HEADER_FP8PAD = os.path.join(HERE, "..", "include", "mmdit_hip_fp8pad.h")
 HEADER_MXPAD = os.path.join(HERE, "..", "include", "mmdit_hip_mxpad.h")
 HEADER_OPTIM = os.path.join(HERE, "..", "include", "mmdit_hip_optim.h")
+HEADER_TAIL = os.path.join(HERE, "..", "include", "mmdit_hip_tail.h")
 SOURCES = ["gemm.hip", "gemm_dma.hip", "gemm_lean.hip", "gemm8p.hip", "gemm8p_inf.hip", "rowops.hip", "fp8_pad.hip", "attention.hip", "attention_e4m3.hip", "attention_hd128.hip", "rowops_rope3.hip", "attention_qkhalf.hip", "rowops_qkhalf.hip", "attention_cos2.hip", "rowops_cos2.hip", "text_loss.hip", "vae.hip", "vae_attn.hip", "optim.hip"]
 HIPCC = os.environ.get("HIPCC", "/opt/rocm/bin/hipcc")
 FLAGS = ["--offload-arch=gfx950", "-O3", "-std=c++17", "-fPIC"] + os.environ.get("MMDIT_EXTRA_HIPCC_FLAGS", "").split()
@@ -40,7 +41,7 @@
 
 
 def source_hash(src):
-    headers = sorted(os.path.join(CSRC, f) for f in os.listdir(CSRC) if f.endswith(".h")) + [HEADER, HEADER_EXT, HEADER_HD128, HEADER_ROPE3, HEADER_QKHALF, HEADER_TEXTLOSS, HEADER_COS2, HEADER_FP8PAD, HEADER_MXPAD, HEADER_OPTIM]
+    headers = sorted(os.path.join(CSRC, f) for f in os.listdir(CSRC) if f.endswith(".h")) + [HEADER, HEADER_EXT, HEADER_HD128, HEADER_ROPE3, HEADER_QKHALF, HEADER_TEXTLOSS, HEADER_COS2, HEADER_FP8PAD, HEADER_MXPAD, HEADER_OPTIM, HEADER_TAIL]
     if src == "gemm8p_inf.hip":
         headers.append(os.path.join(CSRC, "gemm8p.hip"))
     return _sha([os.path.join(CSRC, src)] + headers, " ".join([HIPCC] + FLAGS + SOURCE_FLAGS.get(src, [])))
diff --git a/stable-diffusion-3-from-scratch_amd/csrc/rowops.hip b/stable-diffusion-3-from-scratch_amd/csrc/rowops.hip
--- a/stable-diffusion-3-from-scratch_amd/csrc/rowops.hip
+++ b/stable-diffusion-3-from-scratch_amd/csrc/rowops.hip
@@ -2,6 +2,7 @@
 #include "fp8_quant.h"
 #include "../../include/mmdit_hip_hd128.h"
 #include "../../include/mmdit_hip_mxpad.h"
+#include "../../include/mmdit_hip_tail.h"
 
 namespace {
 
@@ -276,14 +277,18 @@
   }
 }
 
-#ifndef TRB_ROWS
-#define TRB_ROWS 64
+#ifdef TRB_ROWS
+constexpr int TRB_ROWS_FIXED = TRB_ROWS;
+#else
+constexpr int TRB_ROWS_FIXED = 0;
 #endif
+constexpr int TRB_ROWS_MIN = 16, TRB_ROWS_MAX = 64;
 struct TextRmsBwdHalf { const void* dout; const float* w; const float* sp; int rows, cnt, off; float* dw; float* dsp; };
 template <int NITX, typename TI, typename TG>
-__global__ __launch_bounds__(512) void text_rms_bwd_kernel(TextRmsBwdHalf h0, TextRmsBwdHalf h1, const TI* __restrict__ x, int tokens, int d) {
+__global__ __launch_bounds__(512) void text_rms_bwd_kernel(TextRmsBwdHalf h0, TextRmsBwdHalf h1, const TI* __restrict__ x, int tokens, int d, int rpw) {
   constexpr int NIT = NITX < 0 ? -NITX : NITX;
-  constexpr bool EXACT = NITX < 0;
+  constexpr bool EXACT = NITX < 0 && NIT < 16;
+  constexpr int INFL = NIT <= 9 ? 2 : 1;
   const TextRmsBwdHalf& hp = blockIdx.y == 0 ? h0 : h1;
   const TG* __restrict__ dout = (const TG*)hp.dout;
   const float* __restrict__ w = hp.w;
@@ -291,39 +296,58 @@
   const int rows = hp.rows, cnt = hp.cnt, off = hp.off;
   float* __restrict__ dw = hp.dw;
   float* __restrict__ dsp = hp.dsp;
-  __shared__ float red[NIT * 256];
-  for (int c = threadIdx.x; c < NIT * 256; c += 512) red[c] = 0.f;
+  const int mbeg = blockIdx.x * rpw, mend = min(rows, mbeg + rpw);
+  if (mbeg >= rows) return;
+  __shared__ float red[NIT * 256], s_w[NIT * 256];
+  for (int c = threadIdx.x; c < NIT * 256; c += 512) { red[c] = 0.f; s_w[c] = c < d ? w[c] : 0.f; }
   __syncthreads();
   const int lane = threadIdx.x & 63, wave = threadIdx.x >> 6;
   const int nch = d >> 2;
   const float s = sp[0];
-  float accw[NIT][4], wv[NIT][4];
+  float accw[NIT][4];
   float accs = 0.f;
 #pragma unroll
   for (int it = 0; it < NIT; it++) {
-    int ch = lane + 64 * it;
-    if (EXACT || ch < nch) ld4(w + ch * 4, wv[it]); else { wv[it][0] = wv[it][1] = wv[it][2] = wv[it][3] = 0.f; }
 #pragma unroll
     for (int e = 0; e < 4; e++) accw[it][e] = 0.f;
   }
-  for (int m = blockIdx.x * TRB_ROWS + wave; m < min(rows, (int)(blockIdx.x + 1) * TRB_ROWS); m += 8) {
-    const TI* xr = x + ((int64_t)(m / cnt) * tokens + off + m % cnt) * d;
-    float v[NIT][4];
-    float q = 0.f;
-#pragma unroll
-    for (int it = 0; it < NIT; it++) {
-      int ch = lane + 64 * it;
-      if (EXACT || ch < nch) { ld4(xr + ch * 4, v[it]); q += v[it][0] * v[it][0] + v[it][1] * v[it][1] + v[it][2] * v[it][2] + v[it][3] * v[it][3]; }
-    }
-    const float rinv = rsqrtf(wave_sum(q) / d + RMS_EPS);
-#pragma unroll
-    for (int it = 0; it < NIT; it++) {
-      int ch = lane + 64 * it;
-      if (EXACT || ch < nch) {
-        float dy[4];
-        ld4(dout + (int64_t)m * d + ch * 4, dy);
-#pragma unroll
-        for (int e = 0; e < 4; e++) { float xn = v[it][e] * rinv; accw[it][e] += dy[e] * s * xn; accs += dy[e] * xn * wv[it][e]; }
+  for (int m0 = mbeg + wave; m0 < mend; m0 += 8 * INFL) {
+    const bool two = INFL == 2 && m0 + 8 < mend;
+    float v[INFL][NIT][4], dy[INFL == 2 ? 2 : 1][INFL == 2 ? NIT : 1][4];
+#pragma unroll
+    for (int k = 0; k < INFL; k++) {
+      const int m = k && two ? m0 + 8 : m0;
+      const TI* xr = x + ((int64_t)(m / cnt) * tokens + off + m % cnt) * d;
+#pragma unroll
+      for (int it = 0; it < NIT; it++) {
+        int ch = lane + 64 * it;
+        if (EXACT || ch < nch) {
+          ld4(xr + ch * 4, v[k][it]);
+          if constexpr (INFL == 2) ld4(dout + (int64_t)m * d + ch * 4, dy[k][it]);
+        }
+      }
+    }
+#pragma unroll
+    for (int k = 0; k < INFL; k++) {
+      if (k && !two) break;
+      float q = 0.f;
+#pragma unroll
+      for (int it = 0; it < NIT; it++) {
+        int ch = lane + 64 * it;
+        if (EXACT || ch < nch) q += v[k][it][0] * v[k][it][0] + v[k][it][1] * v[k][it][1] + v[k][it][2] * v[k][it][2] + v[k][it][3] * v[k][it][3];
+      }
+      const float rinv = rsqrtf(wave_sum(q) / d + RMS_EPS);
+#pragma unroll
+      for (int it = 0; it < NIT; it++) {
+        int ch = lane + 64 * it;
+        if (EXACT || ch < nch) {
+          float wv[4], dyv[4];
+          ld4(s_w + ch * 4, wv);
+          if constexpr (INFL == 2) { dyv[0] = dy[k][it][0]; dyv[1] = dy[k][it][1]; dyv[2] = dy[k][it][2]; dyv[3] = dy[k][it][3]; }
+          else ld4(dout + (int64_t)m0 * d + ch * 4, dyv);
+#pragma unroll
+          for (int e = 0; e < 4; e++) { float xn = v[k][it][e] * rinv; accw[it][e] += dyv[e] * s * xn; accs += dyv[e] * xn * wv[e]; }
+        }
       }
     }
   }
@@ -879,6 +903,46 @@
   colsum_flush(s, sbuf, out, c, cols);
 }
 
+constexpr int CS_INFL = 4, CS_TARGET_WGS = 1024;
+template <typename T, int CB, bool CAST>
+__global__ __launch_bounds__(256) void colsum_tall_kernel(const T* __restrict__ x, int rows, int cols, int64_t ld, float* __restrict__ out, int rch,
+                                                          bf16_t* __restrict__ y) {
+  constexpr int CL = CB / 8, RL = 256 / CL;
+  __shared__ float sbuf[RL][CB];
+  const int tx = threadIdx.x % CL, ty = threadIdx.x / CL;
+  const int c = blockIdx.x * CB + tx * 8;
+  float s[8];
+#pragma unroll
+  for (int e = 0; e < 8; e++) s[e] = 0.f;
+  if (c < cols) {
+    const int r0 = blockIdx.y * rch, rend = min(rows, r0 + rch);
+    for (int r = r0 + ty; r < rend; r += RL * CS_INFL) {
+      float v[CS_INFL][8];
+#pragma unroll
+      for (int k = 0; k < CS_INFL; k++) ld8(x + (int64_t)min(r + k * RL, rend - 1) * ld + c, v[k]);
+#pragma unroll
+      for (int k = 0; k < CS_INFL; k++) {
+        const int rr = r + k * RL;
+        if (rr < rend) {
+#pragma unroll
+          for (int e = 0; e < 8; e++) s[e] += v[k][e];
+          if constexpr (CAST) st8(y + (int64_t)rr * cols + c, v[k]);
+        }
+      }
+    }
+  }
+#pragma unroll
+  for (int e = 0; e < 8; e++) sbuf[ty][tx * 8 + e] = s[e];
+  __syncthreads();
+  const int col = blockIdx.x * CB + threadIdx.x;
+  if (threadIdx.x < CB && col < cols) {
+    float t = 0.f;
+#pragma unroll
+    for (int r = 0; r < RL; r++) t += sbuf[r][threadIdx.x];
+    atomicAdd(out + col, t);
+  }
+}
+
 template <typename TG, typename TO>
 __global__ __launch_bounds__(256) void silu_bwd_kernel(const TG* __restrict__ dy, const float* __restrict__ pre, TO* __restrict__ dpre, int rpg, int cols, float* __restrict__ dbias) {
   __shared__ float sb[4][64];
@@ -1135,6 +1199,12 @@
   return mmdit_launch_status();
 }
 
+static int trb_rows(int maxrows) {
+  if (TRB_ROWS_FIXED > 0) return TRB_ROWS_FIXED;
+  const int r = maxrows / 256 / 16 * 16;
+  return r < TRB_ROWS_MIN ? TRB_ROWS_MIN : r > TRB_ROWS_MAX ? TRB_ROWS_MAX : r;
+}
+
 extern "C" int mmdit_text_rmsnorm_bwd(const void* dout1, const void* dout2, int dout_dtype, const void* x, int x_dtype,
                                       const float* w1, const float* w2, const float* s1, const float* s2, int batch, int tokens, int split, int d,
                                       float* dw1, float* dw2, float* ds1, float* ds2, mmdit_stream_t stream) {
@@ -1148,8 +1218,9 @@
     h[half] = TextRmsBwdHalf{half ? dout2 : dout1, half ? w2 : w1, half ? s2 : s1, rows, cnt, half ? split : 0, half ? dw2 : dw1, half ? ds2 : ds1};
     maxrows = rows > maxrows ? rows : maxrows;
   }
-  dim3 grid((maxrows + TRB_ROWS - 1) / TRB_ROWS, 2);
-#define TRB(TI, TG) NIT_SWITCH(nit, hipLaunchKernelGGL((text_rms_bwd_kernel<NIT, TI, TG>), grid, dim3(512), 0, s, h[0], h[1], (const TI*)x, tokens, d))
+  const int rpw = trb_rows(maxrows);
+  dim3 grid((maxrows + rpw - 1) / rpw, 2);
+#define TRB(TI, TG) NIT_SWITCH(nit, hipLaunchKernelGGL((text_rms_bwd_kernel<NIT, TI, TG>), grid, dim3(512), 0, s, h[0], h[1], (const TI*)x, tokens, d, rpw))
   if (x_dtype == MMDIT_F32 && dout_dtype == MMDIT_F32) { TRB(float, float); }
   else if (x_dtype == MMDIT_F32 && dout_dtype == MMDIT_BF16) { TRB(float, bf16_t); }
   else if (x_dtype == MMDIT_BF16 && dout_dtype == MMDIT_BF16) { TRB(bf16_t, bf16_t); }
@@ -1394,15 +1465,44 @@
   return mmdit_launch_status();
 }
 
+static void colsum_tall_shape(int rows, int cols, int& cb, int& rch) {
+  cb = cols > 1024 ? 256 : 128;
+  const int64_t ncb = (cols + cb - 1) / cb, pass = (2048 / cb) * CS_INFL;
+  const int64_t want = (rows * ncb + CS_TARGET_WGS - 1) / CS_TARGET_WGS;
+  rch = (int)((want + pass - 1) / pass * pass);
+}
+
+template <bool CAST>
+static int colsum_tall_launch(const void* x, int dtype, int rows, int cols, int64_t ld, float* out, bf16_t* y, hipStream_t s) {
+  int cb, rch;
+  colsum_tall_shape(rows, cols, cb, rch);
+  dim3 grid((cols + cb - 1) / cb, (rows + rch - 1) / rch);
+#define CST(T, CB) hipLaunchKernelGGL((colsum_tall_kernel<T, CB, CAST>), grid, dim3(256), 0, s, (const T*)x, rows, cols, ld, out, rch, y)
+  if (dtype == MMDIT_F32) { if (cb == 128) CST(float, 128); else CST(float, 256); }
+  else if (dtype == MMDIT_BF16) {
+    if constexpr (CAST) return MMDIT_ERR_DTYPE;
+    else { if (cb == 128) CST(bf16_t, 128); else CST(bf16_t, 256); }
+  }
+  else return MMDIT_ERR_DTYPE;
+#undef CST
+  return mmdit_launch_status();
+}
+
 extern "C" int mmdit_colsum(const void* x, int dtype, int rows, int cols, int64_t ld, float* out, mmdit_stream_t stream) {
   MMDIT_CHECK_ARG(x && out && rows > 0 && cols > 0 && cols % 8 == 0 && ld % 8 == 0);
   hipStream_t s = (hipStream_t)stream;
-  const int rch = rows <= 256 ? 8 : CO_RCH;
+  if (rows > 256) return colsum_tall_launch<false>(x, dtype, rows, cols, ld, out, nullptr, s);
+  const int rch = 8;
   dim3 grid((cols + 1023) / 1024, (rows + rch - 1) / rch);
   if (dtype == MMDIT_BF16) hipLaunchKernelGGL((colsum_kernel<bf16_t>), grid, dim3(256), 0, s, (const bf16_t*)x, rows, cols, ld, out, rch);
   else if (dtype == MMDIT_F32) hipLaunchKernelGGL((colsum_kernel<float>), grid, dim3(256), 0, s, (const float*)x, rows, cols, ld, out, rch);
   else return MMDIT_ERR_DTYPE;
   return mmdit_launch_status();
+}
+
+extern "C" int mmdit_colsum_cast(const float* x, int rows, int cols, int64_t ld, void* y_bf16, float* out, mmdit_stream_t stream) {
+  MMDIT_CHECK_ARG(x && y_bf16 && out && rows > 0 && cols > 0 && cols % 8 == 0 && ld % 8 == 0 && ld >= cols);
+  return colsum_tall_launch<true>(x, MMDIT_F32, rows, cols, ld, out, (bf16_t*)y_bf16, (hipStream_t)stream);
 }
 
 namespace {
diff --git a/stable-diffusion-3-from-scratch_amd/engine.py b/stable-diffusion-3-from-scratch_amd/engine.py
--- a/stable-diffusion-3-from-scratch_amd/engine.py
+++ b/stable-diffusion-3-from-scratch_amd/engine.py
@@ -447,7 +447,7 @@
     return dqkv_x, dqkv_c
 
 
-def block_bwd_begin(m, w, sv, dims, dev, defer_cond=False):
+def block_bwd_begin(m, w, sv, dims, dev, defer_cond=False, dmod=None):
     B, N, Mt, H, d = dims
     both = not w.last
     ms = _mod_views(sv.mod, d, w.last)
@@ -458,7 +458,8 @@
     cos2 = getattr(w, "cos2", False)
     shapes = [(nb * d,), (hx,)] + ([] if cos2 else [(nw,), (nw,), (nw,), (nw,)]) + ([(sv.gu_c.shape[1],)] if both else []) + ([] if defer_cond else [(d,)])
     npar = len(shapes)
-    shapes += [tuple(sv.mod.shape), (B, nb * d)]
+    if dmod is None:
+        shapes += [tuple(sv.mod.shape)]
     zs, small_arena = _zeros_views(shapes, dev, prefix=npar)
     st = NS(g=g, ms=ms, zs=zs, npar=npar, small_arena=small_arena, both=both)
     st.bdown, g.mlp_x.bup = zs[:2]
@@ -466,13 +467,13 @@
         g.wq_x, g.wk_x, g.wq_c, g.wk_c = zs[2:6]
     if not defer_cond:
         g.by = zs[npar - 1]
-    st.dmod, st.bpart = zs[npar], zs[npar + 1]
+    st.dmod = zs[npar] if dmod is None else dmod
     g.mlp_x.bdown = st.bdown[:d]
     if both:
         g.mlp_c.bdown, g.mlp_c.bup = st.bdown[d:], zs[2 if cos2 else 6]
     st.dms = _mod_views(st.dmod, d, w.last)
-    st.req_x = (sv.acc_mx, ms.gate2x, st.dms.gate2x, st.bpart[:, :d])
-    st.req_c = (sv.acc_mc, ms.gate2c, st.dms.gate2c, st.bpart[:, d:]) if both else None
+    st.req_x = (sv.acc_mx, ms.gate2x, st.dms.gate2x, st.bdown[:d])
+    st.req_c = (sv.acc_mc, ms.gate2c, st.dms.gate2c, st.bdown[d:]) if both else None
     return st
 
 
@@ -482,19 +483,18 @@
     both = not w.last
     if st is None:
         st = block_bwd_begin(m, w, sv, dims, dev, defer_cond)
-    g, ms, dms, bpart, bdown, dmod = st.g, st.ms, st.dms, st.bpart, st.bdown, st.dmod
+    g, ms, dms, bdown, dmod = st.g, st.ms, st.dms, st.bdown, st.dmod
     pending = []
     fuse = _FUSE_GATE
 
     def defer(ns, name, dY, Xa):
         pending.append((lambda o, ns=ns, name=name: setattr(ns, name, o), _wg(dY, Xa)))
 
-    dacc_x = dacc[0] if dacc is not None else ops.gate_residual_bwd(dX2, sv.acc_mx, ms.gate2x, N, dms.gate2x, bpart[:, :d], m.T)
+    dacc_x = dacc[0] if dacc is not None else ops.gate_residual_bwd(dX2, sv.acc_mx, ms.gate2x, N, dms.gate2x, bdown[:d], m.T)
     probs = [dict(A=dacc_x, B=w.mlp_x.Wdown, b_kmajor=True, out_dtype=m.T)]
     if both:
-        dacc_c = dacc[1] if dacc is not None else ops.gate_residual_bwd(dC2, sv.acc_mc, ms.gate2c, Mt, dms.gate2c, bpart[:, d:], m.T)
+        dacc_c = dacc[1] if dacc is not None else ops.gate_residual_bwd(dC2, sv.acc_mc, ms.gate2c, Mt, dms.gate2c, bdown[d:], m.T)
         probs.append(dict(A=dacc_c, B=w.mlp_c.Wdown, b_kmajor=True, out_dtype=m.T))
-    ops.colsum(bpart, bdown)
     dgu = None
     if (_FUSE_SWIGLU_BWD and m.fast and dev.type == "cuda" and m.prec == PREC_BF16 and dacc_x.dtype == BF16 and sv.gu_x.dtype == BF16
             and not w.mlp_x.gelu and (not both or not w.mlp_c.gelu)):
@@ -570,7 +570,7 @@
     else:
         dX, dC = _ln_bwd_pair(ax, ac)
 
-    dmod_a = m.act(dmod)
+    dmod_a = dmod if (defer_cond and defer_wmod) else m.act(dmod)
     if defer_cond:
         if not defer_wmod:
             defer(g, "Wmod", dmod_a, sv.yp)
@@ -673,7 +673,15 @@
     dmodo = ops.zeros(sv.modo.shape, dev) if sv.modo.dtype == F32 else torch.zeros_like(sv.modo)
     nblk = len(W.blocks)
     sts = [None] * nblk
-    sts[nblk - 1] = block_bwd_begin(m, W.blocks[-1], sv.blocks[-1], sv.dims, dev, defer_cond=True)
+    batch_wmod = on_grads is None and _BATCH_WMOD
+    dmod_of = [None] * nblk
+    if batch_wmod:
+        nmod = [(int(b.mod.numel()) + 7) // 8 * 8 for b in sv.blocks]
+        dmod_all = ops.zeros(sum(nmod), dev)
+        for i in range(nblk):
+            o = sum(nmod[:i])
+            dmod_of[i] = dmod_all[o:o + sv.blocks[i].mod.numel()].view(sv.blocks[i].mod.shape)
+    sts[nblk - 1] = block_bwd_begin(m, W.blocks[-1], sv.blocks[-1], sv.dims, dev, defer_cond=True, dmod=dmod_of[-1])
     dacc = None
     if _FUSE_GATE:
         dX, dax = ops.ln_modulate_bwd(dlnf, sv.Xf, sv.muf, sv.rsf, sv.modo[:, d:], None, N, dmodo[:, d:], dmodo[:, :d], gated=sts[-1].req_x)
@@ -701,15 +709,14 @@
         dC = _dgrad(m, dtxt_a, W.Wtxt, F32)
         defer("Wtxt", dtxt_a, sv.Cfa)
         if _FUSE_GATE:
-            acc_mc, gate2c, dgate2c, bpart_c = sts[-1].req_c
-            dacc = (dacc[0], ops.gate_residual_bwd(dC, acc_mc, gate2c, Mt, dgate2c, bpart_c, m.T))
+            acc_mc, gate2c, dgate2c, bdown_c = sts[-1].req_c
+            dacc = (dacc[0], ops.gate_residual_bwd(dC, acc_mc, gate2c, Mt, dgate2c, bdown_c, m.T))
     g.blocks = [None] * nblk
     dmods = [None] * nblk
     yps = [None] * nblk
-    batch_wmod = on_grads is None and _BATCH_WMOD
     for i in range(nblk - 1, -1, -1):
         if i > 0:
-            sts[i - 1] = block_bwd_begin(m, W.blocks[i - 1], sv.blocks[i - 1], sv.dims, dev, defer_cond=True)
+            sts[i - 1] = block_bwd_begin(m, W.blocks[i - 1], sv.blocks[i - 1], sv.dims, dev, defer_cond=True, dmod=dmod_of[i - 1])
             dX, dC, dmods[i], g.blocks[i], dacc = block_bwd(m, W.blocks[i], sv.blocks[i], dX, dC, None, sv.dims, rope, defer_cond=True,
                                                             st=sts[i], dacc=dacc, nxt=sts[i - 1], defer_wmod=batch_wmod)
         else:
@@ -723,6 +730,9 @@
             if repl is not None:
                 _set_grad_tensors(g.blocks[i], repl)
 
+    if batch_wmod:
+        dmod_all_a = m.act(dmod_all)
+        dmods = [dmod_all_a[sum(nmod[:i]):sum(nmod[:i]) + dmod_of[i].numel()].view(dmod_of[i].shape) for i in range(nblk)]
     dyp_all = ops.zeros((nblk * B, d), dev)
     by_all = ops.zeros((nblk, d), dev)
     for i0 in range(0, nblk, 12):
@@ -743,8 +753,11 @@
             pending.append((lambda o, i=i: setattr(g.blocks[i], "Wmod", o), _wg(dmods[i], yps[i])))
 
     g.bpe = ops.zeros(d, dev)
-    ops.colsum(dX, g.bpe)
-    dX_a = m.act(dX)
+    if m.T == BF16 and dX.dtype == F32:
+        dX_a = ops.colsum_cast(dX, g.bpe)
+    else:
+        ops.colsum(dX, g.bpe)
+        dX_a = m.act(dX)
     dX0 = _dgrad(m, dX_a, W.Wpe, m.T)
     defer("Wpe", dX_a, sv.X0)
     defer("Wpatch", dX0, sv.patches)
diff --git a/stable-diffusion-3-from-scratch_amd/ops.py b/stable-diffusion-3-from-scratch_amd/ops.py
--- a/stable-diffusion-3-from-scratch_amd/ops.py
+++ b/stable-diffusion-3-from-scratch_amd/ops.py
@@ -540,7 +540,7 @@
                 raise RuntimeError(f"ln_modulate_bwd: acc ({acc.dtype}) and dout ({dout.dtype}) must have one dtype")
             dacc = torch.empty((rows, d), dtype=acc.dtype, device=dev)
             q.acc, q.gate, q.ld_gate, q.dacc, q.dgate, q.ld_dgate = _p(acc), _p(gate), gate.stride(0), _p(dacc), _p(dgate), dgate.stride(0)
-            q.dbias, q.ld_dbias = _p(dbias), (dbias.stride(0) if dbias is not None else 0)
+            q.dbias, q.ld_dbias = _p(dbias), (dbias.stride(0) if (dbias is not None and dbias.dim() == 2) else 0)
             keep.append(acc)
             outs.append((dx, dacc))
         else:
@@ -1110,6 +1110,15 @@
     return out
 
 
+def colsum_cast(x, out):
+    rows, cols = x.shape
+    if x.dtype != torch.float32 or x.stride(1) != 1:
+        raise RuntimeError("colsum_cast: an fp32 matrix with unit column stride")
+    y = torch.empty((rows, cols), dtype=torch.bfloat16, device=x.device)
+    check(_lib.lib().mmdit_colsum_cast(_p(x), rows, cols, x.stride(0), _p(y), _p(out), _s()), "mmdit_colsum_cast")
+    return y
+
+
 def patchify(img, out_dtype):
     batch, ch, H, W = img.shape
     tokens = torch.empty((batch * (H // 2) * (W // 2), ch * 4), dtype=out_dtype, device=img.device)
```

Result: no change. 2366 (median of 6 runs) (+0.1%).
